# maiziezhoulab/FocalSV

Hardware: AMD Instinct MI355X
Metric: target regions/sec (50 kb, 30x HiFi) (higher is better)
Workload: dtype u32; 1 GPU; 256 synthetic 50 kb regions per GPU, 30x HiFi-like reads U(10k,20k), 0.2% error, seed 1000+i (BASELINE.json configs[1]); regions_per_gpu=256

## Files before the change

focalsv_amd/csrc/asm.hip:

```cpp
#include "asm_kernels.h"
#include "k_kmer.h"
#include "layout.h"
#include <algorithm>
#include <chrono>
#include <cstdio>
#include <cstdlib>
#include <cstring>
#include <vector>
#include <thread>
#include <atomic>

namespace {

enum { KN_SKETCH, KN_UNIQ, KN_CHAIN, KN_BPM, KN_RESCUE, KN_PATH_FAST, KN_PATH_DP, KN_CONSENSUS, KN_REPACK, KN_EXACT, KN_STITCH, KN_PARTITION, KN_BND, KN_BND_CONS,
       KN_UNIQ_LONG, KN_CHAIN_SPILL,
       KN_COUNT,
       ST_SKETCH = KN_COUNT, ST_CHAIN, ST_VERIFY, ST_PATH, ST_CONSENSUS, ST_FINAL };
const char *const kn_names[KN_COUNT] = {"k_sketch", "k_uniq", "k_chain", "k5_bpm", "k_rescue_accept", "k_path_fast", "k_path_dp", "k_consensus",
                                        "k_repack", "k_exact", "k_stitch", "k_partition", "k_bnd_tasks", "k_bnd_consensus", "k_uniq_long", "k_chain_spill"};
static_assert(KN_COUNT <= FSV_MAX_KERNEL_STATS, "fsv_asm_stats holds every kernel's row");
enum { PASS_NONE = -1, PASS_WINDOWS, PASS_JUNCTIONS, PASS_BCIG, PASS_COUNT };

struct KTimes {
    struct Rec { int k; hipEvent_t a, b; uint64_t bytes; };
// ... 281 lines not shown
    A.ovl = W.ovl.p; A.tasks = W.tasks.p; A.task_counter = ct + CT_TASKS; A.task_cap = R.task_cap;
    A.overflow = ct + CT_OVERFLOW; A.warn = W.warn.p; A.set_cols = W.set_cols.p; A.thr_tab = W.thr_tab.p;
    A.n_sets = B.n_sets; A.k_score = P.k; A.min_anchors = min_anchors; A.min_ovlp = min_ovlp; A.bw = final_pass ? P.bw_final : P.bw_ec;
    A.emit_tasks = final_pass ? 0 : 1; A.primary_only = 0;
    A.upair_tab = W.upair_tab.p; A.pair_list = nullptr; A.n_list_dev = nullptr;
    A.amax = wide_anchors ? FSV_AMAX_WIDE : FSV_AMAX;
    A.wide_list = nullptr; A.n_wide = nullptr;
    if (!wide_anchors) {
        TRY(ensure(ctx, W.wide_list, (size_t)B.n_upairs + 4));
        A.wide_list = W.wide_list.p; A.n_wide = ct + CT_WIDE;
    }
    A.spill_list = nullptr; A.n_spill = nullptr;
    if (P.full_lists) {
        TRY(ensure(ctx, W.spill_list, (size_t)B.n_upairs + 4));
        A.spill_list = W.spill_list.p; A.n_spill = ct + CT_SPILL;
    }
    A.stamps = nullptr;
    if (getenv("FSV_CHAIN_STAMPS")) {
        TRY(ensure(ctx, W.tmp, 16));
        TRY(zero(ctx, W.tmp, 16));
        A.stamps = W.tmp.p;
    }
    W.kt.begin(ctx, PASS_WINDOWS, KN_CHAIN, 0);
    const uint32_t n_chunks = ((B.n_upairs + FSV_CHAIN_CH - 1) / FSV_CHAIN_CH + 7u) & ~7u;
    TRY(launch_chain(ctx, CHAIN_CHUNKS, R.short_reads, n_chunks, A, B.n_upairs));
    if (A.wide_list) TRY(chain_wide_pairs(ctx, A, R.short_reads, B.n_upairs));
    W.kt.end(ctx);
    TRY(chain_spilled_pairs(ctx, W, A, B.n_upairs, max_slot, ct));
    if (A.stamps) {
        unsigned long long h[16];
        TRY(download(ctx, h, W.tmp, 16));
        FSV_HIP(ctx, hipStreamSynchronize(ctx->stream));
        static const char *nm[7] = {"stage lists", "lookups", "exit: few anchors", "compaction", "chain DP", "best + walk", "tasks + records"};
        fprintf(stderr, "[fsv] k_chain (%u pairs, tasks %d):", B.n_upairs, A.emit_tasks);
        for (int i = 0; i < 7; i++) fprintf(stderr, " %s %.0f cyc x %llu;", nm[i], h[8 + i] ? (double)h[i] / h[8 + i] : 0.0, h[8 + i]);
        fprintf(stderr, "\n");
        A.stamps = nullptr;
    }
    W.last_chain = A;
    tc.stop();
    return FSV_OK;
}

struct Piece { uint32_t read, rev, len; };
void layout_set(const int32_t *len, uint32_t n, const fsv_hit *hits, uint32_t n_hit, int min_reads,
                std::vector<std::vector<Piece>> &contigs, bool &fallback)
{
    std::vector<uint8_t> contained(n, 0), used(n, 0);
    std::vector<int32_t> succ(2 * n, -1), sovl(2 * n, 0), pred(2 * n, -1);
    fallback = false;
    struct Geom { int ql, tl, qs, qe, tl5, tl3, ext5, ext3, tspan; bool internal; };
    auto geom = [&](const fsv_hit &h) {
        Geom g;
        g.ql = len[h.q]; g.tl = len[h.t]; g.qs = h.x_s; g.qe = h.x_e + 1; g.tl5 = h.y_s; g.tl3 = g.tl - (h.y_e + 1);
        g.ext5 = std::min(g.qs, g.tl5); g.ext3 = std::min(g.ql - g.qe, g.tl3); g.tspan = h.y_e + 1 - h.y_s;
        g.internal = g.ext5 > 1000 || g.ext3 > 1000 || (g.qe - g.qs) < (g.qe - g.qs + g.ext5 + g.ext3) * 0.8f || g.tspan < (g.tspan + g.ext5 + g.ext3) * 0.8f;
        return g;
    };
    for (uint32_t i = 0; i < n_hit; i++) {
        const fsv_hit &h = hits[i];
        const Geom g = geom(h);
        if (g.internal) continue;
        if (g.qs <= g.tl5 && g.ql - g.qe <= g.tl3) {
            if (g.qs >= g.tl5 && g.ql - g.qe >= g.tl3) { if (h.q > h.t) contained[h.q] = 1; }
            else contained[h.q] = 1;
        }
    }
    for (uint32_t v = 0; v < 2 * n; v++) sovl[v] = 0x7fffffff;
    for (uint32_t i = 0; i < n_hit; i++) {
        const fsv_hit &h = hits[i];
        const Geom g = geom(h);
        if (g.internal || contained[h.q] || contained[h.t]) continue;
        if ((g.qs <= g.tl5 && g.ql - g.qe <= g.tl3) || (g.qs >= g.tl5 && g.ql - g.qe >= g.tl3)) continue;
        if (g.qe - g.qs + g.ext5 + g.ext3 < 50 || g.tspan + g.ext5 + g.ext3 < 50) continue;
        int from, to, l;
        if (g.qs > g.tl5) { from = 2 * (int)h.q; to = 2 * (int)h.t + (int)h.rev; l = g.qs - g.tl5; }
        else { from = 2 * (int)h.q + 1; to = 2 * (int)h.t + (h.rev ? 0 : 1); l = (g.ql - g.qe) - g.tl3; }
        if (l < sovl[from] || (l == sovl[from] && succ[from] >= 0 && to < succ[from])) { succ[from] = to; sovl[from] = l; }
    }
    for (uint32_t v = 0; v < 2 * n; v++) { int w = succ[v]; if (w >= 0 && succ[w ^ 1] != (int)(v ^ 1)) succ[v] = -1; }
    for (uint32_t v = 0; v < 2 * n; v++) if (succ[v] >= 0) pred[succ[v]] = (int)v;
    for (uint32_t v = 0; v < 2 * n; v++) {
        const uint32_t r = v >> 1;
        if (contained[r] || used[r]) continue;
        int start = (int)v, steps = 0;
        while (pred[start] >= 0 && !used[pred[start] >> 1] && steps < (int)(2 * n)) { start = pred[start]; steps++; if (start == (int)v) break; }
        int cnt = 0;
        for (int w = start; w >= 0 && !used[w >> 1] && cnt <= (int)(2 * n); w = succ[w]) { cnt++; if (succ[w] == start) break; }
        if (cnt < min_reads) continue;
        std::vector<Piece> c;
        for (int w = start; w >= 0 && !used[w >> 1]; w = succ[w]) {
            used[w >> 1] = 1;
            const bool more = succ[w] >= 0 && !used[succ[w] >> 1];
            c.push_back(Piece{(uint32_t)(w >> 1), (uint32_t)(w & 1), (uint32_t)(more ? sovl[w] : len[w >> 1])});
        }
        contigs.push_back(std::move(c));
    }
    fallback = contigs.empty();
}

}

extern "C" void fsv_asm_default_params(fsv_asm_params *p)
{
    if (!p) return;
    p->k = 51; p->w = 51; p->hpc = 1; p->n_rounds = 3; p->min_ovlp = 1; p->min_anchors = 1; p->lookback = 64;
    p->bw_ec = 20; p->bw_final = 0; p->min_contig_reads = 4;
    p->win_rate_pm = 40; p->k_cap = FSV_K_MAX; p->accept_err_pm = 30; p->bw_rechain = 1; p->w_later = 0; p->partition = 1; p->second_round = 1; p->ins_dag = 1;
    p->min_anchors_final = 1; p->min_ovlp_final = 1; p->graph_layout = 1; p->junction_cigars = 1;
    p->full_lists = 0;
    p->kmer_filter = 0;
    p->kmer_table = 0;
    p->partial_charge = 0;
}

extern "C" void fsv_asm_ont_params(fsv_asm_params *p)
{
    if (!p) return;
    fsv_asm_default_params(p);
    p->min_ovlp = 500; p->min_anchors = 3;
    p->k = 15; p->w = 15; p->hpc = 0;
    p->bw_ec = 150; p->bw_final = 50;
    p->win_rate_pm = 250; p->k_cap = FSV_K_WIDE; p->accept_err_pm = 300;
    p->bw_rechain = 50;
    p->w_later = 63;
    p->partition = 0;
    p->second_round = 0;
    p->ins_dag = 0;
    p->min_contig_reads = 2;
    p->min_anchors_final = 0; p->min_ovlp_final = 0; p->graph_layout = 0;
}

extern "C" void fsv_asm_clr_params(fsv_asm_params *p)
{
    fsv_asm_ont_params(p);
}

extern "C" int fsv_assemble_batch_bound(const fsv_readsets *sets, uint64_t *seq_cap, uint32_t *contig_cap)
{
    if (!sets || !sets->read_len) return FSV_EINVAL;
    uint64_t tot = 0;
    for (uint32_t r = 0; r < sets->n_reads; r++) tot += (uint64_t)sets->read_len[r];
    if (seq_cap) *seq_cap = tot + tot / 8 + 1024 * (uint64_t)sets->n_sets + 4096;
    if (contig_cap) *contig_cap = sets->n_reads + sets->n_sets + 1;
    return FSV_OK;
}

struct PathJob {
    const uint32_t *store; fsv_wtask *tasks; fsv_wres *res; fsv_wpath *paths;
    uint32_t task_cap; const uint32_t *n_tasks_dev; uint32_t *ct;
    int pass, round;
    bool wide_bands; int k_cap;
    bool all_accepted;
};

template <bool STAMP, class Grid>
static int path_walks(fsv_ctx *ctx, AsmWs &W, const PathJob &J, Grid persistent)
{
    const uint32_t *store = J.store; const fsv_wtask *tasks = J.tasks; const fsv_wres *res = J.res; fsv_wpath *paths = J.paths;
    uint32_t *ct = J.ct;
    unsigned long long h[16] = {0};
    uint32_t nl = 0;
    auto clear_stamps = [&]() -> int { TRY(ensure(ctx, W.tmp, 16)); return zero(ctx, W.tmp, 16); };
    auto read_stamps = [&](const uint32_t *cnt) -> int {
        TRY(download(ctx, h, W.tmp, 16));
        if (cnt) FSV_HIP(ctx, hipMemcpyAsync(&nl, cnt, 4, hipMemcpyDeviceToHost, ctx->stream));
        FSV_HIP(ctx, hipStreamSynchronize(ctx->stream));
        return FSV_OK;
    };
    auto per_wave = [&](int i) { return h[8 + i] ? (double)h[i] / h[8 + i] : 0.0; };
    if (!W.occ_sb) FSV_HIP(ctx, hipOccupancyMaxActiveBlocksPerMultiprocessor(&W.occ_sb, k_path_sb<false>, 64, 0));
    const uint32_t grid = persistent(W.occ_sb);
    TRY(ensure(ctx, W.cols_sb, (size_t)grid * FSV_SB_QUADS * 64));
    if (STAMP) TRY(clear_stamps());
    FSV_LAUNCH(ctx, ctx->stream, k_path_sb<STAMP>, dim3(grid), dim3(64), 0, store, tasks, res, W.dp_list2.p, ct + CT_DP_SB, paths, W.cols_sb.p,
               STAMP ? W.tmp.p : nullptr);
    if (STAMP) {
        TRY(read_stamps(nullptr));
        fprintf(stderr, "[fsv] k_path_sb round %d: %llu waves, cycles per wave: forward %.0f, walk %.0f, finish %.0f (grid %u)\n", J.round, h[8], per_wave(0), per_wave(1),
                per_wave(2), grid);
    }
    auto fr = [&](auto kern, int e, const Dev<uint32_t> &list, uint32_t *cnt) -> int {
        int &pf = W.occ_fr[e - 1];
        if (!pf || STAMP) FSV_HIP(ctx, hipOccupancyMaxActiveBlocksPerMultiprocessor(&pf, kern, 64, 0));
        if (STAMP) TRY(clear_stamps());
        FSV_LAUNCH(ctx, ctx->stream, kern, dim3(persistent(pf)), dim3(64), 0, store, tasks, res, list.p, cnt, paths, STAMP ? W.tmp.p : nullptr);
        if (STAMP) {
            TRY(read_stamps(cnt));
            fprintf(stderr, "[fsv] k_path_fr<%d> round %d: %u windows, %llu waves (%d per CU), cycles per wave: table %.0f, walk %.0f, finish %.0f\n", e, J.round, nl, h[8], pf,
                    per_wave(0), per_wave(1), per_wave(2));
        }
        return FSV_OK;
    };
    TRY(fr(k_path_fr<1, STAMP>, 1, W.dp_list16, ct + CT_DP_SB16));
    TRY(fr(k_path_fr<2, STAMP>, 2, W.dp_list, ct + CT_DP));
    TRY(fr(k_path_fr<3, STAMP>, 3, W.dp_list_e3, ct + CT_DP_FR3));
    return FSV_OK;
}

static int path_stage(fsv_ctx *ctx, AsmWs &W, const PathJob &J)
{
    const uint32_t *store = J.store; const fsv_wtask *tasks = J.tasks; const fsv_wres *res = J.res; fsv_wpath *paths = J.paths;
    uint32_t *ct = J.ct;
    const uint32_t task_cap = J.task_cap, n_cu = (uint32_t)ctx->n_cu;
    auto persistent = [&](int per_cu) { return std::min<uint32_t>(fsv_grid_for(task_cap, 64), (uint32_t)std::max(1, per_cu) * n_cu); };
    W.kt.begin(ctx, J.pass, KN_PATH_FAST, 0);
    const bool fix = J.pass == PASS_WINDOWS && !J.wide_bands;
    if (fix) TRY(ensure(ctx, W.fix_list, task_cap));
    const PathLists lists{{W.dp_list16.p, W.dp_list.p, W.dp_list_e3.p, W.dp_list2.p, W.dp_list3.p, W.dp_wide.p, W.dp_xwide.p, fix ? W.fix_list.p : nullptr},
                          {ct + CT_DP_SB16, ct + CT_DP, ct + CT_DP_FR3, ct + CT_DP_SB, ct + CT_DP_GEN, ct + CT_DP_WIDE, ct + CT_DP_XW, fix ? ct + CT_FIX : nullptr}};
    FSV_LAUNCH(ctx, ctx->stream, k_path_fast, dim3((fsv_grid_for(task_cap, 256) + 7u) & ~7u), dim3(256), 0, store, W.ovl.p, tasks, res, task_cap, paths, lists,
               J.all_accepted, J.n_tasks_dev);
    W.kt.end(ctx);
    W.kt.begin(ctx, J.pass, KN_PATH_DP, 0);
    TRY(getenv("FSV_K6_STAMPS") ? path_walks<true>(ctx, W, J, persistent) : path_walks<false>(ctx, W, J, persistent));
    const uint32_t gridg = persistent(2);
    TRY(ensure(ctx, W.cols, (size_t)gridg * 64 * (FSV_WINDOW + 2) * 3));
    FSV_LAUNCH(ctx, ctx->stream, k_path_dp<uint32_t>, dim3(gridg), dim3(64), 0, store, tasks, W.dp_list3.p, ct + CT_DP_GEN, paths,
               (uint32_t *)W.cols.p );
    FSV_LAUNCH(ctx, ctx->stream, k_path_dp<uint64_t>, dim3(gridg), dim3(64), 0, store, tasks, W.dp_wide.p, ct + CT_DP_WIDE, paths, W.cols.p);
    if (J.wide_bands) {
        if (!W.occ_wide) FSV_HIP(ctx, hipOccupancyMaxActiveBlocksPerMultiprocessor(&W.occ_wide, k_path_wide, 64, 0));
        const uint32_t gridw = persistent(std::min(W.occ_wide, 12));
        TRY(ensure(ctx, W.cols_wide, (size_t)gridw * FSV_WINDOW * 2 * FSV_WL * 64));
        FSV_LAUNCH(ctx, ctx->stream, k_path_wide, dim3(gridw), dim3(64), 0, store, tasks, res, W.dp_xwide.p, ct + CT_DP_XW, paths, W.cols_wide.p, J.k_cap);
    }
    if (fix)
        FSV_LAUNCH(ctx, ctx->stream, k_fix_boundary, dim3(persistent(8)), dim3(64), 0, store, W.fix_list.p, ct + CT_FIX, J.tasks, J.res, paths, J.k_cap, ct + CT_FIXED);
    W.kt.end(ctx);
    return FSV_OK;
}

static int second_pass(fsv_ctx *ctx, AsmWs &W, const Round &R)
{
    const fsv_asm_params &P = R.P; const Batch &B = R.B; const Geometry &G = R.G;
    const uint32_t n_gwin = R.n_gwin, task_cap = R.task_cap;
    uint32_t *ct2 = W.ct_of(R.row(PASS_JUNCTIONS));
    TRY(ensure(ctx, W.lb, std::max(1u, n_gwin)));
    W.kt.begin(ctx, PASS_JUNCTIONS, KN_BND, 0);
    FSV_LAUNCH(ctx, ctx->stream, k_newlen, dim3(fsv_grid_for(B.n_reads, 256)), dim3(256), 0, W.gwin_off.p, W.cwin_len.p, B.n_reads, W.new_len.p, W.lb.p);
    const uint32_t a_words = G.word_off[B.n_reads];
    std::vector<uint32_t> brel(B.n_reads + 1, 0);
    for (uint32_t r = 0; r < B.n_reads; r++) {
        const uint64_t nx = (uint64_t)brel[r] + (uint64_t)(G.gwin_off[r + 1] - G.gwin_off[r]) * (FSV_CW_STRIDE / 16) + 2;
        if (nx + a_words >= (1ull << 32)) return fsv_fail(ctx, FSV_EUNSUP, "second consensus pass: store larger than 2^32 words; split the batch");
        brel[r + 1] = (uint32_t)nx;
    }
    const uint32_t b_words = brel[B.n_reads];
    TRY(ensure(ctx, W.sr_store, (size_t)a_words + b_words + 16));
    FSV_HIP(ctx, hipMemcpyAsync(W.sr_store.p, R.store, (size_t)a_words * 4, hipMemcpyDeviceToDevice, ctx->stream));
    TRY(upload(ctx, W.brel_off, brel));
    uint32_t *store2 = W.sr_store.p;
    FSV_LAUNCH(ctx, ctx->stream, k_repack, dim3(B.n_reads), dim3(256), 0, W.gwin_off.p, W.lb.p, W.cwin.p, W.brel_off.p, W.new_len.p, B.n_reads, 0, store2 + a_words,
               W.read_dirty.p);
    FSV_HIP(ctx, hipMemsetAsync(store2 + a_words + b_words, 0, 32, ctx->stream));
    TRY(ensure_each(ctx, task_cap, W.tasks2, W.res2, W.paths2, W.idx2, W.tasks3, W.res3, W.src3));
    TRY(ensure_each(ctx, (size_t)n_gwin + 2, W.bnd_flag, W.bnd_list, W.bnd_patch));
    TRY(ensure(ctx, W.bnd_bytes, (size_t)(n_gwin + 2) * FSV_CW_STRIDE));
    TRY(zero(ctx, W.bnd_flag, (size_t)n_gwin + 2));
    BndArgs A;
    A.tasks = W.tasks.p; A.paths = W.paths.p; A.n_tasks = R.ct + CT_TASKS;
    A.ovl_c = W.ovl_c.p; A.pair_base = W.pair_base.p; A.set_start = W.set_start.p; A.n_sets = B.n_sets; A.pair_read = W.pair_read.p;
    A.gwin_off = W.gwin_off.p; A.lb = W.lb.p; A.cwin_len = W.cwin_len.p;
    A.cov3 = W.cov3.p; A.read_dirty = W.read_dirty.p;
    A.brel_off = W.brel_off.p; A.b_base = a_words; A.thr_tab = W.thr_tab.p;
    A.tasks2 = W.tasks2.p; A.idx2 = W.idx2.p; A.n_tasks2 = ct2 + CT_TASKS;
    A.bnd_flag = W.bnd_flag.p; A.bnd_list = W.bnd_list.p; A.n_bnd = ct2 + CT_B_LIST; A.store2 = store2;
    FSV_LAUNCH(ctx, ctx->stream, k_bnd_tasks, dim3((fsv_grid_for(task_cap, 256) + 7u) & ~7u), dim3(256), 0, A);
    W.kt.end(ctx);
    W.kt.begin(ctx, PASS_JUNCTIONS, KN_BPM, 0);
    TRY(fsv_bpm_windows_dev_n(ctx, store2, W.tasks2.p, task_cap, ct2 + CT_TASKS, W.res2.p, P.k_cap));
    FSV_LAUNCH(ctx, ctx->stream, k_bnd_retry, dim3(fsv_grid_for(task_cap, 256)), dim3(256), 0, W.tasks2.p, W.res2.p, ct2 + CT_TASKS, W.tasks3.p, W.src3.p,
               ct2 + CT_B_RETRY, P.k_cap);
    TRY(fsv_bpm_windows_dev_n(ctx, store2, W.tasks3.p, task_cap, ct2 + CT_B_RETRY, W.res3.p, P.k_cap));
    FSV_LAUNCH(ctx, ctx->stream, k_bnd_scatter, dim3(fsv_grid_for(task_cap, 256)), dim3(256), 0, W.res2.p, W.res3.p, W.src3.p, ct2 + CT_B_RETRY);
    W.kt.end(ctx);
    TRY(path_stage(ctx, W, PathJob{store2, W.tasks2.p, W.res2.p, W.paths2.p, task_cap, ct2 + CT_TASKS, ct2, PASS_JUNCTIONS, R.round, R.wide_bands, P.k_cap, false}));
    const uint32_t grid_l = std::min<uint32_t>(std::max(1u, n_gwin), (uint32_t)ctx->n_cu * 16);
    W.kt.begin(ctx, PASS_JUNCTIONS, KN_BND_CONS, 0);
    if (R.wide_bands) FSV_LAUNCH(ctx, ctx->stream, k_bnd_consensus<FSV_EV_CAP_WIDE>, dim3(grid_l), dim3(64), 0, R.C, A, W.paths2.p, store2, W.bnd_patch.p, W.bnd_bytes.p);
    else FSV_LAUNCH(ctx, ctx->stream, k_bnd_consensus<FSV_EV_CAP>, dim3(grid_l), dim3(64), 0, R.C, A, W.paths2.p, store2, W.bnd_patch.p, W.bnd_bytes.p);
    FSV_LAUNCH(ctx, ctx->stream, k_bnd_apply, dim3(std::max(1u, n_gwin)), dim3(64), 0, W.gwin_read.p, W.gwin_off.p, W.bnd_patch.p, W.bnd_bytes.p, W.bnd_flag.p, n_gwin,
               W.cwin.p, W.cwin_len.p, W.changed.p, W.warn.p);
    W.kt.end(ctx);
    return FSV_OK;
}

static int fsv_bpm_paths_impl(fsv_ctx *ctx, const uint32_t *store, size_t store_words, const fsv_wtask *tasks, uint32_t n_tasks,
                             fsv_wres *res, fsv_wpath *paths)
{
    if (!ctx || !store || (!tasks && n_tasks) || (!res && n_tasks) || (!paths && n_tasks)) return FSV_EINVAL;
    if (n_tasks == 0) return FSV_OK;
    int kmax = 0;
    for (uint32_t i = 0; i < n_tasks; i++) {
        if (tasks[i].k > FSV_K_WIDE || tasks[i].x_len == 0 || tasks[i].x_len > FSV_WINDOW) return fsv_fail(ctx, FSV_EINVAL, "task k/x_len out of range");
        kmax = std::max<int>(kmax, tasks[i].k);
    }
    const int k_cap = kmax > FSV_K_MAX ? kmax : FSV_K_MAX;
    FSV_HIP(ctx, hipSetDevice(ctx->device));
    AsmWs &W = *ws_get(ctx);
    W.kt.reset();
    std::vector<fsv_wtask> t(tasks, tasks + n_tasks);
    for (auto &x : t) x.ovl = 0;
    fsv_ovl o; memset(&o, 0, sizeof(o)); o.valid = 1; o.is_match = 1;
    Dev<uint32_t> d_store;
    TRY(ensure(ctx, d_store, store_words + 16));
    TRY(zero(ctx, d_store, store_words + 16));
    FSV_HIP(ctx, hipMemcpyAsync(d_store.p, store, store_words * 4, hipMemcpyHostToDevice, ctx->stream));
    TRY(upload(ctx, W.tasks, t));
    TRY(upload(ctx, W.ovl, std::vector<fsv_ovl>{o}));
    TRY(ensure_each(ctx, n_tasks, W.res, W.paths, W.dp_list, W.dp_list2, W.dp_list3, W.dp_list16, W.dp_list_e3, W.dp_wide, W.dp_xwide));
    TRY(ensure(ctx, W.counters, CT_SLOT));
    TRY(zero(ctx, W.counters, CT_SLOT));
    TRY(zero(ctx, W.paths, n_tasks));
    TRY(fsv_bpm_windows_dev_n(ctx, d_store.p, W.tasks.p, n_tasks, nullptr, W.res.p, k_cap));
    TRY(path_stage(ctx, W, PathJob{d_store.p, W.tasks.p, W.res.p, W.paths.p, n_tasks, nullptr, W.counters.p, PASS_NONE, 0, kmax > FSV_K_MAX, k_cap, true}));
    TRY(download(ctx, res, W.res, n_tasks));
    TRY(download(ctx, paths, W.paths, n_tasks));
    FSV_HIP(ctx, hipStreamSynchronize(ctx->stream));
    return FSV_OK;
}

static int launch_bpm_ext(fsv_ctx *ctx, const uint32_t *store, const fsv_wtask *tasks, const uint32_t *list, const uint32_t *n_dev, uint32_t bound, int k_cap,
                          fsv_wext *out, unsigned long long *n_run)
{
    if (!bound) return FSV_OK;
    const uint32_t grid = std::min<uint32_t>(fsv_grid_for(bound, 64), 8u * (uint32_t)std::max(1, ctx->n_cu));
    FSV_LAUNCH(ctx, ctx->stream, k_bpm_ext, dim3(grid), dim3(64), 0, store, tasks, list, n_dev, bound, k_cap, out, n_run);
    return FSV_OK;
}

static int fsv_bpm_extensions_impl(fsv_ctx *ctx, const uint32_t *store, size_t store_words, const fsv_wtask *tasks, const uint8_t *dir, uint32_t n_tasks,
                                   int32_t k_cap, fsv_wext *out)
{
    if (!ctx || !store || (n_tasks && (!tasks || !dir || !out))) return FSV_EINVAL;
    if (k_cap < 1 || k_cap > FSV_K_WIDE) return fsv_fail(ctx, FSV_EINVAL, "k_cap must be in [1, 95]");
    if (n_tasks == 0) return FSV_OK;
    std::vector<fsv_wtask> t(tasks, tasks + n_tasks);
    for (uint32_t i = 0; i < n_tasks; i++) {
        fsv_wtask &x = t[i];
        if (x.k > FSV_K_MAX || x.x_len == 0 || x.x_len > FSV_WINDOW || dir[i] > 1) return fsv_fail(ctx, FSV_EINVAL, "extension task: k <= 31 (FSV_K_MAX), 1 <= x_len <= 375, dir 0 or 1");
        if (x.x_start < 0 || x.y_len < 0 || (uint64_t)x.x_word + ((uint64_t)x.x_start + x.x_len + 15) / 16 > store_words ||
            (uint64_t)x.y_word + ((uint64_t)x.y_len + 15) / 16 > store_words)
            return fsv_fail(ctx, FSV_EINVAL, "extension task reaches outside the store");
        x.ovl = i; x.win = dir[i];
    }
    FSV_HIP(ctx, hipSetDevice(ctx->device));
    AsmWs &W = *ws_get(ctx);
    Dev<uint32_t> d_store;
    TRY(ensure(ctx, d_store, store_words + 16));
    TRY(zero(ctx, d_store, store_words + 16));
    FSV_HIP(ctx, hipMemcpyAsync(d_store.p, store, store_words * 4, hipMemcpyHostToDevice, ctx->stream));
    TRY(upload(ctx, W.ch.ext_tasks, t));
    TRY(ensure(ctx, W.ch.ext_res, n_tasks));
    TRY(launch_bpm_ext(ctx, d_store.p, W.ch.ext_tasks.p, nullptr, nullptr, n_tasks, k_cap, W.ch.ext_res.p, nullptr));
    TRY(download(ctx, out, W.ch.ext_res, n_tasks));
    FSV_HIP(ctx, hipStreamSynchronize(ctx->stream));
    return FSV_OK;
}

static int fsv_asm_last_charge_impl(const fsv_ctx *ctx, fsv_charge_stats *out)
{
    if (!ctx || !out || !ctx->asm_ws) return FSV_EINVAL;
    const AsmWs &W = *(const AsmWs *)ctx->asm_ws;
    if (!W.ch.valid) return FSV_EINVAL;
    *out = W.ch.last;
    return FSV_OK;
}

extern "C" int fsv_asm_last_stats(const fsv_ctx *ctx, fsv_asm_stats *out)
{
    if (!ctx || !out || !ctx->asm_ws) return FSV_EINVAL;
    *out = ((const AsmWs *)ctx->asm_ws)->stats;
    return FSV_OK;
}


static int prepare_batch(fsv_ctx *ctx, AsmWs &W, const fsv_readsets *sets, Round &R)
{
    const fsv_asm_params &P = R.P; Batch &B = R.B;
    B.n_reads = sets->n_reads;
    R.set_flags = sets->set_flags;
    B.set_start.clear(); R.caller_set.clear();
    for (uint32_t s = 0; s < sets->n_sets; s++) {
        const bool low = !R.low_cov.empty() && R.low_cov[s];
        for (uint32_t r = sets->set_start[s]; r < sets->set_start[s + 1]; r++) if (low || r == sets->set_start[s]) { B.set_start.push_back(r); R.caller_set.push_back(s); }
        if (sets->set_start[s + 1] == sets->set_start[s]) { B.set_start.push_back(sets->set_start[s]); R.caller_set.push_back(s); }
    }
    B.n_sets = (uint32_t)R.caller_set.size();
    B.set_start.push_back(B.n_reads);
    B.read_set.resize(B.n_reads); B.pair_base.resize(B.n_sets + 1); B.upair_base.resize(B.n_sets + 1);
    uint64_t np = 0;
    for (uint32_t s = 0; s < B.n_sets; s++) {
        uint64_t ns = B.set_start[s + 1] - B.set_start[s];
        B.pair_base[s] = (uint32_t)np;
        B.upair_base[s] = (uint32_t)(np / 2);
        np += ns > 1 ? ns * (ns - 1) : 0;
        for (uint32_t r = B.set_start[s]; r < B.set_start[s + 1]; r++) B.read_set[r] = s;
    }
    if (np >= (1ull << 31)) return fsv_fail(ctx, FSV_EUNSUP, "too many read pairs in one batch; split it");
    B.pair_base[B.n_sets] = (uint32_t)np; B.n_pairs = (uint32_t)np;
    B.upair_base[B.n_sets] = (uint32_t)(np / 2); B.n_upairs = (uint32_t)(np / 2);
    std::vector<int32_t> &len = R.len;
    len.assign(sets->read_len, sets->read_len + B.n_reads);

    std::vector<uint8_t> thr(FSV_WINDOW + 1);
    for (int i = 0; i <= FSV_WINDOW; i++) thr[i] = thr_for_len_host(i, P.win_rate_pm);
    TRY(upload(ctx, W.thr_tab, thr));
    TRY(upload(ctx, W.set_start, B.set_start));
    TRY(upload(ctx, W.read_set, B.read_set));
    TRY(upload(ctx, W.pair_base, B.pair_base));
    TRY(upload(ctx, W.upair_base, B.upair_base));
    if (B.n_upairs) {
        TRY(ensure(ctx, W.upair_tab, B.n_upairs));
        TRY(ensure(ctx, W.pair_read, B.n_pairs));
        FSV_LAUNCH(ctx, ctx->stream, k_pair_tab, dim3((B.n_upairs + 255) / 256), dim3(256), 0, W.set_start.p, W.pair_base.p, W.upair_base.p, B.n_sets, B.n_upairs,
                   W.upair_tab.p, W.pair_read.p);
    }
    TRY(ensure(ctx, W.warn, B.n_reads));
    TRY(zero(ctx, W.warn, B.n_reads));

    R.mz_fixed.assign(B.n_reads + 1, 0);
    {
        uint64_t m = 0;
        for (uint32_t r = 0; r < B.n_reads; r++) { R.mz_fixed[r] = (uint32_t)m; m += mz_slots((int64_t)len[r] + len[r] / 8 + 64, P.w_later > 0 ? std::min(P.w, P.w_later) : P.w, P.full_lists != 0); }
        if (m >= (1ull << 32)) return fsv_fail(ctx, FSV_EUNSUP, "batch too large for 32-bit offsets; split it");
        R.mz_fixed[B.n_reads] = (uint32_t)m;
    }
    TRY(make_geometry(ctx, B, len, R.G, P.w, &R.mz_fixed));
    for (uint32_t r = 0; r <= B.n_reads; r++) R.G.word_off[r] = (uint32_t)sets->word_off[r];
    R.store = sets->store_dev;
    R.wide_bands = P.k_cap > FSV_K_MAX;
    for (uint32_t r = 0; r < B.n_reads; r++) { R.reads_in_bytes += (uint64_t)(len[r] + 3) / 4; if (len[r] >= 65536) R.short_reads = false; }
    const size_t n_ct = (size_t)(3 * P.n_rounds + 2) * CT_SLOT;
    TRY(ensure(ctx, W.counters, n_ct));
    TRY(zero(ctx, W.counters, n_ct));
    R.h_ct.assign(n_ct, 0u);
    TRY(ensure(ctx, W.set_cols, B.n_reads));
    TRY(zero(ctx, W.set_cols, B.n_reads));
    return FSV_OK;
}

static int begin_round(fsv_ctx *ctx, AsmWs &W, Round &R)
{
    R.ct = W.ct_of(R.row(PASS_WINDOWS));
    TRY(upload(ctx, W.word_off, R.G.word_off));
    TRY(upload(ctx, W.len, R.len));
    TRY(upload(ctx, W.mz_off, R.G.mz_off));
    TRY(upload(ctx, W.gwin_off, R.G.gwin_off));
    TRY(upload(ctx, W.gwin_read, R.G.gwin_read));
    if (R.G.task_bound >= (1ull << 31)) return fsv_fail(ctx, FSV_EUNSUP, "window task bound exceeds 2^31; split the batch");
    const uint32_t task_cap = R.task_cap = (uint32_t)std::max<uint64_t>(R.G.task_bound, 1);
    R.n_gwin = R.G.gwin_off[R.B.n_reads];
    TRY(ensure_each(ctx, task_cap, W.tasks, W.res, W.paths, W.dp_list, W.dp_list_e3, W.dp_list2, W.dp_list3, W.dp_list16, W.dp_wide));
    TRY(ensure(ctx, W.dp_xwide, R.wide_bands ? task_cap : 16));
    return FSV_OK;
}

static int charge_stage(fsv_ctx *ctx, AsmWs &W, const Round &R)
{
    const fsv_asm_params &P = R.P; const Batch &B = R.B;
    const uint32_t ext_cap = 2u * R.task_cap;
    ChargeState &S = W.ch;
    TRY(ensure_each(ctx, ext_cap, S.ext_tasks, S.ext_res, S.ext_list));
    TRY(ensure(ctx, S.list, (size_t)B.n_pairs + 4));
    TRY(ensure(ctx, S.n, 2));
    TRY(zero(ctx, S.n, 2));
    ChargeArgs A;
    A.ovl = W.ovl.p; A.n_pairs = B.n_pairs; A.tasks = W.tasks.p; A.res = W.res.p; A.paths = W.paths.p; A.ovl_c = W.ovl_c.p;
    A.ext_tasks = S.ext_tasks.p; A.ext_res = S.ext_res.p; A.ext_list = S.ext_list.p; A.n_ext = S.n.p;
    A.ovl_list = S.list.p; A.n_ovl = S.n.p + 1; A.stats = S.ct.p;
    A.k_cap = P.k_cap; A.accept_err_pm = P.accept_err_pm;
    TRY(S.clock.mark(ctx));
    FSV_LAUNCH(ctx, ctx->stream, k_charge_tasks, dim3(fsv_grid_for(B.n_pairs, 64)), dim3(64), 0, A);
    TRY(launch_bpm_ext(ctx, R.store, S.ext_tasks.p, S.ext_list.p, S.n.p, ext_cap, P.k_cap, S.ext_res.p, S.ct.p + CH_EXT));
    FSV_LAUNCH(ctx, ctx->stream, k_charge_accept, dim3(fsv_grid_for(B.n_pairs, 64)), dim3(64), 0, A);
    TRY(S.clock.mark(ctx));
    return FSV_OK;
}

static int verify_stage(fsv_ctx *ctx, AsmWs &W, const Round &R)
{
    const fsv_asm_params &P = R.P; const Batch &B = R.B;
    uint32_t *ct = R.ct;
    unsigned long long *cols = (unsigned long long *)(ct + CT_COLS_LO);
    Span tv(ctx, W.kt, ST_VERIFY);
    W.kt.begin(ctx, PASS_WINDOWS, KN_BPM, 0);
    TRY(fsv_bpm_windows_dev_n(ctx, R.store, W.tasks.p, R.task_cap, ct + CT_TASKS, W.res.p, P.k_cap));
    W.kt.end(ctx);
    W.kt.begin(ctx, PASS_WINDOWS, KN_RESCUE, (uint64_t)B.n_pairs * sizeof(fsv_ovl) * 2);
    if (R.wide_bands)
        FSV_LAUNCH(ctx, ctx->stream, k_rescue_accept<true>, dim3(fsv_grid_for(B.n_pairs, 64)), dim3(64), 0, R.store, W.ovl.p, B.n_pairs, W.tasks.p, W.res.p, cols,
                   W.ovl_c.p, P.k_cap, P.accept_err_pm, (uint32_t *)nullptr, (uint32_t *)nullptr);
    else {
        TRY(ensure(ctx, W.left_list, (size_t)B.n_pairs + 4));
        const uint32_t gridl = std::min<uint32_t>(std::max(1u, B.n_pairs), 8u * (uint32_t)ctx->n_cu);
        if (!P.partial_charge) {
            FSV_LAUNCH(ctx, ctx->stream, k_rescue_accept<false>, dim3(fsv_grid_for(B.n_pairs, 64)), dim3(64), 0, R.store, W.ovl.p, B.n_pairs, W.tasks.p, W.res.p, cols,
                       W.ovl_c.p, P.k_cap, P.accept_err_pm, W.left_list.p, ct + CT_LEFT);
            FSV_LAUNCH(ctx, ctx->stream, k_left_rescue<false>, dim3(gridl), dim3(64), 0, R.store, W.ovl.p, W.left_list.p, ct + CT_LEFT, W.tasks.p, W.res.p, W.paths.p,
                       W.ovl_c.p, P.k_cap, P.accept_err_pm);
        } else {
            FSV_LAUNCH(ctx, ctx->stream, (k_rescue_accept<false, true>), dim3(fsv_grid_for(B.n_pairs, 64)), dim3(64), 0, R.store, W.ovl.p, B.n_pairs, W.tasks.p, W.res.p,
                       cols, W.ovl_c.p, P.k_cap, P.accept_err_pm, W.left_list.p, ct + CT_LEFT);
            FSV_LAUNCH(ctx, ctx->stream, k_left_rescue<true>, dim3(gridl), dim3(64), 0, R.store, W.ovl.p, W.left_list.p, ct + CT_LEFT, W.tasks.p, W.res.p, W.paths.p,
                       W.ovl_c.p, P.k_cap, P.accept_err_pm);
        }
    }
    W.kt.end(ctx);
    tv.stop();
    Span tp(ctx, W.kt, ST_PATH);
    TRY(path_stage(ctx, W, PathJob{R.store, W.tasks.p, W.res.p, W.paths.p, R.task_cap, R.ct + CT_TASKS, R.ct, PASS_WINDOWS, R.round, R.wide_bands, R.P.k_cap, false}));
    tp.stop();
    if (P.partial_charge) TRY(charge_stage(ctx, W, R));
    return FSV_OK;
}

static int consensus_setup(fsv_ctx *ctx, AsmWs &W, Round &R)
{
    const fsv_asm_params &P = R.P; const Batch &B = R.B;
    const uint32_t n_gwin = R.n_gwin;
    TRY(ensure(ctx, W.cwin, (size_t)n_gwin * FSV_CW_STRIDE));
    TRY(ensure(ctx, W.cwin_len, n_gwin));
    TRY(ensure(ctx, W.new_len, B.n_reads));
    if (!B.n_pairs) TRY(zero(ctx, W.ovl_c, 1));
    TRY(ensure(ctx, W.gwin_tab, std::max(1u, n_gwin)));
    FSV_LAUNCH(ctx, ctx->stream, k_gwin_tab, dim3(fsv_grid_for(n_gwin, 256)), dim3(256), 0, W.gwin_read.p, W.gwin_off.p, W.read_set.p, W.set_start.p, W.pair_base.p, n_gwin,
               W.gwin_tab.p);
    ConsArgs &C = R.C;
    C.store = R.store; C.word_off = W.word_off.p; C.read_len = W.len.p;
    C.read_set = W.read_set.p; C.set_start = W.set_start.p; C.pair_base = W.pair_base.p;
    C.gwin_off = W.gwin_off.p; C.gwin_read = W.gwin_read.p; C.ovl_c = W.ovl_c.p;
    C.gwin_tab = W.gwin_tab.p; C.tasks = W.tasks.p;
    C.paths = W.paths.p; C.cwin = W.cwin.p; C.cwin_len = W.cwin_len.p; C.warn = W.warn.p;
    C.n_reads = B.n_reads;
    TRY(ensure(ctx, W.changed, B.n_reads));
    TRY(zero(ctx, W.changed, B.n_reads));
    C.changed = W.changed.p;
    C.read_dirty = nullptr;
    C.junction_vote = P.second_round ? 0 : 1;
    C.ins_dag = P.ins_dag ? 1 : 0;
    C.cov3 = nullptr;
    if (P.second_round && B.n_pairs) { TRY(ensure(ctx, W.cov3, std::max(1u, n_gwin))); C.cov3 = W.cov3.p; }
    if (B.n_pairs) {
        TRY(ensure(ctx, W.read_dirty, B.n_reads));
        FSV_LAUNCH(ctx, ctx->stream, k_read_dirty, dim3(B.n_reads), dim3(64), 0, W.ovl_c.p, W.paths.p, W.read_set.p, W.set_start.p, W.pair_base.p, B.n_reads, W.read_dirty.p);
        C.read_dirty = W.read_dirty.p;
    }
    return FSV_OK;
}

static int partition_setup(fsv_ctx *ctx, AsmWs &W, const Round &R, SiteArgs &SA, SiteLists &SL)
{
    const Batch &B = R.B;
    const uint32_t n_gwin = R.n_gwin;
    const size_t vec_cap = (size_t)B.n_pairs * 64 + (1u << 20);
    TRY(ensure(ctx, W.site_cnt, std::max(1u, n_gwin)));
    const size_t rec_cap = (size_t)n_gwin * 4 + 65536;
    TRY(ensure(ctx, W.site_rec, rec_cap));
    TRY(ensure(ctx, W.site_off, std::max(1u, n_gwin)));
    TRY(ensure(ctx, W.site_vec, vec_cap));
    TRY(ensure(ctx, W.site_cursor, 4));
    TRY(ensure(ctx, W.redo, B.n_reads));
    TRY(ensure(ctx, W.site_lists, (size_t)std::max(1u, n_gwin) * 2));
    TRY(zero(ctx, W.site_cursor, 4));
    TRY(zero(ctx, W.redo, B.n_reads));
    SA.site_cnt = W.site_cnt.p; SA.site_rec = W.site_rec.p; SA.vec = W.site_vec.p;
    SA.site_off = W.site_off.p; SA.rec_cursor = W.site_cursor.p + 3; SA.rec_cap = (uint32_t)std::min<size_t>(rec_cap, 0xfffffff0u);
    SA.vec_cursor = W.site_cursor.p; SA.vec_cap = (uint32_t)std::min<size_t>(vec_cap, 0xfffffff0u);
    SA.read_sites = W.redo.p;
    SL.site_cnt = SA.site_cnt; SL.win_list = W.site_lists.p; SL.redo_list = SL.win_list + std::max(1u, n_gwin);
    SL.win_n = W.site_cursor.p + 1;
    return FSV_OK;
}

static int junction_cigars(fsv_ctx *ctx, AsmWs &W, const Round &R, SiteArgs &SA, SiteLists &SL)
{
    const fsv_asm_params &P = R.P;
    const uint32_t n_gwin = R.n_gwin, task_cap = R.task_cap;
    uint32_t *ct3 = W.ct_of(R.row(PASS_BCIG));
    TRY(ensure_each(ctx, task_cap, W.tasks2, W.res2, W.paths2, W.bc_idx, W.bc_rec));
    TRY(ensure(ctx, W.bc_win, (size_t)(n_gwin + 2) * 3));
    FSV_LAUNCH(ctx, ctx->stream, k_bcwin_init, dim3(fsv_grid_for(n_gwin + 2, 256)), dim3(256), 0, W.bc_win.p, n_gwin + 2);
    BcigArgs BA;
    BA.tasks = W.tasks.p; BA.paths = W.paths.p; BA.n_tasks = R.ct + CT_TASKS;
    BA.pair_read = W.pair_read.p; BA.read_dirty = W.read_dirty.p; BA.gwin_off = W.gwin_off.p;
    BA.thr_tab = W.thr_tab.p; BA.k_cap = P.k_cap;
    BA.tasks2 = W.tasks2.p; BA.bc_idx = W.bc_idx.p; BA.n_tasks2 = ct3 + CT_TASKS;
    BA.n_same = ct3 + CT_B_RETRY; BA.n_used = ct3 + CT_B_LIST;
    BA.res2 = W.res2.p; BA.paths2 = W.paths2.p; BA.bc_rec = W.bc_rec.p; BA.bc_win = W.bc_win.p;
    W.kt.begin(ctx, KN_PARTITION, 0);
    FSV_LAUNCH(ctx, ctx->stream, k_bcig_tasks, dim3((fsv_grid_for(task_cap, 256) + 7u) & ~7u), dim3(256), 0, BA);
    W.kt.end(ctx);
    W.kt.begin(ctx, PASS_BCIG, KN_BPM, 0);
    TRY(fsv_bpm_windows_dev_n(ctx, R.store, W.tasks2.p, task_cap, ct3 + CT_TASKS, W.res2.p, P.k_cap));
    W.kt.end(ctx);
    TRY(path_stage(ctx, W, PathJob{R.store, W.tasks2.p, W.res2.p, W.paths2.p, task_cap, ct3 + CT_TASKS, ct3, PASS_BCIG, R.round, R.wide_bands, P.k_cap, false}));
    W.kt.begin(ctx, KN_PARTITION, 0);
    FSV_LAUNCH(ctx, ctx->stream, k_bcig_accept, dim3(fsv_grid_for(task_cap, 256)), dim3(256), 0, BA);
    W.kt.end(ctx);
    SA.bc_idx = W.bc_idx.p; SA.bc_rec = W.bc_rec.p; SA.bc_paths = W.paths2.p;
    SL.bc_win = W.bc_win.p;
    return FSV_OK;
}

static int consensus_stage(fsv_ctx *ctx, AsmWs &W, Round &R)
{
    const fsv_asm_params &P = R.P; const Batch &B = R.B;
    const uint32_t n_gwin = R.n_gwin;
    TRY(consensus_setup(ctx, W, R));
    const ConsArgs &C = R.C;
    const bool partition = B.n_pairs && P.partition;
    SiteArgs SA{};
    SiteLists SL{};
    if (partition) TRY(partition_setup(ctx, W, R, SA, SL));
    if (partition && P.junction_cigars) TRY(junction_cigars(ctx, W, R, SA, SL));
    const dim3 grid_w((n_gwin + 7u) & ~7u);
    W.kt.begin(ctx, PASS_WINDOWS, KN_CONSENSUS, (uint64_t)n_gwin * (96 + 448));
    if (R.wide_bands) {
        if (partition) FSV_LAUNCH(ctx, ctx->stream, (k_consensus<FSV_EV_CAP_WIDE, 1>), grid_w, dim3(64), 0, C, n_gwin, SL);
        else FSV_LAUNCH(ctx, ctx->stream, (k_consensus<FSV_EV_CAP_WIDE, 0>), grid_w, dim3(64), 0, C, n_gwin, SL);
    } else {
        if (partition) FSV_LAUNCH(ctx, ctx->stream, (k_consensus<FSV_EV_CAP, 1>), grid_w, dim3(64), 0, C, n_gwin, SL);
        else FSV_LAUNCH(ctx, ctx->stream, (k_consensus<FSV_EV_CAP, 0>), grid_w, dim3(64), 0, C, n_gwin, SL);
    }
    W.kt.end(ctx);
    if (partition) {
        const uint32_t grid_l = std::min<uint32_t>(std::max(1u, n_gwin), (uint32_t)ctx->n_cu * 16);
        W.kt.begin(ctx, KN_PARTITION, (uint64_t)B.n_reads * 4);
        FSV_LAUNCH(ctx, ctx->stream, k_snp_sites, dim3(grid_l), dim3(64), 0, C, SA, SL);
        FSV_LAUNCH(ctx, ctx->stream, k_hap_partition, dim3(B.n_reads), dim3(64), 0, C, SA, W.ovl.p, W.ovl_c.p, SL);
        if (R.wide_bands) FSV_LAUNCH(ctx, ctx->stream, k_consensus_redo<FSV_EV_CAP_WIDE>, dim3(grid_l), dim3(64), 0, C, SL);
        else FSV_LAUNCH(ctx, ctx->stream, k_consensus_redo<FSV_EV_CAP>, dim3(grid_l), dim3(64), 0, C, SL);
        W.kt.end(ctx);
    }
    return FSV_OK;
}

static int finish_round(fsv_ctx *ctx, AsmWs &W, Round &R)
{
    const fsv_asm_params &P = R.P; const Batch &B = R.B;
    const uint32_t n_gwin = R.n_gwin;
    TRY(ensure(ctx, W.lb, std::max(1u, n_gwin)));
    FSV_LAUNCH(ctx, ctx->stream, k_newlen, dim3(fsv_grid_for(B.n_reads, 256)), dim3(256), 0, W.gwin_off.p, W.cwin_len.p, B.n_reads, W.new_len.p, W.lb.p);
    std::vector<int32_t> nlen(B.n_reads);
    TRY(download(ctx, nlen.data(), W.new_len, B.n_reads));
    for (int pass = 0; pass < PASS_COUNT; pass++)
        FSV_HIP(ctx, hipMemcpyAsync(R.h_ct.data() + (size_t)R.row(pass) * CT_SLOT, W.ct_of(R.row(pass)), CT_SLOT * 4, hipMemcpyDeviceToHost, ctx->stream));
    FSV_HIP(ctx, hipStreamSynchronize(ctx->stream));
    if (R.h_ct[(size_t)R.round * CT_SLOT + CT_OVERFLOW]) return fsv_fail(ctx, FSV_ECAP, "internal window task buffer overflow");
    Geometry G2;
    TRY(make_geometry(ctx, B, nlen, G2, P.w, &R.mz_fixed));
    Dev<uint32_t> &dst = W.store[R.round & 1];
    const uint32_t total_words = G2.word_off[B.n_reads];
    TRY(ensure(ctx, dst, (size_t)total_words + 8));
    TRY(upload(ctx, W.unpack_off, G2.word_off));
    W.kt.begin(ctx, KN_REPACK, (uint64_t)n_gwin * 384 + (uint64_t)total_words * 4);
    FSV_LAUNCH(ctx, ctx->stream, k_repack, dim3(B.n_reads), dim3(256), 0, W.gwin_off.p, W.lb.p, W.cwin.p, W.unpack_off.p, W.new_len.p, B.n_reads,
               R.round + 1 < P.n_rounds ? 1 : 0, dst.p);
    W.kt.end(ctx);
    FSV_HIP(ctx, hipMemsetAsync(dst.p + total_words, 0, 32, ctx->stream));
    R.store = dst.p;
    R.len = nlen;
    for (int32_t l : R.len) if (l >= 65536) R.short_reads = false;
    R.G = G2;
    return FSV_OK;
}

struct SetLayout { std::vector<std::vector<Piece>> contigs; bool fallback = false; };
struct Final {
    std::vector<uint32_t> hit_first, hwarn, h_setcols;
    const fsv_hit *hraw = nullptr;
    bool any_inexact = false;
    std::vector<SetLayout> lay;
    uint64_t used = 0;
    Trace trace;
};

static int begin_final(fsv_ctx *ctx, AsmWs &W, Round &R)
{
    R.ct = W.ct_of(R.P.n_rounds); R.task_cap = 0;
    TRY(upload(ctx, W.word_off, R.G.word_off));
    TRY(upload(ctx, W.len, R.len));
    TRY(upload(ctx, W.mz_off, R.G.mz_off));
    TRY(ensure(ctx, W.tasks, 2));
    return FSV_OK;
}

static int rechain_listed(fsv_ctx *ctx, AsmWs &W, const Round &R, const uint32_t *n_list_dev)
{
    const fsv_asm_params &P = R.P; const Batch &B = R.B;
    ChainArgs A2 = W.last_chain;
    A2.bw = P.bw_rechain; A2.emit_tasks = 0; A2.pair_list = W.inexact_list.p; A2.n_list_dev = n_list_dev;
    A2.primary_only = 1;
    TRY(ensure(ctx, W.upair_tab_sw, std::max(1u, B.n_upairs)));
    FSV_LAUNCH(ctx, ctx->stream, k_pair_tab_swap, dim3(fsv_grid_for(B.n_upairs, 256)), dim3(256), 0, W.upair_tab.p, B.n_upairs, W.upair_tab_sw.p);
    for (int side = 0; side < 2; side++) {
        const size_t tk = W.kt.begin(ctx, KN_CHAIN, 0);
        if (side == 1) A2.upair_tab = W.upair_tab_sw.p;
        if (A2.wide_list) FSV_HIP(ctx, hipMemsetAsync(A2.n_wide, 0, 4, ctx->stream));
        if (A2.spill_list) FSV_HIP(ctx, hipMemsetAsync(A2.n_spill, 0, 4, ctx->stream));
        TRY(launch_chain(ctx, CHAIN_PAIRS, R.short_reads, B.n_upairs, A2, B.n_upairs));
        if (A2.wide_list) TRY(chain_wide_pairs(ctx, A2, R.short_reads, B.n_upairs));
        W.kt.end(ctx, tk);
        TRY(chain_spilled_pairs(ctx, W, A2, B.n_upairs, longest_slot(R.G, B.n_reads), R.ct));
    }
    return FSV_OK;
}

static int final_overlaps(fsv_ctx *ctx, AsmWs &W, Round &R, Final &F)
{
    const fsv_asm_params &P = R.P; const Batch &B = R.B;
    TRY(begin_final(ctx, W, R));
    const bool have_prev = P.n_rounds > 0 && B.n_pairs > 0;
    if (have_prev) {
        TRY(ensure(ctx, W.ovl_prev, B.n_pairs));
        FSV_HIP(ctx, hipMemcpyAsync(W.ovl_prev.p, W.ovl.p, (size_t)B.n_pairs * sizeof(fsv_ovl), hipMemcpyDeviceToDevice, ctx->stream));
    }
    TRY(overlap_stage(ctx, W, R, true));
    F.trace("overlaps");
    if (!B.n_pairs) return FSV_OK;
    TRY(ensure(ctx, W.hits, B.n_pairs));
    TRY(ensure(ctx, W.set_hits, (size_t)2 * B.n_sets + 2));
    TRY(zero(ctx, W.set_hits, B.n_sets));
    W.kt.begin(ctx, KN_EXACT, (uint64_t)B.n_pairs * sizeof(fsv_ovl));
    TRY(ensure(ctx, W.exact_flag, (size_t)B.n_upairs + 16));
    FSV_LAUNCH(ctx, ctx->stream, k_exact, dim3(B.n_upairs), dim3(64), 0, R.store, W.word_off.p, W.len.p, W.read_set.p, W.pair_base.p, W.upair_tab.p, W.ovl.p,
               W.hits.p, W.set_hits.p, W.exact_flag.p);
    W.kt.end(ctx);
    if (!have_prev) return FSV_OK;
    TRY(ensure(ctx, W.inexact_list, (size_t)B.n_upairs + 4));
    uint32_t *n_list_dev = R.ct + CT_INEXACT;
    FSV_LAUNCH(ctx, ctx->stream, k_inexact_list, dim3(fsv_grid_for(B.n_upairs, 256)), dim3(256), 0, W.upair_tab.p, W.exact_flag.p, W.ovl_prev.p, B.n_upairs,
               W.inexact_list.p, n_list_dev);
    TRY(rechain_listed(ctx, W, R, n_list_dev));
    FSV_LAUNCH(ctx, ctx->stream, k_accept_inexact, dim3(fsv_grid_for(2ull * B.n_upairs, 256)), dim3(256), 0, W.upair_tab.p, W.inexact_list.p, 0u, W.ovl.p, W.ovl_prev.p,
               W.read_set.p, W.pair_base.p, W.hits.p, W.set_hits.p, n_list_dev);
    return FSV_OK;
}

static int gather_hits(fsv_ctx *ctx, AsmWs &W, Round &R, Final &F)
{
    const Batch &B = R.B;
    F.hit_first.assign(B.n_sets + 1, 0);
    F.hwarn.resize(B.n_reads); F.h_setcols.assign(B.n_reads, 0u);
    if (B.n_pairs) TRY(download(ctx, F.hit_first.data() + 1, W.set_hits, B.n_sets));
    TRY(download(ctx, F.hwarn.data(), W.warn, B.n_reads));
    TRY(download(ctx, F.h_setcols.data(), W.set_cols, B.n_reads));
    FSV_HIP(ctx, hipMemcpyAsync(R.h_ct.data() + (size_t)R.P.n_rounds * CT_SLOT, R.ct, CT_SLOT * 4, hipMemcpyDeviceToHost, ctx->stream));
    FSV_HIP(ctx, hipStreamSynchronize(ctx->stream));
    if (B.n_pairs) {
        std::vector<uint32_t> &hit_first = F.hit_first;
// ... 23 lines not shown
{
    const fsv_asm_params &P = R.P; const Batch &B = R.B; const Geometry &G = R.G;
    const std::vector<int32_t> &len = R.len;
    const std::vector<uint32_t> &hit_first = F.hit_first;
    const fsv_hit *hraw = F.hraw;
    std::vector<uint32_t> &h_store = W.h_store;
    bool any_inexact = false;
    if (P.graph_layout && hraw) {
        for (uint32_t s2 = 0; s2 < B.n_sets; s2++) {
            bool inexact = false;
            for (uint32_t i = hit_first[s2]; i < hit_first[s2 + 1] && !inexact; i++) inexact = !(hraw[i].slot >> 31);
            if (!inexact) continue;
            if (!any_inexact && h_store.size() < (size_t)G.word_off[B.n_reads] + 1) h_store.resize((size_t)G.word_off[B.n_reads] + 1);
            any_inexact = true;
            const uint32_t w0 = G.word_off[B.set_start[s2]], w1 = G.word_off[B.set_start[s2 + 1]];
            if (w1 > w0) FSV_HIP(ctx, hipMemcpyAsync(h_store.data() + w0, R.store + w0, (size_t)(w1 - w0) * 4, hipMemcpyDeviceToHost, ctx->stream));
        }
        if (any_inexact) FSV_HIP(ctx, hipStreamSynchronize(ctx->stream));
    }
    F.any_inexact = any_inexact;
    const uint8_t *set_flags = R.set_flags;
    std::vector<SetLayout> &lay = F.lay;
    lay.resize(B.n_sets);
    const uint32_t nthr = std::max(1u, std::min({8u, std::thread::hardware_concurrency(), B.n_sets / 16 + 1}));
    std::atomic<uint32_t> next{0};
    std::atomic<int> rc_work{FSV_OK};
    auto work = [&]() {
        try {
        for (uint32_t s = next.fetch_add(1); s < B.n_sets && rc_work.load() == FSV_OK; s = next.fetch_add(1)) {
            const uint32_t r0 = B.set_start[s], ns = B.set_start[s + 1] - r0;
            if (ns == 0) continue;
            if (R.is_low(s)) { lay[s].fallback = true; continue; }
            const uint32_t nh_s = hit_first[s + 1] - hit_first[s];
            const bool unphased = set_flags && (set_flags[R.caller_set[s]] & FSV_SET_UNPHASED);
            if (P.graph_layout && !unphased) {
                fsv_layout::ReadBases rb; rb.words = any_inexact ? h_store.data() : nullptr; rb.word_off = G.word_off.data() + r0; rb.len = len.data() + r0;
                fsv_layout::Graph g(len.data() + r0, (int)ns, rb);
                std::vector<fsv_layout::Hit> hs(nh_s);
                for (uint32_t i = 0; i < nh_s; i++) {
                    const fsv_hit &h = hraw[hit_first[s] + i];
                    const int tl = len[r0 + h.t];
                    fsv_layout::Hit &x = hs[i];
                    x.qn = (int32_t)h.q; x.tn = (int32_t)h.t; x.qs = h.x_s; x.qe = h.x_e + 1; x.rev = (uint8_t)h.rev; x.el = (uint8_t)(h.slot >> 31); x.del = 0;
                    if (h.rev) { x.ts = tl - h.y_e - 1; x.te = tl - h.y_s; } else { x.ts = h.y_s; x.te = h.y_e + 1; }
                }
                g.set_hits(std::move(hs));
                g.build();
                std::vector<std::vector<fsv_layout::PieceOut>> cs;
                g.unitigs(P.min_contig_reads, cs);
                for (auto &c : cs) { std::vector<Piece> pc; for (auto &e : c) pc.push_back(Piece{e.read, e.rev, e.len}); lay[s].contigs.push_back(std::move(pc)); }
                lay[s].fallback = cs.empty();
                continue;
            }
            layout_set(len.data() + r0, ns, hraw + hit_first[s], nh_s, P.min_contig_reads, lay[s].contigs, lay[s].fallback);
        }
        } catch (const std::bad_alloc &) { int ok = FSV_OK; rc_work.compare_exchange_strong(ok, FSV_ENOMEM); }
        catch (...) { int ok = FSV_OK; rc_work.compare_exchange_strong(ok, FSV_EINTERNAL); }
    };
    struct Joiner { std::vector<std::thread> thr; ~Joiner() { for (auto &t : thr) if (t.joinable()) t.join(); } };
    {
        Joiner j;
        j.thr.reserve(nthr);
        for (uint32_t t = 1; t < nthr; t++) j.thr.emplace_back(work);
        work();
    }
    if (rc_work.load() != FSV_OK) return fsv_fail(ctx, rc_work.load(), rc_work.load() == FSV_ENOMEM ? "out of host memory (layout)" : "exception in the layout of a read set");
    return FSV_OK;
}

static int emit_contigs(fsv_ctx *ctx, AsmWs &W, const Round &R, Final &F, fsv_contigs *out)
{
    const Batch &B = R.B;
    std::vector<fsv_piece> pieces;
    uint64_t used = 0;
    uint32_t nc = 0;
    int rc_out = FSV_OK;
    for (uint32_t s = 0; s < B.n_sets && rc_out == FSV_OK; s++) {
        const uint32_t r0 = B.set_start[s], ns = B.set_start[s + 1] - r0;
        int32_t st = 0;
        for (uint32_t r = r0; r < r0 + ns; r++) st |= (int32_t)(F.hwarn[r] & (FSV_W_MZ_TRUNC | FSV_W_ANCHOR_TRUNC | FSV_W_INS_EVENTS | FSV_W_WINDOW_KEPT | FSV_W_INTERNAL | FSV_W_SITES));
        const uint32_t cs = R.caller_set[s];
        if (ns == 0) { out->set_status[cs] |= st; continue; }
        if (F.lay[s].fallback) st |= FSV_W_NO_LAYOUT;
        for (auto &c : F.lay[s].contigs) {
            uint64_t clen = 0;
            for (auto &pc : c) clen += pc.len;
            if (nc >= out->contig_cap || used + clen > out->seq_cap) { rc_out = fsv_fail(ctx, FSV_ECAP, "contig output buffers too small (use fsv_assemble_batch_bound)"); break; }
            for (auto &pc : c) { pieces.push_back(fsv_piece{r0 + pc.read, pc.rev, pc.len, 0u, used}); used += pc.len; }
            out->set[nc] = cs; out->n_reads[nc] = (uint32_t)c.size();
            out->off[++nc] = used;
        }
        out->set_status[cs] |= st;
    }
    F.trace("layout");
    if (rc_out != FSV_OK) return rc_out;
    out->n_contigs = nc;
    ctx->last_contigs_dev = nullptr;
    ctx->last_contig_off.assign(out->off, out->off + nc + 1);
    if (!pieces.empty()) {
        TRY(upload(ctx, W.pieces, pieces));
        TRY(ensure(ctx, W.contig_out, used + 16));
        W.kt.begin(ctx, KN_STITCH, used + used / 4);
        FSV_LAUNCH(ctx, ctx->stream, k_stitch, dim3((uint32_t)pieces.size()), dim3(256), 0, R.store, W.word_off.p, W.len.p, W.pieces.p, W.contig_out.p);
        W.kt.end(ctx);
        ctx->last_contigs_dev = W.contig_out.p;
        TRY(download(ctx, out->seq, W.contig_out, used));
        FSV_HIP(ctx, hipStreamSynchronize(ctx->stream));
    }
    F.trace("stitch+d2h");
    F.used = used;
    return FSV_OK;
}

static void fill_stats(AsmWs &W, const Round &R, const Final &F)
{
    const fsv_asm_params &P = R.P; const Batch &B = R.B;
    const std::vector<uint32_t> &h_ct = R.h_ct;
    KTimes &kt = W.kt;
    auto set = [&](int pass, int k, size_t round, uint64_t bytes) { if (uint64_t *b = kt.bytes_of(pass, k, round)) *b = bytes; };
    auto add = [&](int pass, int k, size_t round, uint64_t bytes) { if (uint64_t *b = kt.bytes_of(pass, k, round)) *b += bytes; };
    auto n_dp_of = [](const uint32_t *c) { return (uint64_t)c[CT_DP_SB] + c[CT_DP_SB16] + c[CT_DP] + c[CT_DP_FR3] + c[CT_DP_GEN] + c[CT_DP_WIDE] + c[CT_DP_XW]; };
    uint64_t mz_total[17] = {0}, n_windows2 = 0;
    for (int sl = 0; sl <= P.n_rounds; sl++) {
        const uint32_t *c = h_ct.data() + (size_t)sl * CT_SLOT;
        mz_total[sl] = (uint64_t)c[CT_MZ_LO] | (uint64_t)c[CT_MZ_HI] << 32;
        W.n_long_reads += c[CT_UQ_LONG]; W.n_spilled_pairs += c[CT_SPILLED];
        if (sl == P.n_rounds) { W.stats.n_inexact_candidates = c[CT_INEXACT]; break; }
        W.stats.n_windows += c[CT_TASKS];
        W.stats.dp_columns += (uint64_t)c[CT_COLS_LO] | (uint64_t)c[CT_COLS_HI] << 32;
        W.stats.n_path_dp += n_dp_of(c);
        W.stats.n_path_fr += (uint64_t)c[CT_DP_SB16] + c[CT_DP] + c[CT_DP_FR3];
        const uint64_t nt = c[CT_TASKS], n_dp = n_dp_of(c);
        set(PASS_WINDOWS, KN_BPM, sl, nt * 212ull);
        add(PASS_WINDOWS, KN_RESCUE, sl, nt * 16ull);
        set(PASS_WINDOWS, KN_PATH_FAST, sl, nt * (16ull + 196ull) + (nt - n_dp) * 128ull);
        set(PASS_WINDOWS, KN_PATH_DP, sl, n_dp * (196ull + 128ull));
        add(PASS_WINDOWS, KN_CONSENSUS, sl, nt * 128ull);
        if (kt.bytes_of(PASS_BCIG, KN_BPM, sl)) {
            const uint32_t *c3 = h_ct.data() + (size_t)(PASS_BCIG * (P.n_rounds + 1) + sl) * CT_SLOT;
            const uint64_t n3 = c3[CT_TASKS], n_dp3 = n_dp_of(c3);
            n_windows2 += n3;
            W.stats.n_junction_cigars += n3;
            W.stats.n_junction_used += c3[CT_B_LIST];
            if (getenv("FSV_BCIG_DEBUG")) fprintf(stderr, "[fsv] round %d: %u overlaps set aside for the left-extension pass; fix_boundary: %u candidates, %u windows moved\n", sl, c[CT_LEFT], c[CT_FIX], c[CT_FIXED]);
            if (getenv("FSV_BCIG_DEBUG")) fprintf(stderr, "[fsv] round %d: %llu junction cigars, %u accepted but showing what the window cigars show, %u used\n", sl, (unsigned long long)n3, c3[CT_B_RETRY], c3[CT_B_LIST]);
            set(PASS_BCIG, KN_BPM, sl, n3 * 212ull);
            set(PASS_BCIG, KN_PATH_FAST, sl, n3 * (16ull + 196ull) + (n3 - n_dp3) * 128ull);
            set(PASS_BCIG, KN_PATH_DP, sl, n_dp3 * (196ull + 128ull));
        }
        if (kt.bytes_of(PASS_JUNCTIONS, KN_BND, sl)) {
            const uint32_t *c2 = h_ct.data() + (size_t)(PASS_JUNCTIONS * (P.n_rounds + 1) + sl) * CT_SLOT;
            const uint64_t n2 = c2[CT_TASKS], n3 = c2[CT_B_RETRY], n_dp2 = n_dp_of(c2);
            n_windows2 += n2 + n3;
            set(PASS_JUNCTIONS, KN_BND, sl, nt * (sizeof(fsv_wtask) + 128ull) + n2 * sizeof(fsv_wtask));
            set(PASS_JUNCTIONS, KN_BPM, sl, (n2 + n3) * 212ull);
            set(PASS_JUNCTIONS, KN_PATH_FAST, sl, n2 * (16ull + 196ull) + (n2 - n_dp2) * 128ull);
            set(PASS_JUNCTIONS, KN_PATH_DP, sl, n_dp2 * (196ull + 128ull));
            set(PASS_JUNCTIONS, KN_BND_CONS, sl, n2 * 128ull + (uint64_t)c2[CT_B_LIST] * (sizeof(BndPatch) + 2ull * FSV_BND_HALF));
        }
    }
    for (size_t i = 0; i <= (size_t)P.n_rounds; i++) {
        const uint32_t *c = h_ct.data() + i * CT_SLOT;
        const uint64_t raw = (uint64_t)c[CT_MZRAW_LO] | (uint64_t)c[CT_MZRAW_HI] << 32, bases = (uint64_t)c[CT_BASES_LO] | (uint64_t)c[CT_BASES_HI] << 32;
        set(PASS_WINDOWS, KN_SKETCH, i, bases / 4 + raw * sizeof(fsv_mz));
        set(PASS_WINDOWS, KN_UNIQ, i, raw * sizeof(fsv_mz) + mz_total[i] * 2 * sizeof(fsv_mz));
        set(PASS_WINDOWS, KN_CHAIN, i, mz_total[i] * 32ull + (uint64_t)B.n_pairs * sizeof(fsv_ovl) + (i < (size_t)P.n_rounds ? (uint64_t)c[CT_TASKS] * sizeof(fsv_wtask) : 0ull));
    }
    for (uint32_t s2 = 0; s2 < B.n_sets; s2++) if (B.set_start[s2] < B.n_reads && B.set_start[s2 + 1] > B.set_start[s2]) W.stats.dp_columns += F.h_setcols[B.set_start[s2]];
    W.stats.algo_bytes = (W.stats.n_windows + n_windows2) * 212ull + R.reads_in_bytes * (uint64_t)(P.n_rounds + 1) + F.used;
    W.stats.ms_total = std::chrono::duration<double, std::milli>(std::chrono::steady_clock::now() - R.t_enter).count();
    W.stats.n_kernels = KN_COUNT;
    for (int k = 0; k < KN_COUNT; k++) { memset(&W.stats.kernels[k], 0, sizeof(fsv_kernel_stat)); strncpy(W.stats.kernels[k].name, kn_names[k], 23); }
    for (auto &r : kt.recs) {
        float ms = 0;
        const bool ok = hipEventElapsedTime(&ms, r.a, r.b) == hipSuccess;
        if (r.k >= KN_COUNT) {
            double *dst = r.k == ST_SKETCH ? &W.stats.ms_sketch : r.k == ST_CHAIN ? &W.stats.ms_chain : r.k == ST_VERIFY ? &W.stats.ms_verify
                        : r.k == ST_PATH ? &W.stats.ms_path : r.k == ST_CONSENSUS ? &W.stats.ms_consensus : &W.stats.ms_final;
            if (ok) *dst += ms;
            continue;
        }
        if (ok) W.stats.kernels[r.k].ms += ms;
        W.stats.kernels[r.k].launches++;
        W.stats.kernels[r.k].algo_bytes += r.bytes;
    }
}

static void add_stats(fsv_asm_stats &total, const fsv_asm_stats &st)
{
    total.n_pairs += st.n_pairs; total.n_overlaps += st.n_overlaps; total.n_windows += st.n_windows; total.n_windows_matched += st.n_windows_matched;
    total.n_paths += st.n_paths; total.n_path_dp += st.n_path_dp; total.dp_columns += st.dp_columns; total.algo_bytes += st.algo_bytes;
    total.n_exact_overlaps += st.n_exact_overlaps; total.n_inexact_candidates += st.n_inexact_candidates; total.n_path_fr += st.n_path_fr;
    total.ms_sketch += st.ms_sketch; total.ms_chain += st.ms_chain; total.ms_verify += st.ms_verify; total.ms_path += st.ms_path;
    total.ms_consensus += st.ms_consensus; total.ms_final += st.ms_final; total.ms_total += st.ms_total;
    total.n_kernels = st.n_kernels;
    for (uint32_t k = 0; k < st.n_kernels; k++) {
        memcpy(total.kernels[k].name, st.kernels[k].name, sizeof(st.kernels[k].name));
        total.kernels[k].ms += st.kernels[k].ms; total.kernels[k].launches += st.kernels[k].launches; total.kernels[k].algo_bytes += st.kernels[k].algo_bytes;
    }
}

static bool readsets_present(const fsv_readsets *sets, bool with_sets)
{
    return sets && sets->store_dev && sets->word_off && sets->read_len && (!with_sets || sets->set_start);
}

enum { RS_SETS = 1, RS_LEN = 2, RS_WORD_OFF = 4, RS_ALL = RS_SETS | RS_LEN | RS_WORD_OFF };
static int check_readsets(fsv_ctx *ctx, const fsv_readsets *sets, unsigned what)
{
    const uint32_t n_reads = sets->n_reads, n_sets = sets->n_sets;
    if (what & RS_SETS) {
        if (n_sets == 0 ? n_reads != 0 : (sets->set_start[0] != 0 || sets->set_start[n_sets] != n_reads)) return fsv_fail(ctx, FSV_EINVAL, "set_start must span [0, n_reads]");
        for (uint32_t s = 0; s < n_sets; s++) if (sets->set_start[s + 1] < sets->set_start[s]) return fsv_fail(ctx, FSV_EINVAL, "set_start not monotone");
    }
    if (what & RS_LEN)
        for (uint32_t r = 0; r < n_reads; r++) if (sets->read_len[r] < 1 || sets->read_len[r] >= (1 << 24)) return fsv_fail(ctx, FSV_EUNSUP, "read length must be in [1, 2^24)");
    if ((what & RS_WORD_OFF) && n_reads)
        for (uint32_t r = 0; r <= n_reads; r++) if (sets->word_off[r] >= (1ull << 32)) return fsv_fail(ctx, FSV_EUNSUP, "store larger than 2^32 words; split the batch");
    return FSV_OK;
}

static std::vector<uint32_t> read_set_of(const fsv_readsets *sets)
{
    std::vector<uint32_t> read_set(sets->n_reads);
    for (uint32_t s = 0; s < sets->n_sets; s++) for (uint32_t r = sets->set_start[s]; r < sets->set_start[s + 1]; r++) read_set[r] = s;
    return read_set;
}

static int stage_sketch_reads(fsv_ctx *ctx, AsmWs &W, const fsv_readsets *sets, int w, const std::vector<uint32_t> *read_set, Geometry &G, bool full_lists = false)
{
    const uint32_t n_reads = sets->n_reads;
    Batch B;
    B.n_reads = n_reads; B.n_sets = 1; B.set_start = {0u, n_reads};
    const std::vector<int32_t> len(sets->read_len, sets->read_len + n_reads);
    TRY(make_geometry(ctx, B, len, G, w, nullptr, full_lists));
    for (uint32_t r = 0; r <= n_reads; r++) G.word_off[r] = (uint32_t)sets->word_off[r];
    TRY(upload(ctx, W.word_off, G.word_off));
    TRY(upload(ctx, W.len, len));
    TRY(upload(ctx, W.mz_off, G.mz_off));
    if (read_set) TRY(upload(ctx, W.read_set, *read_set));
    TRY(ensure(ctx, W.warn, n_reads));
    TRY(zero(ctx, W.warn, n_reads));
    TRY(ensure(ctx, W.mz, G.mz_off[n_reads]));
    TRY(ensure(ctx, W.mz_cnt, n_reads));
    return FSV_OK;
}

template <class T> int append_on_device(fsv_ctx *ctx, Dev<T> &b, size_t have, const T *src, size_t n, size_t slack = 0, size_t min_elems = 0)
{
    if (!n) return FSV_OK;
    if (b.cap < (have + n + slack) * sizeof(T)) {
        Dev<T> bigger;
        TRY(ensure(ctx, bigger, std::max((have + n) * 2, min_elems)));
        if (have) FSV_HIP(ctx, hipMemcpyAsync(bigger.p, b.p, have * sizeof(T), hipMemcpyDeviceToDevice, ctx->stream));
        FSV_HIP(ctx, hipStreamSynchronize(ctx->stream));
        b.swap(bigger);
    }
    FSV_HIP(ctx, hipMemcpyAsync(b.p + have, src, n * sizeof(T), hipMemcpyDeviceToDevice, ctx->stream));
    return FSV_OK;
}

struct KmerJob {
    const fsv_readsets *sets; int w, k, hpc;
    const SketchFilter *sketch_flt;
    double *ms;
};
struct KmerResult {
    std::vector<fsv_kmer_set> sets;
    std::vector<uint32_t> hist;
    std::vector<uint64_t> flt_off;
};
struct KmerRun {
    const KmerJob &J; KmerResult &R; EventClock clock;
    std::vector<uint64_t> entries, tab_off; std::vector<KmerTile> tiles; std::vector<int32_t> cutoff;
};

static int kmer_sketch(fsv_ctx *ctx, AsmWs &W, KmerRun &K)
{
    const KmerJob &J = K.J; const fsv_readsets *sets = J.sets;
    const uint32_t n_reads = sets->n_reads, n_sets = sets->n_sets;
    K.entries.assign(n_sets, 0); K.tab_off.assign((size_t)n_sets + 1, 0);
    if (!n_reads) return FSV_OK;
    const std::vector<uint32_t> read_set = read_set_of(sets);
    Geometry G;
    TRY(stage_sketch_reads(ctx, W, sets, J.w, &read_set, G));
    TRY(K.clock.mark(ctx));
    TRY(launch_sketch(ctx, W, SketchJob{sets->store_dev, n_reads, G.word_off[n_reads], G.max_words, J.w, J.k, J.hpc, nullptr, J.w, false, nullptr,
                                     J.sketch_flt ? *J.sketch_flt : SketchFilter{}}));
    TRY(K.clock.mark(ctx));
    std::vector<uint32_t> cnt(n_reads);
    TRY(download(ctx, cnt.data(), W.mz_cnt, n_reads));
    FSV_HIP(ctx, hipStreamSynchronize(ctx->stream));
    for (uint32_t r = 0; r < n_reads; r++) K.entries[read_set[r]] += std::min<uint32_t>(cnt[r], G.mz_off[r + 1] - G.mz_off[r]);
    for (uint32_t s = 0; s < n_sets; s++) {
        const uint64_t slots = kmer_table_slots(K.entries[s]), tile = std::min<uint64_t>(slots, FSV_KMER_TILE);
        K.tab_off[s + 1] = K.tab_off[s] + slots;
        for (uint64_t f = 0; f < slots; f += tile) K.tiles.push_back(KmerTile{s, (uint32_t)tile, f});
    }
    if (K.tiles.size() >= (1ull << 31)) return fsv_fail(ctx, FSV_EUNSUP, "k-mer tables too large for one pass; split the batch");
    return FSV_OK;
}

static int kmer_count(fsv_ctx *ctx, AsmWs &W, KmerRun &K)
{
    KmerTableState &S = W.km;
    const uint32_t n_reads = K.J.sets->n_reads, n_sets = K.J.sets->n_sets;
    const uint64_t total_slots = K.tab_off[n_sets];
// ... 635 lines not shown
```

focalsv_amd/csrc/asm_kernels.h:

```cpp
#pragma once
#include "bpm_device.h"
#include "k_sketch.h"
#include <type_traits>

#define FSV_AMAX       1024
#define FSV_AMAX_WIDE_LONG 2560
#define FSV_AMAX_WIDE  4096
#define FSV_PATH_CAP    416
#define FSV_CW_STRIDE   448
#define FSV_INS_MAXLEN   12
#define FSV_SB_MAXERR    7
#define FSV_SB_QUADS ((FSV_WINDOW + 3) / 4)
#define FSV_FR_MAXERR    3
#define FSV_EV_CAP_WIDE 2048
#define FSV_EV_CAP     256

static_assert(sizeof(fsv_wpath) == 128, "fsv_wpath layout");

namespace {


struct ChainArgs {
    const uint32_t *store;
    const uint32_t *word_off;
// ... 705 lines not shown
        __threadfence_block();
        __syncthreads();
    }
}

__host__ __device__ inline size_t chain_lds_bytes(bool short_reads, int amax) { return short_reads ? (size_t)amax * 12 + (size_t)amax / 8 : (size_t)amax * 24; }

__device__ __forceinline__ int double_thr(int pre, int x_len, int k_cap)
{
    if (pre == 0 && x_len >= 4) pre = 1;
    int t = pre * 2;
    if (x_len >= 300 && t < k_cap) t = k_cap;
    if (t > k_cap) t = k_cap;
    return t;
}

template <bool WIDE, bool DEFER = false>
__global__ __launch_bounds__(64) void k_rescue_accept(const uint32_t *__restrict__ store, fsv_ovl *__restrict__ ovl, uint32_t n_pairs,
                                                      fsv_wtask *__restrict__ tasks, fsv_wres *__restrict__ res,
                                                      unsigned long long *__restrict__ stat_cols, uint4 *__restrict__ ovl_c, int k_cap, int accept_err_pm,
                                                      uint32_t *__restrict__ left_list, uint32_t *__restrict__ n_left)
{
    const uint32_t p = blockIdx.x * 64 + threadIdx.x;
    if (p >= n_pairs) return;
    fsv_ovl o = ovl[p];
    if (!o.valid) { ovl_c[p] = make_uint4(0u, 0u, 0u, 0u); return; }
    fsv_wtask *T = tasks + o.first_win;
    fsv_wres *R = res + o.first_win;
    int align = 0;
    unsigned long long cols = 0;
    int n_bad = 0;
    long long tlen0 = 0, terr0 = 0;
#pragma unroll 4
    for (int j = 0; j < o.n_win; j++) {
        const int e = R[j].err, xl = T[j].x_len;
        if (e >= 0) { align += xl; terr0 += e; } else n_bad++;
        tlen0 += xl;
    }
    for (int j = n_bad ? o.n_win - 1 : -1; j >= 0; j--) {
        if (R[j].err < 0) continue;
        int next = R[j].y_beg + R[j].end_site - R[j].extra_begin + 1;
        for (int k2 = j + 1; k2 < o.n_win && R[k2].err < 0; k2++) {
            fsv_wtask u = T[k2];
            if (next >= u.y_len) break;
            u.k = (uint8_t)double_thr(u.k, u.x_len, k_cap);
            u.y_start = next;
            fsv_wres r;
            if (!bpm_window_geometry(u, r, k_cap)) break;
            if ((u.x_len + 2 * u.k - r.extra_begin - r.extra_end) + u.k < u.x_len) break;
            if (WIDE) { WideNoSink none; bpm_run_wide(store, u, r, none, k_cap); }
            else bpm_run(store, u, r, BpmNoSink());
            cols += u.x_len;
            if (r.err < 0) break;
            T[k2] = u; R[k2] = r;
            align += u.x_len;
            next = r.y_beg + r.end_site - r.extra_begin + 1;
        }
    }
    if (n_bad && left_list) {
        bool left = false;
        for (int j = 1; j < o.n_win && !left; j++) left = R[j].err >= 0 && R[j - 1].err < 0;
        if (left) {
            left_list[atomicAdd(n_left, 1u)] = p;
            o.is_match = 0; ovl[p] = o;
            ovl_c[p] = make_uint4((uint32_t)o.x_s, (uint32_t)o.first_win, (uint32_t)o.n_win, 0u);
            if (cols) atomicAdd(stat_cols, cols);
            return;
        }
    }
    long long tlen = tlen0, terr = terr0;
    if (n_bad) {
        terr = 0;
#pragma unroll 4
        for (int j = 0; j < o.n_win; j++) { const int e = R[j].err; terr += e >= 0 ? e : T[j].x_len; }
    }
    o.align_len = align; o.err_sum = (int32_t)terr;
    const bool covered = (long long)(o.x_e - o.x_s + 1) * 9 <= (long long)align * 10;
    o.is_match = (covered && (DEFER || terr * 1000 <= tlen * accept_err_pm)) ? 1 : 0;
    ovl[p] = o;
    ovl_c[p] = make_uint4((uint32_t)o.x_s, (uint32_t)o.first_win, (uint32_t)o.n_win | (o.is_match && !DEFER ? 0x80000000u : 0u), 0u);
    if (cols) atomicAdd(stat_cols, cols);
}

struct PathLists {
    uint32_t *list[8], *cnt[8];
};
template <class Words>
__device__ __forceinline__ void path_record(fsv_wpath *__restrict__ P, const fsv_wtask &t, int start, int end, int plen, int err, bool raw0, uint32_t tail10,
                                            bool with_ops, Words word)
{
    uint32_t head10 = 0;
    if (with_ops) {
        uint2 *dst = reinterpret_cast<uint2 *>(P->ops);
        for (int i = 0; i < FSV_PATH_CAP / 32; i++) {
            const uint32_t v0 = word(2 * i), v1 = word(2 * i + 1);
            if (i == 0) head10 = v0 & 0xfffffu;
            dst[i] = make_uint2(v0, v1);
        }
    }
    P->ry_start = t.y_start - t.k + start;
    P->ry_end = t.y_start - t.k + end;
    P->path_len = (int16_t)plen; P->err = (int16_t)err; P->state = 1; P->y_rev = t.y_rev;
    P->pad = (uint16_t)((head10 ? 1u : 0u) | (tail10 ? 2u : 0u) | (raw0 ? 4u : 0u)); P->y_word = t.y_word; P->y_len = t.y_len;
}

__device__ __forceinline__ bool path_gapfree(const uint32_t *__restrict__ store, const fsv_wtask &t, const fsv_wres &r, fsv_wpath *__restrict__ P, bool write_clean_ops)
{
    const int n = t.x_len;
    const int start = r.end_site - n + 1;
    uint32_t ops32[26];
#pragma unroll
    for (int i = 0; i < 26; i++) ops32[i] = 0;
    bool ok = r.err == 0;
    if (!ok && start >= 0) {
        int mm = 0;
        const int win0 = t.y_start - t.k;
#pragma unroll
        for (int c = 0; c < 6; c++) {
            if (c * 64 < n) {
                uint32_t xb4[4], yb4[4], yv4[4];
                fetch64_x(store, t.x_word, t.x_start + c * 64, xb4);
                fetch64(store, t.y_word, t.y_len, t.y_rev, win0 + start + c * 64, yb4, yv4);
#pragma unroll
                for (int q = 0; q < 4; q++) {
                    const int b = c * 4 + q;
                    if (b * 16 < n) {
                        uint32_t d = mismatch_fields16(xb4[q], yb4[q], yv4[q]);
                        const int lim = min(16, n - b * 16);
                        if (lim < 16) d &= (1u << (2 * lim)) - 1u;
                        ops32[b] = d;
                        mm += __popc(d);
                    }
                }
            }
        }
        ok = (mm == r.err);
    }
    if (!ok) return false;
    int s2 = start, e2 = r.end_site;
    if (r.err > 0) {
        for (int i = n - 1; i >= 0 && ((ops32[i >> 4] >> ((i & 15) << 1)) & 3u) == 1u; i--) { ops32[i >> 4] |= 3u << ((i & 15) << 1); e2--; }
        for (int i = 0; i < n && ((ops32[i >> 4] >> ((i & 15) << 1)) & 3u) == 1u; i++) { ops32[i >> 4] |= 3u << ((i & 15) << 1); s2++; }
    }
    uint32_t tail10 = 0;
    if (r.err > 0) {
        const int a = max(n - 10, 0), wi = a >> 4, sh = (a & 15) << 1;
        const uint32_t lo = ops32[wi] >> sh, hi = (sh && wi + 1 < 26) ? ops32[wi + 1] << (32 - sh) : 0u;
        tail10 = (lo | hi) & 0xfffffu;
    }
    path_record(P, t, s2, e2, n, r.err, r.err > 0 && start == 0, tail10, r.err > 0 || write_clean_ops, [&](int wd) { return ops32[wd]; });
    return true;
}

__global__ __launch_bounds__(256) void k_path_fast(const uint32_t *__restrict__ store, const fsv_ovl *__restrict__ ovl,
                                                   const fsv_wtask *__restrict__ tasks, const fsv_wres *__restrict__ res, uint32_t n_tasks,
                                                   fsv_wpath *__restrict__ paths, PathLists L, bool write_clean_ops, const uint32_t *__restrict__ n_dev)
{
    if (n_dev) n_tasks = min(*n_dev, n_tasks);
    uint32_t blk;
    if (!xcd_block((n_tasks + 255u) >> 8, blk)) return;
    const uint32_t tid = blk * blockDim.x + threadIdx.x;
    if (tid >= n_tasks) return;
    const fsv_wtask t = tasks[tid];
    const fsv_wres r = res[tid];
    fsv_wpath *P = paths + tid;
    if (r.err < 0 || !ovl[t.ovl].is_match) { P->state = 0; return; }
    const bool ok = path_gapfree(store, t, r, P, write_clean_ops);
    if (L.cnt[7] && r.err > 0 && t.k <= FSV_K_MAX && (r.end_site == (int)t.x_len + 2 * (int)t.k - 1 || r.end_site - ((int)t.x_len - 1) <= r.err))
        L.list[7][atomicAdd(L.cnt[7], 1u)] = tid;
    {
        const int cls = ok ? -1 : (t.k <= FSV_K_MAX && r.err <= FSV_FR_MAXERR) ? r.err - 1 : t.k <= 15 ? (r.err <= FSV_SB_MAXERR ? 3 : 4) : t.k <= FSV_K_MAX ? 5 : 6;
        if (__any(cls >= 0)) {
            const int lane = (int)(threadIdx.x & 63u);
            unsigned long long mine = 0ull;
#pragma unroll
            for (int c = 0; c < 7; c++) {
                const unsigned long long m = __ballot(cls == c);
                if (cls == c) mine = m;
            }
            const int leader = mine ? __ffsll((long long)mine) - 1 : lane;
            uint32_t base = 0, *cnt = L.cnt[0], *list = L.list[0];
#pragma unroll
            for (int c = 1; c < 7; c++) { cnt = cls == c ? L.cnt[c] : cnt; list = cls == c ? L.list[c] : list; }
            if (cls >= 0 && lane == leader) base = atomicAdd(cnt, (uint32_t)__popcll(mine));
            const uint32_t at = __shfl(base, leader, 64) + (uint32_t)__popcll(mine & ((1ull << lane) - 1ull));
            if (cls >= 0) { P->state = 2; list[at] = tid; }
        }
    }
}

struct PathWalk {
    static constexpr int WORDS = 28, CAP = WORDS * 16;
    uint32_t (*ops)[64]; int lane;
    int plen, start, ci, cur, row, dir;
    uint32_t acc;
    __device__ __forceinline__ PathWalk(uint32_t (*s_ops)[64], int lane64) : ops(s_ops), lane(lane64) {}
    __device__ __forceinline__ void clear(int n, int end, int err, int row_)
    {
        for (int i = 0; i < WORDS; i++) ops[i][lane] = 0;
        plen = 0; start = end; ci = n - 1; cur = err; row = row_; dir = 0; acc = 0;
    }
    __device__ __forceinline__ void put(uint32_t code)
    {
        acc |= code << ((plen & 15) << 1);
        if ((plen & 15) == 15) { ops[plen >> 4][lane] = acc; acc = 0; }
        plen++;
        cur -= (int)(code != 0u);
        start -= (int)(code != 3u);
        row += (int)(code == 3u) - (int)(code == 2u);
        ci -= (int)(code != 2u);
        dir = (int)code;
    }
    __device__ __forceinline__ void matches(int steps)
    {
        const int np = plen + steps;
        if ((np >> 4) != (plen >> 4)) { ops[plen >> 4][lane] = acc; acc = 0; }
        plen = np; start -= steps; ci -= steps; dir = 0;
    }
    __device__ __forceinline__ void flush() { if (plen & 15) ops[plen >> 4][lane] = acc; }
    __device__ __forceinline__ uint32_t word(int wi) const { return ops[wi][lane]; }
    __device__ __forceinline__ uint32_t get(int i) const { return (ops[i >> 4][lane] >> ((i & 15) << 1)) & 3u; }
    __device__ __forceinline__ void set(int i, uint32_t v)
    {
        const int wi = i >> 4, sh = (i & 15) << 1;
        ops[wi][lane] = (ops[wi][lane] & ~(3u << sh)) | (v << sh);
    }
};

__device__ __forceinline__ void path_finish(const uint32_t *__restrict__ store, const fsv_wtask &t, fsv_wpath *__restrict__ P, PathWalk &w, int end, int err)
{
    int plen = w.plen, start = w.start, dir = w.dir;
    const int col = w.ci + 1;
    if (col > 0) { start -= col; plen += col; dir = 0; }
    if (plen > FSV_PATH_CAP) { P->state = 0; return; }
    if (dir != 3) start++;
    const bool raw0 = err > 0 && start == 0;
    if (err > 0) {
        int stop = -1;
        for (int i = 0; i < plen && w.get(i) == 1; i++) { w.set(i, 3); end--; stop = i; }
        for (int i = plen - 1; i >= 0 && w.get(i) == 1; i--) { w.set(i, 3); start++; }
        int xi = 0, yi = 0;
        BaseCache xc, yc;
        for (int i = plen - 1; i > stop;) {
            const int f = i & 15;
            const uint32_t wv = w.word(i >> 4);
            const uint32_t m = wv & 0xAAAAAAAAu & (f == 15 ? 0xffffffffu : ((1u << (2 * f + 2)) - 1u));
            const int skip = min(m == 0u ? f + 1 : f - ((31 - __clz(m)) >> 1), i - stop);
            if (skip > 0) { xi += skip; yi += skip; i -= skip; continue; }
            const uint32_t op = (wv >> (2 * f)) & 3u;
            int pi = i + 1, x2 = xi, y2 = yi;
            if (op == 3) y2--; else x2--;
            for (; pi < plen && x2 >= 0 && y2 >= 0; pi++, x2--, y2--) {
                const uint32_t pv = w.get(pi);
                const bool same = xc.get(store, t.x_word, t.x_start + x2) == yc.ycol(store, t, start + y2);
                if (pv >= 2 || (pv == 0 && !same)) break;
                if (pv == 1 && same) { w.set(pi - 1, 0); err--; }
                else w.set(pi - 1, pv);
                w.set(pi, op);
            }
            if (op == 2) yi++; else xi++;
            i--;
        }
    }
    auto packed = [&](int wd) -> uint32_t {
        const int a = plen - 16 - 16 * wd;
        uint32_t v = 0;
        if (a >= 0) {
            const int wi = a >> 4, sh = (a & 15) << 1;
            const uint32_t w0 = w.word(wi), w1 = (sh && wi + 1 < PathWalk::WORDS) ? w.word(wi + 1) : 0u;
            v = sh ? (w0 >> sh) | (w1 << (32 - sh)) : w0;
        } else if (a > -16) v = w.word(0) << ((-a) << 1);
        return rev_fields2(v);
    };
    path_record(P, t, start, end, plen, err, raw0, w.word(0) & 0xfffffu, true, packed);
}

template <class WordT, int LANES> struct PathSink {
    WordT *cols; uint32_t lane;
    __device__ __forceinline__ WordT &at(int c, int w) const { return cols[((size_t)c * 3 + w) * LANES + lane]; }
    __device__ __forceinline__ void operator()(int i, uint64_t d0, uint64_t vp, uint64_t vn) const
    {
        at(i + 1, 0) = (WordT)d0; at(i + 1, 1) = (WordT)vp; at(i + 1, 2) = (WordT)vn;
    }
};

template <class WordT, int LANES>
__device__ __forceinline__ void path_general(const uint32_t *__restrict__ store, const fsv_wtask &t, fsv_wpath *__restrict__ P, uint32_t (*s_ops)[64],
                                             int lane64, WordT *cols_slice)
{
    const int n = t.x_len, k = t.k, band = 2 * k + 1;
    fsv_wres r;
    const PathSink<WordT, LANES> sink{cols_slice, LANES == 1 ? 0u : (uint32_t)lane64};
    bpm_run(store, t, r, sink);
    if (r.err < 0) { P->state = 0; return; }
    PathWalk w(s_ops, lane64);
    w.clear(n, r.end_site, r.err, band - (n + 2 * k - r.end_site));
    WordT vp = sink.at(n, 1), vn = sink.at(n, 2);
    while (w.ci >= 0 && w.cur != 0) {
        const int row = w.row, cur = w.cur;
        const WordT d0 = sink.at(w.ci + 1, 0);
        const WordT vpi = w.ci > 0 ? sink.at(w.ci, 1) : (WordT)0, vni = w.ci > 0 ? sink.at(w.ci, 2) : (WordT)0;
        const WordT hn = vpi & d0, hp = vni | ~(vpi | d0);
        const int diag = cur - (int)((~(d0 >> row)) & 1u);
        const bool can_up = row != 0, can_left = row == 0 || row != band - 1;
        int left = cur, up = cur;
        if (can_left) left = cur - (int)((hp >> row) & 1u) + (int)((hn >> row) & 1u);
        if (can_up) up = cur - (int)((vp >> (row - 1)) & 1u) + (int)((vn >> (row - 1)) & 1u);
        int best = diag;
        uint32_t code = diag != cur ? 1u : 0u;
        if (can_up && up < best) { best = up; code = 2u; }
        if (can_left && left < best) code = 3u;
        if (code != 2u) { vp = vpi; vn = vni; }
        w.put(code);
    }
    w.flush();
    path_finish(store, t, P, w, r.end_site, r.err);
}

template <class WordT>
__global__ __launch_bounds__(64) void k_path_dp(const uint32_t *__restrict__ store, const fsv_wtask *__restrict__ tasks,
                                                const uint32_t *__restrict__ dp_list, const uint32_t *__restrict__ n_dev,
                                                fsv_wpath *__restrict__ paths, WordT *__restrict__ cols)
{
    __shared__ uint32_t s_ops[PathWalk::WORDS][64];
    const int lane64 = threadIdx.x;
    const uint32_t n_list = *n_dev;
    for (uint32_t li = blockIdx.x * 64 + threadIdx.x; li < n_list; li += gridDim.x * 64) {
        const uint32_t tid = dp_list[li];
        const fsv_wtask t = tasks[tid];
        path_general<WordT, 64>(store, t, paths + tid, s_ops, lane64, cols + (size_t)blockIdx.x * (FSV_WINDOW + 2) * 3 * 64);
    }
}

__device__ __forceinline__ void fix_boundary_dev(const uint32_t *__restrict__ store, fsv_wtask &t, fsv_wres &r, fsv_wpath *__restrict__ P, uint32_t (*s_ops)[64],
                                                 uint64_t *cols, int k_cap)
{
    const uint4 h = *reinterpret_cast<const uint4 *>(P);
    if ((h.w & 0xffu) != 1u || r.err <= 0 || t.k > FSV_K_MAX || (r.extra_begin & 0x4000)) return;
    const int n = t.x_len, k = t.k, wlen = n + 2 * k;
    const bool raw0 = ((h.w >> 16) & 4u) != 0u;
    fsv_wtask t2 = t;
// ... 655 lines not shown
```

focalsv_amd/csrc/fsv_internal.h:

```cpp
#pragma once
#include <hip/hip_runtime.h>
#include <stdint.h>
#include <chrono>
#include <cstdio>
#include <cstdlib>
#include <new>
#include <stdexcept>
#include <string>
#include <vector>
#include "focalsv_hip.h"

struct fsv_ctx {
    int device = -1;
    hipStream_t stream = nullptr;
    bool own_stream = false;
    int n_cu = 0;
    int clock_khz = 0;
    uint64_t hbm_bytes = 0;
    std::string name;
    std::string last_error;
    void *asm_ws = nullptr;
    void (*asm_ws_free)(fsv_ctx *) = nullptr;
    const char *last_contigs_dev = nullptr;
    std::vector<uint64_t> last_contig_off;
// ... 13 lines not shown
static inline int fsv_fail(fsv_ctx *ctx, int code, const char *msg)
{
    if (ctx) ctx->last_error = msg;
    return code;
}

__device__ __forceinline__ uint32_t fsv_base_fwd(const uint32_t *__restrict__ store, uint32_t word_off, int pos)
{
    return (store[word_off + ((uint32_t)pos >> 4)] >> (((uint32_t)pos & 15u) << 1)) & 3u;
}

__device__ __forceinline__ uint32_t fsv_base_at(const uint32_t *__restrict__ store, uint32_t word_off, int len, int rev, int p)
{
    int q = rev ? (len - 1 - p) : p;
    uint32_t b = fsv_base_fwd(store, word_off, q);
    return rev ? (3u - b) : b;
}

__device__ __forceinline__ int wave_max_i32(int v)
{
    const int lowest = -2147483647 - 1;
    v = max(v, __builtin_amdgcn_update_dpp(lowest, v, 0xB1, 0xF, 0xF, false));
    v = max(v, __builtin_amdgcn_update_dpp(lowest, v, 0x4E, 0xF, 0xF, false));
    v = max(v, __builtin_amdgcn_update_dpp(lowest, v, 0x141, 0xF, 0xF, false));
    v = max(v, __builtin_amdgcn_update_dpp(lowest, v, 0x140, 0xF, 0xF, false));
    const int a = __builtin_amdgcn_readlane(v, 0), b = __builtin_amdgcn_readlane(v, 16);
    const int c = __builtin_amdgcn_readlane(v, 32), d = __builtin_amdgcn_readlane(v, 48);
    return max(max(a, b), max(c, d));
}
__device__ __forceinline__ long long wave_max_i64(long long v)
{
    for (int off = 32; off > 0; off >>= 1) { long long o = __shfl_xor(v, off, 64); v = o > v ? o : v; }
    return v;
}

__device__ __forceinline__ uint32_t block_waves_before_256(uint32_t wave_total, uint32_t *s_w, uint32_t *total)
{
    const uint32_t wv = threadIdx.x >> 6;
    if ((threadIdx.x & 63u) == 63u) s_w[wv] = wave_total;
    __syncthreads();
    uint32_t before = 0, all = 0;
#pragma unroll
    for (uint32_t v = 0; v < 4; v++) { const uint32_t c = s_w[v]; if (v < wv) before += c; all += c; }
    *total = all;
    return before;
}
__device__ __forceinline__ uint32_t block_offset_256(uint32_t cnt, uint32_t *s_w, uint32_t *total)
{
    const uint32_t lane = threadIdx.x & 63u;
    uint32_t incl = cnt;
    for (uint32_t off = 1; off < 64; off <<= 1) { const uint32_t o = __shfl_up(incl, off, 64); if (lane >= off) incl += o; }
    return block_waves_before_256(incl, s_w, total) + incl - cnt;
}
__device__ __forceinline__ uint32_t block_rank_256(bool keep, uint32_t *s_w, uint32_t *total)
{
    const uint64_t bal = __ballot(keep);
    return block_waves_before_256((uint32_t)__popcll(bal), s_w, total) + (uint32_t)__popcll(bal & ((1ull << (threadIdx.x & 63u)) - 1ull));
}

#define FSV_KMER_EMPTY (~0ull)
struct KmerSet {
    uint64_t base, size;
    __device__ __forceinline__ uint64_t start(uint64_t h) const { return (h ^ (h >> 29)) & (size - 1); }
    __device__ __forceinline__ bool has(const unsigned long long *__restrict__ keys, uint64_t h) const
    {
        uint64_t slot = start(h);
        for (uint64_t probe = 0; probe < size; probe++) {
            const unsigned long long cur = keys[base + slot];
            if (cur == h) return true;
            if (cur == FSV_KMER_EMPTY) return false;
            slot = (slot + 1) & (size - 1);
        }
        return false;
    }
    __device__ __forceinline__ uint64_t claim(unsigned long long *keys, uint64_t h) const
    {
        uint64_t slot = start(h);
        for (uint64_t probe = 0; probe < size; probe++) {
            unsigned long long cur = keys[base + slot];
            if (cur == FSV_KMER_EMPTY) { cur = atomicCAS(&keys[base + slot], FSV_KMER_EMPTY, h); if (cur == FSV_KMER_EMPTY) cur = h; }
            if (cur == h) return slot;
            slot = (slot + 1) & (size - 1);
        }
        return size;
    }
};

int fsv_live_contexts(int device);

#define FSV_GUARD(ctx, call)                                                            \
    try { return (call); }                                                              \
    catch (const std::bad_alloc &) { return fsv_fail(ctx, FSV_ENOMEM, "out of host memory"); } \
    catch (const std::exception &e) { if (ctx) (ctx)->last_error = std::string("exception: ") + e.what(); return FSV_EINTERNAL; } \
    catch (...) { return fsv_fail(ctx, FSV_EINTERNAL, "unknown exception"); }

static inline unsigned fsv_grid_for(uint64_t n, unsigned block) { return (unsigned)((n + block - 1) / block); }

#define TRY(x) do { int rc_ = (x); if (rc_ != FSV_OK) return rc_; } while (0)

template <class T> struct Dev {
    T *p = nullptr;
    size_t cap = 0;
    Dev() = default;
    Dev(const Dev &) = delete;
    Dev &operator=(const Dev &) = delete;
    ~Dev() { if (p) (void)hipFree(p); }
    void swap(Dev &o) { T *tp = p; p = o.p; o.p = tp; const size_t tc = cap; cap = o.cap; o.cap = tc; }
};

template <class T> int ensure(fsv_ctx *ctx, Dev<T> &b, size_t n)
{
    const size_t bytes = n * sizeof(T);
    if (bytes <= b.cap && b.p) return FSV_OK;
    if (b.p) { FSV_HIP(ctx, hipStreamSynchronize(ctx->stream)); FSV_HIP(ctx, hipFree(b.p)); b.p = nullptr; b.cap = 0; }
    const size_t want = bytes + bytes / 8 + 256;
    FSV_HIP(ctx, hipMalloc((void **)&b.p, want));
    b.cap = want;
    return FSV_OK;
}

template <class T> int upload(fsv_ctx *ctx, Dev<T> &b, const std::vector<T> &v)
{
    TRY(ensure(ctx, b, v.empty() ? 1 : v.size()));
    if (!v.empty()) FSV_HIP(ctx, hipMemcpyAsync(b.p, v.data(), v.size() * sizeof(T), hipMemcpyHostToDevice, ctx->stream));
    return FSV_OK;
}

template <class T> int zero(fsv_ctx *ctx, Dev<T> &b, size_t n) { FSV_HIP(ctx, hipMemsetAsync(b.p, 0, n * sizeof(T), ctx->stream)); return FSV_OK; }
template <class T> int download(fsv_ctx *ctx, T *host, const Dev<T> &b, size_t n) { FSV_HIP(ctx, hipMemcpyAsync(host, b.p, n * sizeof(T), hipMemcpyDeviceToHost, ctx->stream)); return FSV_OK; }
template <class... Ts> int ensure_each(fsv_ctx *ctx, size_t n, Dev<Ts> &...b) { int rc = FSV_OK; (void)(((rc = ensure(ctx, b, n)) == FSV_OK) && ...); return rc; }

#define FSV_LAUNCH(ctx, stream, kern, grid, block, lds, ...) \
    do { hipLaunchKernelGGL(kern, grid, block, lds, stream, __VA_ARGS__); FSV_HIP(ctx, hipGetLastError()); } while (0)

struct Timer {
    std::chrono::steady_clock::time_point t0; fsv_ctx *ctx;
    explicit Timer(fsv_ctx *c) : ctx(c) { (void)hipStreamSynchronize(c->stream); t0 = std::chrono::steady_clock::now(); }
    double stop() { (void)hipStreamSynchronize(ctx->stream); return std::chrono::duration<double, std::milli>(std::chrono::steady_clock::now() - t0).count(); }
};
struct Trace {
    fsv_ctx *ctx = nullptr; const char *who = ""; std::chrono::steady_clock::time_point t0 = std::chrono::steady_clock::now();
    void operator()(const char *what)
    {
        if (!getenv("FSV_TRACE")) return;
        (void)hipStreamSynchronize(ctx->stream);
        const auto t = std::chrono::steady_clock::now();
        fprintf(stderr, "[fsv] %s %-14s %.2f ms\n", who, what, std::chrono::duration<double, std::milli>(t - t0).count());
        t0 = t;
    }
};

int fsv_bpm_windows_dev_n(fsv_ctx *ctx, const uint32_t *store_dev, const fsv_wtask *tasks_dev, uint32_t n_tasks, const uint32_t *n_dev,
                          fsv_wres *res_dev, int k_cap);
```

focalsv_amd/csrc/k5_bpm.hip:

```cpp
#include "bpm_device.h"
#include <algorithm>

namespace {

__global__ __launch_bounds__(256) void k5_bpm_kernel(const uint32_t *__restrict__ store, const fsv_wtask *__restrict__ tasks,
                                                     uint32_t n_tasks, fsv_wres *__restrict__ res, const uint32_t *__restrict__ n_dev)
{
    if (n_dev) n_tasks = min(*n_dev, n_tasks);
    uint32_t blk;
    if (!xcd_block((n_tasks + 255u) >> 8, blk)) return;
    const uint32_t tid = blk * blockDim.x + threadIdx.x;
    if (tid >= n_tasks) return;
    const fsv_wtask t = tasks[tid];
    fsv_wres r;
    bool exact = bpm_window_geometry(t, r);
    if (exact) {
        const int n = t.x_len;
        uint32_t acc = 0;
#pragma unroll
        for (int c = 0; c < (FSV_WINDOW + 63) / 64; c++) {
            if (c * 64 < n) {
                uint32_t xb[4], yb[4], yv[4];
                fetch64_x(store, t.x_word, t.x_start + c * 64, xb);
                fetch64(store, t.y_word, t.y_len, t.y_rev, t.y_start + c * 64, yb, yv);
#pragma unroll
                for (int j = 0; j < 4; j++) {
                    const int i = c * 64 + j * 16;
                    if (i < n) {
                        const int lim = min(16, n - i);
                        const uint32_t fm = lim < 16 ? (1u << (2 * lim)) - 1u : 0xffffffffu, vm = (1u << lim) - 1u;
                        acc |= ((xb[j] ^ yb[j]) & fm) | ((yv[j] & vm) ^ vm);
                    }
                }
            }
        }
        exact = acc == 0u;
        if (exact) { r.end_site = n - 1 + t.k; r.err = 0; }
    }
    if (!exact) {
        if (t.k <= 15) { BpmNoSink32 none; bpm_run32(store, t, r, none); }
        else bpm_run(store, t, r, BpmNoSink());
    }
    res[tid] = r;
}

__global__ __launch_bounds__(256) void k5_bpm_wide_kernel(const uint32_t *__restrict__ store, const fsv_wtask *__restrict__ tasks,
                                                          uint32_t n_tasks, fsv_wres *__restrict__ res, const uint32_t *__restrict__ n_dev, int k_cap)
{
    uint32_t tid = blockIdx.x * blockDim.x + threadIdx.x;
    if (n_dev) n_tasks = min(*n_dev, n_tasks);
    if (tid >= n_tasks) return;
    const fsv_wtask t = tasks[tid];
    fsv_wres r;
    WideNoSink none;
    bpm_run_wide(store, t, r, none, k_cap);
    res[tid] = r;
}

}

extern "C" int fsv_bpm_windows_dev(fsv_ctx *ctx, const uint32_t *store_dev, const fsv_wtask *tasks_dev, uint32_t n_tasks,
                                   fsv_wres *res_dev)
{
    return fsv_bpm_windows_dev_n(ctx, store_dev, tasks_dev, n_tasks, nullptr, res_dev, FSV_K_MAX);
}

int fsv_bpm_windows_dev_n(fsv_ctx *ctx, const uint32_t *store_dev, const fsv_wtask *tasks_dev, uint32_t n_tasks, const uint32_t *n_dev,
                          fsv_wres *res_dev, int k_cap)
{
    if (!ctx || !store_dev || (!tasks_dev && n_tasks) || (!res_dev && n_tasks)) return FSV_EINVAL;
    if (n_tasks == 0) return FSV_OK;
    if (k_cap > FSV_K_WIDE) return fsv_fail(ctx, FSV_EUNSUP, "window thresholds above 95 (bands above 191 rows) are not built");
    FSV_HIP(ctx, hipSetDevice(ctx->device));
    if (k_cap > FSV_K_MAX)
        FSV_LAUNCH(ctx, ctx->stream, k5_bpm_wide_kernel, dim3(fsv_grid_for(n_tasks, 256)), dim3(256), 0, store_dev, tasks_dev, n_tasks, res_dev, n_dev, k_cap);
    else
    FSV_LAUNCH(ctx, ctx->stream, k5_bpm_kernel, dim3((fsv_grid_for(n_tasks, 256) + 7u) & ~7u), dim3(256), 0, store_dev, tasks_dev, n_tasks, res_dev, n_dev);
    return FSV_OK;
}

extern "C" int fsv_bpm_windows(fsv_ctx *ctx, const uint32_t *store, size_t store_words, const fsv_wtask *tasks,
                               uint32_t n_tasks, fsv_wres *res)
{
    if (!ctx || !store || (!tasks && n_tasks) || (!res && n_tasks)) return FSV_EINVAL;
    int kmax = 0;
    for (uint32_t i = 0; i < n_tasks; i++) {
        if (tasks[i].k > FSV_K_WIDE || tasks[i].x_len == 0 || tasks[i].x_len > FSV_WINDOW) return fsv_fail(ctx, FSV_EINVAL, "task k/x_len out of range");
        kmax = std::max<int>(kmax, tasks[i].k);
    }
    const int k_cap = kmax > FSV_K_MAX ? kmax : FSV_K_MAX;
    void *d_store = nullptr, *d_tasks = nullptr, *d_res = nullptr;
    int rc = FSV_OK;
    FSV_HIP(ctx, hipSetDevice(ctx->device));
    if (hipMalloc(&d_store, store_words * 4 + 16) != hipSuccess || hipMalloc(&d_tasks, (size_t)n_tasks * sizeof(fsv_wtask) + 16) != hipSuccess ||
        hipMalloc(&d_res, (size_t)n_tasks * sizeof(fsv_wres) + 16) != hipSuccess) {
        rc = fsv_fail(ctx, FSV_ENOMEM, "hipMalloc failed");
    }
    if (rc == FSV_OK) rc = fsv_h2d(ctx, d_store, store, store_words * 4);
    if (rc == FSV_OK) rc = fsv_h2d(ctx, d_tasks, tasks, (size_t)n_tasks * sizeof(fsv_wtask));
    if (rc == FSV_OK) rc = fsv_bpm_windows_dev_n(ctx, (const uint32_t *)d_store, (const fsv_wtask *)d_tasks, n_tasks, nullptr, (fsv_wres *)d_res, k_cap);
    if (rc == FSV_OK) rc = fsv_d2h(ctx, res, d_res, (size_t)n_tasks * sizeof(fsv_wres));
    (void)hipFree(d_store); (void)hipFree(d_tasks); (void)hipFree(d_res);
    return rc;
}
```

focalsv_amd/csrc/k_consensus.h:

```cpp
#pragma once

namespace {

struct ConsArgs {
    const uint32_t *store;
    const uint32_t *word_off;
    const int32_t *read_len;
    const uint32_t *read_set;
    const uint32_t *set_start;
    const uint32_t *pair_base;
    const uint32_t *gwin_off;
    const uint32_t *gwin_read;
    const uint4 *ovl_c;
    const uint4 *gwin_tab;
    const fsv_wtask *tasks;
    const fsv_wpath *paths;
    uint8_t *cwin;
    uint16_t *cwin_len;
    uint32_t *warn;
    uint32_t *changed;
    uint32_t n_reads;
    const uint32_t *read_dirty;
    uint8_t *cov3;
    int junction_vote;
    int ins_dag;
};

__device__ __forceinline__ bool vote_wins(int cnt, int total, bool homo)
{
    if (cnt * 5 >= total * 3) return true;
    return homo && cnt * 1000 >= total * 515;
}

__global__ __launch_bounds__(64) void k_read_dirty(const uint4 *__restrict__ ovl_c, const fsv_wpath *__restrict__ paths, const uint32_t *__restrict__ read_set,
                                                   const uint32_t *__restrict__ set_start, const uint32_t *__restrict__ pair_base, uint32_t n_reads,
                                                   uint32_t *__restrict__ read_dirty)
{
    const uint32_t r = blockIdx.x;
    if (r >= n_reads) return;
    const uint32_t s = read_set[r], r0 = set_start[s], ns = set_start[s + 1] - r0;
    const uint32_t pbase = pair_base[s] + (r - r0) * (ns - 1), n_ovl = ns - 1;
    bool dirty = false;
    for (uint32_t oi = threadIdx.x; oi < n_ovl; oi += 64) {
        const uint4 oc = ovl_c[pbase + oi];
        if (!(oc.z >> 31)) continue;
        const int n_win = (int)(oc.z & 0x7fffffffu);
        int prev_end = 0; bool prev_ok = false;
        for (int j = 0; j < n_win && !dirty; j++) {
            const uint4 h0 = *reinterpret_cast<const uint4 *>(paths + (oc.y + (uint32_t)j));
            const bool ok = (h0.w & 0xffu) == 1u;
            if (ok) {
                if ((int16_t)(h0.z >> 16) != 0) dirty = true;
                if (prev_ok && (int)h0.x - prev_end - 1 != 0) dirty = true;
                prev_end = (int)h0.y;
            }
            prev_ok = ok;
        }
    }
    const bool any = __ballot(dirty) != 0ull;
    if (threadIdx.x == 0) read_dirty[r] = any ? 1u : 0u;
}

__global__ void k_gwin_tab(const uint32_t *__restrict__ gwin_read, const uint32_t *__restrict__ gwin_off, const uint32_t *__restrict__ read_set,
                           const uint32_t *__restrict__ set_start, const uint32_t *__restrict__ pair_base, uint32_t n_gwin, uint4 *__restrict__ tab)
{
    const uint32_t gw = blockIdx.x * blockDim.x + threadIdx.x;
    if (gw >= n_gwin) return;
    const uint32_t r = gwin_read[gw], s = read_set[r], r0 = set_start[s], ns = set_start[s + 1] - r0;
    tab[gw] = make_uint4(r, pair_base[s] + (r - r0) * (ns - 1), ns - 1, gw - gwin_off[r]);
}

#define FSV_SITE_MARK 0xffffffffu
#define FSV_DG_N 64
#define FSV_DG_E 128
#define FSV_DG_A 8
#define FSV_DG_D 8
#define FSV_DG_K 64
struct DagLds {
    uint32_t keys[FSV_DG_K];
    uint16_t e_w[FSV_DG_E];
    uint8_t e_from[FSV_DG_E], e_to[FSV_DG_E], e_alive[FSV_DG_E], e_vis[FSV_DG_E];
    uint8_t base[FSV_DG_N], alive[FSV_DG_N], out_n[FSV_DG_N], in_n[FSV_DG_N];
    uint8_t out_e[FSV_DG_N][FSV_DG_A], in_e[FSV_DG_N][FSV_DG_A];
    uint8_t queue[4 * FSV_DG_E];
    uint8_t stk_node[16], stk_bi[16], stk_cons[16];
    int n_node, n_edge, ok;
};

__device__ __forceinline__ int dg_node(DagLds &D, uint8_t b)
{
    const int id = D.n_node;
    if (id >= FSV_DG_N) { D.ok = 0; return FSV_DG_N - 1; }
    D.base[id] = b; D.alive[id] = 1; D.out_n[id] = 0; D.in_n[id] = 0; D.n_node = id + 1;
    return id;
}
__device__ __forceinline__ void dg_edge(DagLds &D, int u, int v, int w, int vis)
{
    const int e = D.n_edge;
    if (e >= FSV_DG_E || D.out_n[u] >= FSV_DG_A || D.in_n[v] >= FSV_DG_A) { D.ok = 0; return; }
    D.e_from[e] = (uint8_t)u; D.e_to[e] = (uint8_t)v; D.e_w[e] = (uint16_t)w; D.e_alive[e] = 1; D.e_vis[e] = (uint8_t)vis; D.n_edge = e + 1;
    D.out_e[u][D.out_n[u]++] = (uint8_t)e; D.in_e[v][D.in_n[v]++] = (uint8_t)e;
}
__device__ __forceinline__ int dg_find(const DagLds &D, int u, int v)
{
    for (int i = 0; i < D.in_n[v]; i++) { const int e = D.in_e[v][i]; if (D.e_alive[e] && D.e_from[e] == u) return e; }
    return -1;
}
__device__ __forceinline__ int dg_outdeg(const DagLds &D, int u) { int c = 0; for (int i = 0; i < D.out_n[u]; i++) c += D.e_alive[D.out_e[u][i]]; return c; }
__device__ __forceinline__ int dg_indeg(const DagLds &D, int u) { int c = 0; for (int i = 0; i < D.in_n[u]; i++) c += D.e_alive[D.in_e[u][i]]; return c; }
__device__ __forceinline__ void dg_delete(DagLds &D, int x)
{
    D.alive[x] = 0; D.base[x] = 'D';
    for (int i = 0; i < D.out_n[x]; i++) D.e_alive[D.out_e[x][i]] = 0;
    for (int i = 0; i < D.in_n[x]; i++) D.e_alive[D.in_e[x][i]] = 0;
    D.out_n[x] = 0; D.in_n[x] = 0;
}
template <bool OUT>
__device__ __forceinline__ void dg_merge(DagLds &D, int start)
{
    int sp = 0;
    D.stk_node[0] = (uint8_t)start; D.stk_bi[0] = 0;
    if (!D.alive[start] || (OUT ? dg_outdeg(D, start) : dg_indeg(D, start)) == 0) return;
    while (sp >= 0 && D.ok) {
        const int cur = D.stk_node[sp], bi = D.stk_bi[sp];
        if (bi >= 4) { sp--; continue; }
        D.stk_bi[sp] = (uint8_t)(bi + 1);
        const uint8_t want = (uint8_t)("ACGT"[bi]);
        int flag = 0, weight = 0, cons = -1;
        const int nl = OUT ? D.out_n[cur] : D.in_n[cur];
        for (int i = 0; i < nl; i++) {
            const int e = OUT ? D.out_e[cur][i] : D.in_e[cur][i];
            if (!D.e_alive[e]) continue;
            const int g = OUT ? D.e_to[e] : D.e_from[e];
            if (D.base[g] != want || (OUT ? dg_indeg(D, g) : dg_outdeg(D, g)) != 1) continue;
            if (flag == 0) { flag = 1; cons = g; D.e_vis[e] = 1; weight = D.e_w[e]; }
            else {
                flag++;
                weight += D.e_w[e];
                const int ng = OUT ? D.out_n[g] : D.in_n[g];
                for (int j = 0; j < ng; j++) {
                    const int e2 = OUT ? D.out_e[g][j] : D.in_e[g][j];
                    if (!D.e_alive[e2]) continue;
                    const int o = OUT ? D.e_to[e2] : D.e_from[e2];
                    const int e3 = OUT ? dg_find(D, cons, o) : dg_find(D, o, cons);
                    if (e3 >= 0) { D.e_vis[e3] = 1; D.e_w[e3] = (uint16_t)(D.e_w[e3] + D.e_w[e2]); }
                    else if (OUT) dg_edge(D, cons, o, D.e_w[e2], 1);
                    else dg_edge(D, o, cons, D.e_w[e2], 1);
                }
                dg_delete(D, g);
            }
        }
        if (flag > 1) { const int e = OUT ? dg_find(D, cur, cons) : dg_find(D, cons, cur); if (e >= 0) D.e_w[e] = (uint16_t)weight; }
        if (flag > 0 && D.alive[cons] && (OUT ? dg_outdeg(D, cons) : dg_indeg(D, cons)) != 0) {
            if (sp + 1 >= 16) { D.ok = 0; return; }
            sp++;
            D.stk_node[sp] = (uint8_t)cons; D.stk_bi[sp] = 0;
        }
    }
}
__device__ __forceinline__ int dg_weight(const DagLds &D, int u, bool in)
{
    int w = 0;
    if (in) { for (int i = 0; i < D.in_n[u]; i++) if (D.e_alive[D.in_e[u][i]]) w += D.e_w[D.in_e[u][i]]; }
    else for (int i = 0; i < D.out_n[u]; i++) if (D.e_alive[D.out_e[u][i]]) w += D.e_w[D.out_e[u][i]];
    return w;
}
__device__ __forceinline__ int dag_insertion(DagLds &D, int nk, uint32_t &out_key)
{
    out_key = 0;
    if (nk > FSV_DG_K) return -1;
    for (int z = 1; z < nk; z++) { const uint32_t kv = D.keys[z]; int z2 = z; for (; z2 > 0 && D.keys[z2 - 1] > kv; z2--) D.keys[z2] = D.keys[z2 - 1]; D.keys[z2] = kv; }
    uint32_t distinct[FSV_DG_D]; int cnt[FSV_DG_D], nd = 0;
    for (int i = 0; i < nk; i++) {
        if (nd && distinct[nd - 1] == D.keys[i]) { cnt[nd - 1]++; continue; }
        if (nd == FSV_DG_D) return -1;
        distinct[nd] = D.keys[i]; cnt[nd] = 1; nd++;
    }
    if (nd == 1) { out_key = distinct[0]; return cnt[0]; }
    D.n_node = 0; D.n_edge = 0; D.ok = 1;
    const int S = dg_node(D, 'S'), E = dg_node(D, 'E');
    for (int i = 0; i < nd; i++) {
        const int len = (int)(distinct[i] >> 24);
        int last = S;
        for (int j = 0; j < len; j++) { const int nn = dg_node(D, (uint8_t)("ACGT"[(distinct[i] >> (2 * j)) & 3u])); dg_edge(D, last, nn, cnt[i], 0); last = nn; }
        if (last != S) dg_edge(D, last, E, cnt[i], 0);
    }
    int qh = 0, qt = 0;
    D.queue[qt++] = (uint8_t)S;
    while (qh < qt && D.ok) {
        const int cur = D.queue[qh++];
        dg_merge<false>(D, cur);
        dg_merge<true>(D, cur);
        if (!D.alive[cur]) continue;
        for (int i = 0; i < D.out_n[cur]; i++) if (D.e_alive[D.out_e[cur][i]]) D.e_vis[D.out_e[cur][i]] = 1;
        for (int i = 0; i < D.out_n[cur]; i++) {
            const int e = D.out_e[cur][i];
            if (!D.e_alive[e]) continue;
            const int o = D.e_to[e];
            bool all = true;
            for (int j = 0; j < D.in_n[o]; j++) if (D.e_alive[D.in_e[o][j]] && !D.e_vis[D.in_e[o][j]]) { all = false; break; }
            if (all) { if (qt < 4 * FSV_DG_E) D.queue[qt++] = (uint8_t)o; else D.ok = 0; }
        }
    }
    if (!D.ok) return -1;
    int best_s = -1, best_e = -1, ws = 0, we = 0;
    for (int i = 0; i < D.out_n[S]; i++) { const int e = D.out_e[S][i]; if (D.e_alive[e]) { const int o = D.e_to[e], w = o == E ? dg_weight(D, E, true) : dg_weight(D, o, false); if (w > ws) { ws = w; best_s = o; } } }
    for (int i = 0; i < D.in_n[E]; i++) { const int e = D.in_e[E][i]; if (D.e_alive[e]) { const int o = D.e_from[e], w = dg_weight(D, o, false); if (w > we) { we = w; best_e = o; } } }
    uint32_t seq = 0; int L = 0;
    if (ws >= we) {
// ... 314 lines not shown
                    np++;
                }
            }
            n2 += L; p += L;
            continue;
        }
        const bool after_ins = pend && p > 0;
        if (pend) { atomicAdd(&S.cnt[xp][2], 1u << 16); pend = false; }
        if (op == 3u) { atomicAdd(&S.cnt[xp][2], 1u); n3++; }
        else if (op == 1u) {
            const bool flagged = after_ins || fmm_pos == p;
            const uint32_t e = (uint32_t)xp | ((uint32_t)(p - n3) << 9) | (flagged ? 1u << 23 : 0u);
            if (np == 0) ent[0] = e; else if (np == 1) ent[1] = e; else if (np == 2) ent[2] = e; else ent[3] = e;
            np++;
            if (flagged) fmm_pos = p + 1;
        } else if (after_ins) fstart = xp;
        p++;
    }
    if (fstart >= 0) { atomicAdd(&S.cov[fstart], 65536); atomicAdd(&S.cov[xs + plen - n2], -65536); }
    if (np) cons_flush<EVC>(S, store, y_word, y_len, y_rev, ry_start, ent, np);
    return n2;
}

struct SiteLists {
    uint32_t *site_cnt;
    uint32_t *win_list;
    uint32_t *redo_list;
    uint32_t *win_n;
    const int32_t *bc_win;
};
template <int EVC, int MODE>
__device__ __forceinline__ void consensus_window(const ConsArgs &A, const uint32_t gw, const SiteLists &L)
{
    __shared__ Tally<EVC> S;
    __shared__ uint32_t s_anydev;
    const int lane = threadIdx.x;
    const uint4 gt = A.gwin_tab[gw];
    const uint32_t r = gt.x, pbase = gt.y, n_ovl = gt.z;
    const int g = (int)gt.w;
    const int xlen = A.read_len[r];
    const int gs = g * FSV_WINDOW, glen = min(FSV_WINDOW, xlen - gs);
    S.stage_backbone(lane, A.store + A.word_off[r], gs, xlen);
    uint8_t *dst = A.cwin + (size_t)gw * FSV_CW_STRIDE;
    if (A.read_dirty && !A.read_dirty[r]) {
        __syncthreads();
        for (int c = lane; c < glen; c += 64) dst[c] = (uint8_t)S.xb(gs, gs + c);
        if (lane == 0) { A.cwin_len[gw] = (uint16_t)glen; if (MODE == 1) L.site_cnt[gw] = 0u; }
        return;
    }
    S.reset(lane);
    if (lane == 0) s_anydev = 0;
    __syncthreads();
    for (uint32_t oi = lane; oi < n_ovl; oi += 64) {
        const uint4 oc = A.ovl_c[pbase + oi];
        const int o_x_s = (int)oc.x, o_n_win = (int)(oc.z & 0x7fffffffu);
        const int j = g - o_x_s / FSV_WINDOW;
        if (!(oc.z >> 31) || j < 0 || j >= o_n_win) continue;
        const uint32_t ti = oc.y + (uint32_t)j;
        const fsv_wpath *P = A.paths + ti;
        const uint4 h0 = *reinterpret_cast<const uint4 *>(P);
        const uint2 h1 = *reinterpret_cast<const uint2 *>((const uint8_t *)P + 16);
        uint2 pv[13];
        load_path_ops(P, pv);
        atomicAdd(&S.cover, 1u);
        if ((h0.w & 0xffu) != 1u) continue;
        const bool clean_path = (int16_t)(h0.z >> 16) == 0;
        const uint32_t nz = clean_path ? 0u : S.stage_path(lane, pv);
        const int ry_start = (int)h0.x, plen = (int)(int16_t)(h0.z & 0xffffu);
        const uint32_t y_word = h1.x; const int y_len = (int)h1.y, y_rev = (int)((h0.w >> 8) & 0xffu);
        const int xs = max(gs, o_x_s) - gs;
        bool pend = false;
        if (j > 0 && A.junction_vote) {
            const uint4 hp = *reinterpret_cast<const uint4 *>(A.paths + ti - 1);
            if ((hp.w & 0xffu) == 1u) {
                const int gap = ry_start - (int)hp.y - 1;
                if (gap > 0 && xs == 0) {
                    pend = true;
                    if (gap <= FSV_INS_MAXLEN) {
                        uint32_t key = (uint32_t)gap << 24;
                        for (int b = 0; b < gap; b++) key |= fsv_base_at(A.store, y_word, y_len, y_rev, ry_start - gap + b) << (2 * b);
                        S.add_event(0, key);
                    }
                }
            }
        }
        if (pend || nz) s_anydev = 1u;
        int n2 = 0;
        if (clean_path) { if (pend) S.cnt_add(xs, 5u); }
        else n2 = cons_walk<EVC>(S, S.path[lane], nz, plen, xs, glen, pend, A.store, y_word, y_len, y_rev, ry_start);
        atomicAdd(&S.cov[xs], 1);
        atomicAdd(&S.cov[xs + plen - n2], -1);
    }
    __syncthreads();
    const bool verbatim = S.cover < 3u || s_anydev == 0u;
    if (A.cov3 && lane == 0) A.cov3[gw] = S.cover >= 3u ? 1 : 0;
    if (S.evn > (uint32_t)EVC && lane == 0) atomicOr(&A.warn[r], (uint32_t)FSV_W_INS_EVENTS);
    const int bc_lo = (MODE == 1 && L.bc_win) ? L.bc_win[3 * (size_t)gw + 1] : 1, bc_hi = (MODE == 1 && L.bc_win) ? L.bc_win[3 * (size_t)gw + 2] : 0;
    bool site = false;
    int c0, c1;
    lane_columns(lane, glen, c0, c1);
    const bool differs = S.decide_columns(lane, c0, c1, gs, glen, xlen, verbatim, A.ins_dag, [&](int c, int arrived, bool) {
        if (MODE != 1) return;
        int oa[4], alt;
#pragma unroll
        for (int b = 0; b < 4; b++) oa[b] = (int)S.cnt_get(c, (uint32_t)b);
        if (oa[0] + oa[1] + oa[2] + oa[3] > 1 && c >= bc_lo && c <= bc_hi) site = true;
        if (split_sub_site(oa, (int)S.cnt_get(c, 4u), arrived, alt)) site = true;
    });
    if (differs && A.changed) A.changed[r] = 1u;
    if (MODE == 1) {
        const bool any_site = __ballot(site) != 0ull || (L.bc_win && L.bc_win[3 * (size_t)gw]);
        if (lane == 0) {
            L.site_cnt[gw] = any_site ? FSV_SITE_MARK : 0u;
            if (any_site) L.win_list[atomicAdd(&L.win_n[0], 1u)] = gw;
        }
    }
    uint8_t (*s_out)[14] = S.out();
    uint32_t mine = 0;
    for (int c = c0; c < c1; c++) mine += s_out[c][0];
    const int incl = wave_incl_sum((int)mine, lane);
    uint32_t off = (uint32_t)incl - mine;
    const uint32_t tot = (uint32_t)__shfl(incl, 63, 64);
    if (tot > FSV_CW_STRIDE) {
        for (int c = lane; c < glen; c += 64) dst[c] = (uint8_t)S.xb(gs, gs + c);
        if (lane == 0) { A.cwin_len[gw] = (uint16_t)glen; atomicOr(&A.warn[r], (uint32_t)FSV_W_WINDOW_KEPT); }
        return;
    }
    for (int c = c0; c < c1; c++) for (int b = 0; b < s_out[c][0]; b++) dst[off++] = s_out[c][1 + b];
    if (lane == 0) A.cwin_len[gw] = (uint16_t)tot;
}

template <int EVC, int MODE>
__global__ __launch_bounds__(64) void k_consensus(ConsArgs A, uint32_t n_gwin, SiteLists L)
{
    uint32_t gw;
    if (xcd_block(n_gwin, gw)) consensus_window<EVC, MODE>(A, gw, L);
}

template <int EVC>
__global__ __launch_bounds__(64) void k_consensus_redo(ConsArgs A, SiteLists L)
{
    const uint32_t n = L.win_n[1];
    for (uint32_t i = blockIdx.x; i < n; i += gridDim.x) {
        consensus_window<EVC, 0>(A, L.redo_list[i], L);
        __syncthreads();
    }
}

#define FSV_BC_SIDE 100
#define FSV_BC_USELESS 50
#define FSV_BC_SCAN 10
struct BcigArgs {
    const fsv_wtask *tasks; const fsv_wpath *paths; const uint32_t *n_tasks;
    const uint32_t *pair_read, *read_dirty, *gwin_off; const uint8_t *thr_tab; int k_cap;
    fsv_wtask *tasks2; int32_t *bc_idx; uint32_t *n_tasks2;
    const fsv_wres *res2; const fsv_wpath *paths2; uint4 *bc_rec; int32_t *bc_win;
    uint32_t *n_same, *n_used;
};
struct OpReader {
    const uint32_t *w; uint32_t cur = 0; int idx = -1;
    __device__ __forceinline__ OpReader(const fsv_wpath *P) : w(reinterpret_cast<const uint32_t *>(P->ops)) {}
    __device__ __forceinline__ uint32_t get(int i) { const int wi = i >> 4; if (wi != idx) { cur = w[wi]; idx = wi; } return (cur >> ((i & 15) << 1)) & 3u; }
};
__device__ __forceinline__ int scan_ops(const fsv_wpath *P, int plen, int err0, int scan_x, int dir)
{
    if (err0 == 0) return 0;
    OpReader R(P);
    int x_i = 0, err = 0;
    for (int p = 0; p < plen; p++) {
        const uint32_t op = R.get(dir ? plen - 1 - p : p);
        if (op == 2u) { err++; continue; }
        if (op != 0u) err++;
        if (++x_i >= scan_x) return err;
    }
    return err;
}
__device__ __forceinline__ int scan_ops_interval(const fsv_wpath *P, int plen, int err0, int xb, int xe)
{
    if (err0 == 0) return 0;
    OpReader R(P);
    int x_i = 0, err = 0;
    for (int p = 0; p < plen; p++) {
        const uint32_t op = R.get(p);
        if (op == 2u) { err++; continue; }
        if (x_i == xb) err = 0;
        x_i++;
        if (op != 0u) err++;
        if (x_i == xe + 1) return err;
    }
    return err;
}

__global__ void k_bcwin_init(int32_t *__restrict__ bc_win, uint32_t n_gwin)
{
    const uint32_t gw = blockIdx.x * blockDim.x + threadIdx.x;
    if (gw < n_gwin) { bc_win[3 * (size_t)gw] = 0; bc_win[3 * (size_t)gw + 1] = 0x7fffffff; bc_win[3 * (size_t)gw + 2] = -1; }
}

__global__ __launch_bounds__(256) void k_bcig_tasks(BcigArgs A)
{
    const uint32_t n_tasks = min(*A.n_tasks, gridDim.x * blockDim.x);
    uint32_t blk;
    if (!xcd_block((n_tasks + 255u) >> 8, blk)) return;
    const uint32_t ti = blk * blockDim.x + threadIdx.x;
    if (ti >= n_tasks) return;
    A.bc_idx[ti] = -1;
    if (ti + 1 >= n_tasks) return;
    const fsv_wtask t0 = A.tasks[ti];
    if (!A.read_dirty[A.pair_read[t0.ovl]]) return;
    const uint4 h0 = *reinterpret_cast<const uint4 *>(A.paths + ti), h1 = *reinterpret_cast<const uint4 *>(A.paths + ti + 1);
    if ((h0.w & 0xffu) != 1u || (h1.w & 0xffu) != 1u) return;
    const int y_distance = (int)h1.x - (int)h0.y - 1;
    if (y_distance == 0 && !((h0.w >> 16) & 2u) && !((h1.w >> 16) & 1u)) return;
    const fsv_wtask t1 = A.tasks[ti + 1];
    if (t1.ovl != t0.ovl) return;
    int y_start = (int)h0.y, x_start = t0.x_start + (int)t0.x_len - 1;
    const int leftLen = min(min(x_start - t0.x_start, y_start), FSV_BC_SIDE);
    const int rightLen = min(min(t1.x_start + (int)t1.x_len - x_start, t0.y_len - y_start), FSV_BC_SIDE);
    const int xLen = leftLen + rightLen;
    if (xLen <= 0) return;
    x_start -= leftLen; y_start -= leftLen;
    const int thr = double_thr(A.thr_tab[xLen], xLen, A.k_cap);
    if (thr > FSV_K_MAX) return;
    const uint32_t slot = atomicAdd(A.n_tasks2, 1u);
    fsv_wtask w;
    w.x_word = t0.x_word; w.y_word = t0.y_word; w.x_start = x_start; w.y_start = y_start; w.y_len = t0.y_len;
    w.x_len = (uint16_t)xLen; w.k = (uint8_t)thr; w.y_rev = t0.y_rev; w.ovl = t0.ovl; w.win = ti;
    A.tasks2[slot] = w;
    A.bc_idx[ti] = (int32_t)slot;
}

__global__ __launch_bounds__(256) void k_bcig_accept(BcigArgs A)
{
    const uint32_t slot = blockIdx.x * blockDim.x + threadIdx.x;
    if (slot >= *A.n_tasks2) return;
    A.bc_rec[slot] = make_uint4(0, 0, 0, 0);
    const fsv_wtask w = A.tasks2[slot];
    const fsv_wres r = A.res2[slot];
    const uint32_t ti = w.win;
    const fsv_wpath *PB = A.paths2 + slot, *P0 = A.paths + ti, *P1 = A.paths + ti + 1;
    const uint4 hb = *reinterpret_cast<const uint4 *>(PB);
    if (r.err < 0 || (hb.w & 0xffu) != 1u) return;
    const int xLen = w.x_len, thr = w.k;
    if (xLen + 2 * thr - r.extra_begin - r.extra_end < xLen) return;
    const fsv_wtask t0 = A.tasks[ti], t1 = A.tasks[ti + 1];
    const uint4 h0 = *reinterpret_cast<const uint4 *>(P0), h1 = *reinterpret_cast<const uint4 *>(P1);
    const int x_end0 = t0.x_start + (int)t0.x_len - 1, leftLen = x_end0 - w.x_start, rightLen = xLen - leftLen;
    int y_distance = (int)h1.x - (int)h0.y - 1;
    if (y_distance < 0) y_distance = -y_distance;
    int L = FSV_BC_USELESS, R = FSV_BC_USELESS;
    const uint32_t first_ti = ti - t0.win;
    if (t0.win == 0 && w.x_start == t0.x_start) L = 0;
    {
        const bool last_junction = ti + 2 >= *A.n_tasks || A.tasks[ti + 2].ovl != t0.ovl;
        if (last_junction && w.x_start + xLen - 1 == t1.x_start + (int)t1.x_len - 1) R = 0;
    }
    (void)first_ti;
    if (leftLen <= L || rightLen <= R) return;
    const int plb = (int)(int16_t)(hb.z & 0xffffu), eb = (int)(int16_t)(hb.z >> 16);
    const int pl0 = (int)(int16_t)(h0.z & 0xffffu), e0 = (int)(int16_t)(h0.z >> 16), pl1 = (int)(int16_t)(h1.z & 0xffffu), e1 = (int)(int16_t)(h1.z >> 16);
    const int m_err = scan_ops_interval(PB, plb, eb, L, xLen - R - 1);
    const int b_err = scan_ops(P0, pl0, e0, leftLen - L, 1), f_err = scan_ops(P1, pl1, e1, rightLen - R, 0);
    if (f_err + b_err + y_distance + 1 < m_err) return;
    bool differs = false, mm0 = false, mm1 = false;
    int lo0 = 0x7fffffff, hi0d = -1, lo1 = 0x7fffffff, hi1d = -1;
    {
        OpReader RB(PB), R0(P0), R1(P1);
        int pb = 0, xb = 0, yb = (int)hb.x;
        const int x0c = (w.x_start + L) - t0.x_start;
        int p0 = 0, x0 = 0, y0 = (int)h0.x;
        if (e0 != 0) { while (p0 < pl0 && x0 < x0c) { const uint32_t op = R0.get(p0++); if (op == 2u) y0++; else { x0++; if (op != 3u) y0++; } } }
        else { x0 = x0c; y0 += x0c; p0 = x0c; }
        if (eb != 0) { while (pb < plb && xb < L) { const uint32_t op = RB.get(pb++); if (op == 2u) yb++; else { xb++; if (op != 3u) yb++; } } }
        else { xb = L; yb += L; pb = L; }
        auto next = [](OpReader &Rd, int &p, int pl, int e, int &y, uint32_t &op_out, int &y_out) {
            if (e == 0) { op_out = 0u; y_out = y; y++; p++; return; }
            while (p < pl) { const uint32_t op = Rd.get(p++); if (op == 2u) { y++; continue; } op_out = op; y_out = y; if (op != 3u) y++; return; }
            op_out = 0u; y_out = y;
        };
        const int hi0 = leftLen;
        for (; xb <= hi0; xb++) {
            uint32_t ob, ow; int ybp, ywp;
            next(RB, pb, plb, eb, yb, ob, ybp);
            next(R0, p0, pl0, e0, y0, ow, ywp);
            if (ob != ow || (ob != 3u && ybp != ywp)) { if (lo0 > xb) lo0 = xb; hi0d = xb; }
            if (ob == 1u || ow == 1u) mm0 = true;
        }
        int p1 = 0, y1 = (int)h1.x;
        const int hi1 = leftLen + (rightLen - 1 - R);
        for (; xb <= hi1; xb++) {
            uint32_t ob, ow; int ybp, ywp;
            next(RB, pb, plb, eb, yb, ob, ybp);
            next(R1, p1, pl1, e1, y1, ow, ywp);
            if (ob != ow || (ob != 3u && ybp != ywp)) { if (lo1 > xb) lo1 = xb; hi1d = xb; }
            if (ob == 1u || ow == 1u) mm1 = true;
        }
        differs = lo0 <= hi0d || lo1 <= hi1d;
    }
    if (!differs) { atomicAdd(A.n_same, 1u); return; }
    atomicAdd(A.n_used, 1u);
    A.bc_rec[slot] = make_uint4(1u, (uint32_t)w.x_start, (uint32_t)xLen | ((uint32_t)L << 16) | ((uint32_t)R << 24), 0u);
    const uint32_t rd = A.pair_read[t0.ovl], g0 = A.gwin_off[rd] + (uint32_t)(t0.x_start / FSV_WINDOW);
    const int gs0 = (t0.x_start / FSV_WINDOW) * FSV_WINDOW;
    if (lo0 <= hi0d) {
        if (mm0) A.bc_win[3 * (size_t)g0] = 1;
        atomicMin(&A.bc_win[3 * (size_t)g0 + 1], w.x_start + lo0 - gs0); atomicMax(&A.bc_win[3 * (size_t)g0 + 2], w.x_start + hi0d - gs0);
    }
    if (lo1 <= hi1d) {
        if (mm1) A.bc_win[3 * (size_t)(g0 + 1)] = 1;
        atomicMin(&A.bc_win[3 * (size_t)(g0 + 1) + 1], w.x_start + lo1 - gs0 - FSV_WINDOW); atomicMax(&A.bc_win[3 * (size_t)(g0 + 1) + 2], w.x_start + hi1d - gs0 - FSV_WINDOW);
    }
}

#define FSV_SITE_WIN_CAP 255
#define FSV_SITE_RAW_CAP 1024
#define FSV_SITE_READ_CAP 512
#define FSV_K7_GROUP_CAP 10000
struct SiteArgs {
    uint32_t *site_cnt;
    uint2 *site_rec;
    uint32_t *site_off;
    uint32_t *rec_cursor; uint32_t rec_cap;
    int8_t *vec;
    uint32_t *vec_cursor;
    uint32_t vec_cap;
    uint32_t *read_sites;
    const int32_t *bc_idx;
    const uint4 *bc_rec;
    const fsv_wpath *bc_paths;
};

__device__ __forceinline__ void snp_sites_window(const ConsArgs &A, const uint32_t gw, const SiteArgs &S)
{
    __shared__ TallyCols T;
    __shared__ uint8_t s_alt[FSV_WINDOW + 1];
    __shared__ uint8_t s_sidx[FSV_WINDOW + 1];
    __shared__ uint32_t s_nsite, s_vbase, s_rbase;
    __shared__ uint32_t s_scan[64];
    const int lane = threadIdx.x;
    const uint4 gt = A.gwin_tab[gw];
    const uint32_t r = gt.x, pbase = gt.y, n_ovl = gt.z;
    const int g = (int)gt.w;
    const int xlen = A.read_len[r];
    const int gs = g * FSV_WINDOW, glen = min(FSV_WINDOW, xlen - gs);
    if (lane == 0) S.site_cnt[gw] = 0;
    T.stage_backbone(lane, A.store + A.word_off[r], gs, xlen);
    T.reset(lane);
    for (int i = lane; i < FSV_WINDOW + 1; i += 64) s_alt[i] = 0;
    if (lane == 0) s_nsite = 0;
    __syncthreads();
    const uint32_t vstride = (n_ovl + 3u) & ~3u;
    for (int pass = 0; pass < 2; pass++) {
        for (uint32_t oi = lane; oi < n_ovl; oi += 64) {
            const uint4 oc = A.ovl_c[pbase + oi];
            const int o_x_s = (int)oc.x, o_n_win = (int)(oc.z & 0x7fffffffu);
            const int j = g - o_x_s / FSV_WINDOW;
            if (!(oc.z >> 31) || j < 0 || j >= o_n_win) continue;
            const uint32_t ti = oc.y + (uint32_t)j;
            const fsv_wpath *P = A.paths + ti;
            const uint4 h0 = *reinterpret_cast<const uint4 *>(P);
            if ((h0.w & 0xffu) != 1u) continue;
            const int xs = max(gs, o_x_s) - gs;
            if (pass == 0) atomicAdd(&T.cover, 1u);
            auto walk = [&](const fsv_wpath *Q, int x0, int lo, int hi) -> int {
                const uint4 q0 = *reinterpret_cast<const uint4 *>(Q);
                const int plen = (int)(int16_t)(q0.z & 0xffffu), ry0 = (int)q0.x, col0 = x0 - gs;
                if ((int16_t)(q0.z >> 16) == 0) {
                    if (pass == 1) for (int xi = max(lo, -col0); xi <= min(hi, plen - 1) && col0 + xi < glen; xi++) if (s_alt[col0 + xi]) S.vec[s_vbase + (uint32_t)s_sidx[col0 + xi] * vstride + oi] = 0;
                    return plen;
                }
                const uint2 q1 = *reinterpret_cast<const uint2 *>((const uint8_t *)Q + 16);
                const uint32_t y_word = q1.x; const int y_len = (int)q1.y, y_rev = (int)((q0.w >> 8) & 0xffu);
                uint2 pv[13];
                load_path_ops(Q, pv);
                T.stage_path(lane, pv);
                int n2 = 0, n3 = 0;
                for (int p = 0; p < plen; p++) {
                    const uint32_t rest = T.path[lane][p >> 4] >> ((p & 15) << 1);
                    if (pass == 0 && rest == 0u) { p = (((p >> 4) + 1) << 4) - 1; continue; }
                    const uint32_t op = rest & 3u;
                    if (op == 2u) { n2++; continue; }
                    const int xi = p - n2, c = col0 + xi;
                    if (xi >= lo && xi <= hi && c >= 0 && c < glen) {
                        if (pass == 0) {
                            if (op == 3u) T.cnt_add(c, 4u);
                            else if (op == 1u) T.cnt_add(c, fsv_base_at(A.store, y_word, y_len, y_rev, ry0 + p - n3));
                        } else {
                            const uint32_t alt = s_alt[c];
                            if (alt) {
                                int8_t v = 0;
                                if (op == 3u) v = 2;
                                else if (op == 1u) v = fsv_base_at(A.store, y_word, y_len, y_rev, ry0 + p - n3) + 1u == alt ? 1 : 2;
                                S.vec[s_vbase + (uint32_t)s_sidx[c] * vstride + oi] = v;
                            }
                        }
                    }
                    if (op == 3u) n3++;
                }
                return plen - n2;
            };
            int cur_beg = 0, cur_end = 0x7fffffff;
            if (S.bc_idx) {
                const int32_t sb = j >= 1 ? S.bc_idx[ti - 1] : -1, se = j + 1 < o_n_win ? S.bc_idx[ti] : -1;
                const uint4 rb = sb >= 0 ? S.bc_rec[sb] : make_uint4(0, 0, 0, 0), re = se >= 0 ? S.bc_rec[se] : make_uint4(0, 0, 0, 0);
                if ((rb.x | re.x) & 1u) {
                    const fsv_wtask t = A.tasks[ti];
                    const int x_total_start = t.x_start, x_length = t.x_len, x_total_end = x_total_start + x_length - 1;
                    if (rb.x & 1u) {
                        const int bx = (int)rb.y, blen = (int)(rb.z & 0xffffu), bL = (int)((rb.z >> 16) & 0xffu), bR = (int)(rb.z >> 24);
                        const int xleft = x_total_start - bx, xright = bx + blen - 1 - x_total_start + 1;
                        if (xleft > bL && xright > bR) { cur_beg = xright - bR; walk(S.bc_paths + sb, bx, xleft, xleft + (xright - bR) - 1); }
                    }
                    if (re.x & 1u) {
                        const int bx = (int)re.y, blen = (int)(re.z & 0xffffu), bL = (int)((re.z >> 16) & 0xffu), bR = (int)(re.z >> 24);
                        const int xleft = x_total_end - bx, xright = bx + blen - 1 - x_total_end + 1;
                        if (xleft > bL && xright > bR) { cur_end = (x_length - 1) - ((xleft + 1) - bL); walk(S.bc_paths + se, bx, bL, xleft); }
                    }
                }
            }
            const int xcols = walk(P, gs + xs, cur_beg, cur_end);
            if (pass == 0) {
                atomicAdd(&T.cov[xs], 1);
                atomicAdd(&T.cov[xs + xcols], -1);
            }
        }
        __syncthreads();
        if (pass == 1 || T.cover == 0u) break;
        int c0, c1, run = 0;
        lane_columns(lane, glen, c0, c1);
        for (int c = c0; c < c1; c++) run += T.cov[c];
        s_scan[lane] = (uint32_t)run;
        __syncthreads();
        int arrived = 0, mine = 0;
        for (int i = 0; i < lane; i++) arrived += (int)s_scan[i];
        for (int c = c0; c < c1; c++) {
            arrived += T.cov[c];
            int oa[4], alt;
#pragma unroll
            for (int b = 0; b < 4; b++) oa[b] = (int)T.cnt_get(c, (uint32_t)b);
            if (!split_sub_site(oa, (int)T.cnt_get(c, 4u), arrived, alt)) continue;
            s_alt[c] = (uint8_t)(alt + 1);
            mine++;
        }
        s_scan[lane] = (uint32_t)mine;
        __syncthreads();
        int first = 0, all = 0;
        for (int i = 0; i < 64; i++) { if (i < lane) first += (int)s_scan[i]; all += (int)s_scan[i]; }
        if (all == 0) break;
        if (all > FSV_SITE_WIN_CAP) { if (lane == 0) atomicOr(&A.warn[r], (uint32_t)FSV_W_SITES); break; }
        if (lane == 0) {
            const uint32_t off = atomicAdd(S.vec_cursor, (uint32_t)all * vstride), roff = atomicAdd(S.rec_cursor, (uint32_t)all);
            s_vbase = off; s_rbase = roff;
            s_nsite = (off + (uint32_t)all * vstride <= S.vec_cap && roff + (uint32_t)all <= S.rec_cap) ? (uint32_t)all : 0u;
            if (!s_nsite) atomicOr(&A.warn[r], (uint32_t)FSV_W_SITES);
        }
        __syncthreads();
        if (!s_nsite) break;
        for (uint32_t i = lane; i < (uint32_t)all * vstride; i += 64) S.vec[s_vbase + i] = -1;
        for (int c = c0, k = first; c < c1; c++) {
            if (!s_alt[c]) continue;
            s_sidx[c] = (uint8_t)k;
            const int p = gs + c;
            const bool homo = homo_strict([&](int pp) { return T.xb(gs, pp); }, p, xlen);
            S.site_rec[(size_t)s_rbase + k] = make_uint2((uint32_t)p | (homo ? 0x80000000u : 0u), s_vbase + (uint32_t)k * vstride);
// ... 33 lines not shown
    const uint4 gt = A.gwin_tab[g0];
    const uint32_t pbase = gt.y, n_ovl = gt.z;
    if (lane == 0) s_n = 0;
    __syncthreads();
    for (uint32_t gb = g0; gb < g1; gb += 64) {
        const uint32_t gw = gb + lane;
        const uint32_t c = gw < g1 ? S.site_cnt[gw] : 0u;
        uint32_t incl = c;
        for (int d = 1; d < 64; d <<= 1) { const uint32_t v = __shfl_up(incl, d); if (lane >= d) incl += v; }
        const uint32_t base = s_n + incl - c;
        for (uint32_t k = 0; k < c; k++)
            if (base + k < FSV_SITE_RAW_CAP) { const uint2 rec = S.site_rec[(size_t)S.site_off[gw] + k]; s_pos[base + k] = (int32_t)rec.x; s_voff[base + k] = rec.y; }
        __syncthreads();
        if (lane == 63) s_n = base + c;
        __syncthreads();
    }
    int nS = (int)s_n;
    if (nS == 0) return;
    if (nS > FSV_SITE_RAW_CAP) { if (lane == 0) atomicOr(&A.warn[r], (uint32_t)FSV_W_SITES); return; }
    if (nS > 1) {
        for (int j = lane; j < nS; j += 64) {
            const int p = s_pos[j] & 0x7fffffff;
            const bool left = j > 0 && p == (s_pos[j - 1] & 0x7fffffff) + 1, right = j + 1 < nS && p + 1 == (s_pos[j + 1] & 0x7fffffff);
            s_keep[j] = !(left || right);
        }
        __syncthreads();
        if (lane == 0) {
            int m = 0;
            for (int j = 0; j < nS; j++) if (s_keep[j]) { s_pos[m] = s_pos[j]; s_voff[m] = s_voff[j]; m++; }
            s_n = (uint32_t)m;
        }
        __syncthreads();
        nS = (int)s_n;
        if (nS == 0) return;
    }
    if (nS > FSV_SITE_READ_CAP) { if (lane == 0) atomicOr(&A.warn[r], (uint32_t)FSV_W_SITES); return; }
    for (uint32_t i = lane; i < n_ovl; i += 64) {
        if (!(ovl_c[pbase + i].z >> 31)) continue;
        int st = -1;
        for (int j = 0; j < nS; j++) {
            const int8_t v = S.vec[s_voff[j] + i];
            const bool inf = v == 0 || v == 1;
            if (st == -1) { if (inf) st = 0; }
            else if (st == 0) { if (!inf) st = 2; }
            else if (inf) { st = 3; break; }
        }
        if (st == 3) {
            for (int j = 0; j < nS; j++) S.vec[s_voff[j] + i] = 2;
            ovl[pbase + i].is_match = 4;
            ovl_c[pbase + i].z &= 0x7fffffffu;
            s_redo = 1u;
        }
    }
    __threadfence_block();
    __syncthreads();
    for (int i = 0; i < nS; i++) {
        if (lane < FSV_SITE_READ_CAP / 32) s_bt[i][lane] = 0;
        int best = 1;
        for (int j = 0; j < i; j++) {
            bool bad = false;
            for (uint32_t o = lane; o < n_ovl; o += 64) {
                const int8_t a = S.vec[s_voff[i] + o], b = S.vec[s_voff[j] + o];
                if (a != b && (a == 0 || a == 1) && (b == 0 || b == 1)) bad = true;
            }
            if (__ballot(bad)) continue;
            const int cand = (int)s_max[j] + 1;
            if (cand > best) {
                best = cand;
                if (lane < FSV_SITE_READ_CAP / 32) s_bt[i][lane] = 0;
            }
            if (cand == best && lane == 0) s_bt[i][j >> 5] |= 1u << (j & 31);
            __syncthreads();
        }
        if (lane == 0) { s_max[i] = (uint16_t)best; s_visit[i] = 0; }
        __syncthreads();
    }
    for (int i = lane; i < nS; i += 64) {
        int rank = 0;
        for (int j = 0; j < nS; j++) rank += (s_max[j] > s_max[i]) || (s_max[j] == s_max[i] && j < i);
        s_order[rank] = (uint16_t)i;
    }
    __syncthreads();
    uint32_t n_groups = 0;
    for (int oi = 0; oi < nS; oi++) {
        const int root = s_order[oi];
        if (s_visit[root]) continue;
        int depth = 0;
        if (lane == 0) { s_buf[0] = (uint16_t)root; s_cur[0] = 0; s_visit[root] = 1; }
        __syncthreads();
        while (depth >= 0) {
            const int id = s_buf[depth];
            bool leaf = true;
            for (int w = 0; w < FSV_SITE_READ_CAP / 32; w++) if (s_bt[id][w]) leaf = false;
            if (leaf) {
                if (n_groups <= FSV_K7_GROUP_CAP) {
                    const int plen = depth + 1;
                    int occ0 = 0, occ1 = 0;
                    for (uint32_t ob = 0; ob < n_ovl; ob += 64) {
                        const uint32_t o = ob + lane;
                        int8_t rv = -1;
                        if (o < n_ovl) for (int k = 0; k < plen && rv == -1; k++) { const int8_t v = S.vec[s_voff[s_buf[k]] + o]; if (v == 0 || v == 1) rv = v; }
                        occ0 += __popcll(__ballot(rv == 0));
                        occ1 += __popcll(__ballot(rv == 1));
                    }
                    bool useful = false;
                    if (occ0 && occ1) {
                        const double low = (double)(occ0 + occ1) * 0.3;
                        if ((double)occ1 >= low && (double)occ0 >= low) useful = true;
                        else if (occ1 >= 5 && occ0 >= 5) useful = true;
                        else if (occ1 >= 3 && occ0 >= 3 && plen >= 2) {
                            int far = 0;
                            for (int k = 0; k < plen; k++) {
                                const int cur = s_pos[s_buf[k]] & 0x7fffffff;
                                bool nearby = false;
                                if (k > 0 && (s_pos[s_buf[k - 1]] & 0x7fffffff) - cur < 10) nearby = true;
                                if (k + 1 < plen && cur - (s_pos[s_buf[k + 1]] & 0x7fffffff) < 10) nearby = true;
                                if (!nearby) far++;
                            }
                            useful = far > 0;
                        }
                    }
                    if (useful)
                        for (uint32_t o = lane; o < n_ovl; o += 64) {
                            int8_t rv = -1;
                            for (int k = 0; k < plen && rv == -1; k++) { const int8_t v = S.vec[s_voff[s_buf[k]] + o]; if (v == 0 || v == 1) rv = v; }
                            if (rv == 1 && (ovl_c[pbase + o].z >> 31)) { ovl[pbase + o].is_match = 2; ovl_c[pbase + o].z &= 0x7fffffffu; s_redo = 1u; }
                        }
                    n_groups++;
                }
                depth--;
                continue;
            }
            int nxt = -1;
            for (int j = s_cur[depth]; j < id; j++) if (s_bt[id][j >> 5] >> (j & 31) & 1u) { nxt = j; break; }
            __syncthreads();
            if (nxt < 0 || n_groups > FSV_K7_GROUP_CAP) { depth--; continue; }
            if (lane == 0) { s_cur[depth] = (uint16_t)(nxt + 1); s_buf[depth + 1] = (uint16_t)nxt; s_cur[depth + 1] = 0; s_visit[nxt] = 1; }
            __syncthreads();
            depth++;
        }
        __syncthreads();
    }
    if (s_redo) {
        uint32_t base = lane == 0 ? atomicAdd(&L.win_n[1], g1 - g0) : 0u;
        base = __shfl(base, 0);
        for (uint32_t i = lane; i < g1 - g0; i += 64) L.redo_list[base + i] = g0 + i;
    }
}

#define FSV_BND_HALF 187
#define FSV_BND_SIDE 25
struct BndArgs {
    const fsv_wtask *tasks; const fsv_wpath *paths; const uint32_t *n_tasks;
    const uint4 *ovl_c; const uint32_t *pair_base, *set_start; uint32_t n_sets; const uint32_t *pair_read;
    const uint32_t *gwin_off, *lb; const uint16_t *cwin_len; const uint8_t *cov3; const uint32_t *read_dirty;
    const uint32_t *brel_off; uint32_t b_base;
    const uint8_t *thr_tab;
    fsv_wtask *tasks2; int32_t *idx2; uint32_t *n_tasks2;
    uint32_t *bnd_flag, *bnd_list, *n_bnd;
    const uint32_t *store2;
};

__global__ __launch_bounds__(256) void k_bnd_tasks(BndArgs A)
{
    const uint32_t n_tasks = min(*A.n_tasks, gridDim.x * blockDim.x);
    uint32_t blk;
    if (!xcd_block((n_tasks + 255u) >> 8, blk)) return;
    const uint32_t ti = blk * blockDim.x + threadIdx.x;
    if (ti >= n_tasks) return;
    A.idx2[ti] = -1;
    const fsv_wtask t = A.tasks[ti];
    if (t.x_start % FSV_WINDOW != 0 || t.x_start == 0) return;
    const uint32_t p = t.ovl;
    const uint32_t r = A.pair_read[p];
    const uint4 oc = A.ovl_c[p];
    const uint4 h0 = *reinterpret_cast<const uint4 *>(A.paths + ti);
    const uint32_t dirty = A.read_dirty[r], gwo = A.gwin_off[r];
    if (!(dirty && (oc.z >> 31) && (h0.w & 0xffu) == 1u)) return;
    const uint32_t gw = gwo + (uint32_t)(t.x_start / FSV_WINDOW);
    const uint32_t cov = A.cov3[gw], cwl = A.cwin_len[gw];
    const int LB = (int)A.lb[gw];
    if (!cov || LB == 0) return;
    const int len_now = LB + (int)cwl;
    const int cws = max(0, LB - FSV_BND_HALF), cwe = min(len_now - 1, LB + FSV_BND_HALF - 1), blen = cwe - cws + 1;
    const int y_start = (int)h0.x - FSV_BND_HALF;
    if (y_start < 0 || blen < 1) return;
    const uint32_t xw2 = A.b_base + A.brel_off[r];
    if (y_start + blen <= t.y_len) {
        uint32_t acc = 0;
#pragma unroll
        for (int c = 0; c < 6; c++) {
            if (c * 64 < blen) {
                uint32_t xb[4], yb[4], yv[4];
                fetch64_x(A.store2, xw2, cws + c * 64, xb);
                fetch64(A.store2, t.y_word, t.y_len, t.y_rev, y_start + c * 64, yb, yv);
#pragma unroll
                for (int j = 0; j < 4; j++) {
                    const int b = c * 64 + j * 16;
                    if (b < blen) {
                        const int lim = min(16, blen - b);
                        acc |= (xb[j] ^ yb[j]) & (lim < 16 ? (1u << (2 * lim)) - 1u : 0xffffffffu);
                    }
                }
            }
        }
        const bool same = acc == 0u;
        if (same) { A.idx2[ti] = -2; atomicAdd(&A.bnd_flag[gw], 2u); return; }
    }
    const uint32_t slot = atomicAdd(A.n_tasks2, 1u);
    fsv_wtask w;
    w.x_word = xw2; w.y_word = t.y_word; w.x_start = cws; w.y_start = y_start; w.y_len = t.y_len;
    w.x_len = (uint16_t)blen; w.k = A.thr_tab[blen]; w.y_rev = t.y_rev; w.ovl = p; w.win = ti;
    A.tasks2[slot] = w;
    A.idx2[ti] = (int32_t)slot;
    if (!(atomicOr(&A.bnd_flag[gw], 1u) & 1u)) A.bnd_list[atomicAdd(A.n_bnd, 1u)] = gw;
}

__global__ __launch_bounds__(256) void k_bnd_retry(fsv_wtask *__restrict__ tasks2, const fsv_wres *__restrict__ res2, const uint32_t *__restrict__ n_tasks2,
                                                   fsv_wtask *__restrict__ tasks3, uint32_t *__restrict__ src3, uint32_t *__restrict__ n3, int k_cap)
{
    const uint32_t i = blockIdx.x * blockDim.x + threadIdx.x;
    if (i >= *n_tasks2 || res2[i].err >= 0) return;
    fsv_wtask t = tasks2[i];
    t.k = (uint8_t)double_thr(t.k, t.x_len, k_cap);
    tasks2[i].k = t.k;
    const uint32_t j = atomicAdd(n3, 1u);
    tasks3[j] = t; src3[j] = i;
}

__global__ __launch_bounds__(256) void k_bnd_scatter(fsv_wres *__restrict__ res2, const fsv_wres *__restrict__ res3, const uint32_t *__restrict__ src3,
                                                     const uint32_t *__restrict__ n3)
{
    const uint32_t j = blockIdx.x * blockDim.x + threadIdx.x;
    if (j < *n3) res2[src3[j]] = res3[j];
}

struct BndPatch { uint16_t ts, told, tnew, hs, hold, hnew, valid, pad; };

template <int EVC>
__global__ __launch_bounds__(64) void k_bnd_consensus(ConsArgs A, BndArgs B, const fsv_wpath *__restrict__ paths2, const uint32_t *__restrict__ store2,
                                                      BndPatch *__restrict__ patch, uint8_t *__restrict__ patch_bytes)
{
    static_assert(2 * FSV_BND_HALF + 1 <= FSV_WINDOW, "a junction's backbone fits the tally of a window");
    struct Lds : Tally<EVC> {
        uint32_t terr;
        uint16_t off[FSV_WINDOW + 2];
        uint8_t own[FSV_WINDOW + 1];
    };
    __shared__ Lds S;
    const int lane = threadIdx.x;
    const uint32_t n_list = *B.n_bnd;
    for (uint32_t li = blockIdx.x; li < n_list; li += gridDim.x) {
        __syncthreads();
        const uint32_t gw = B.bnd_list[li];
        const uint4 gt = A.gwin_tab[gw];
        const uint32_t r = gt.x, pbase = gt.y, n_ovl = gt.z;
        const int g = (int)gt.w;
        const int gs = g * FSV_WINDOW;
        const int LB = (int)B.lb[gw], len_now = LB + (int)B.cwin_len[gw];
        const int cws = max(0, LB - FSV_BND_HALF), cwe = min(len_now - 1, LB + FSV_BND_HALF - 1), blen = cwe - cws + 1;
        if (lane == 0) { patch[gw].valid = 0; S.terr = 0; }
        S.stage_backbone(lane, store2 + B.b_base + B.brel_off[r], cws, len_now);
        S.reset(lane);
        __syncthreads();
        for (uint32_t oi = lane; oi < n_ovl; oi += 64) {
            const uint4 oc = A.ovl_c[pbase + oi];
            const int o_x_s = (int)oc.x, o_n_win = (int)(oc.z & 0x7fffffffu);
            const int j = g - o_x_s / FSV_WINDOW;
            if (!(oc.z >> 31) || j < 0 || j >= o_n_win || o_x_s > gs) continue;
            const int32_t slot = B.idx2[oc.y + (uint32_t)j];
            if (slot == -2) { atomicAdd(&S.cover, 1u); atomicAdd(&S.cov[0], 1); atomicAdd(&S.cov[blen], -1); continue; }
            if (slot < 0) continue;
            const fsv_wpath *P = paths2 + slot;
            const uint4 h0 = *reinterpret_cast<const uint4 *>(P);
            if ((h0.w & 0xffu) != 1u) continue;
            const uint2 h1 = *reinterpret_cast<const uint2 *>((const uint8_t *)P + 16);
            const int perr = (int)(int16_t)(h0.z >> 16);
            atomicAdd(&S.cover, 1u);
            const int ry_start = (int)h0.x, plen = (int)(int16_t)(h0.z & 0xffffu);
            int n2 = 0;
            if (perr != 0) {
                atomicAdd(&S.terr, (uint32_t)perr);
                uint2 pv[13];
                load_path_ops(P, pv);
                const uint32_t nz = S.stage_path(lane, pv);
                n2 = cons_walk<EVC>(S, S.path[lane], nz, plen, 0, blen, false, A.store, h1.x, (int)h1.y, (int)((h0.w >> 8) & 0xffu), ry_start);
            }
            atomicAdd(&S.cov[0], 1);
            atomicAdd(&S.cov[plen - n2], -1);
        }
        __syncthreads();
        if (S.cover < 3u || S.terr == 0u) continue;
        if (S.evn > (uint32_t)EVC && lane == 0) atomicOr(&A.warn[r], (uint32_t)FSV_W_INS_EVENTS);
        int c0, c1;
        lane_columns(lane, blen, c0, c1);
        for (int c = c0; c < c1; c++) S.own[c] = 1;
        const bool differs = S.decide_columns(lane, c0, c1, cws, blen, len_now, false, A.ins_dag, [&](int c, int, bool kept) { S.own[c] = kept; });
        uint8_t (*s_out)[14] = S.out();
        int mine = 0;
        for (int c = c0; c < c1; c++) mine += s_out[c][0];
        if (__ballot(differs) == 0ull) continue;
        int off = wave_incl_sum(mine, lane) - mine;
        for (int c = c0; c < c1; c++) { S.off[c] = (uint16_t)off; off += s_out[c][0]; }
        const int sb = FSV_BND_SIDE, eb = blen - 1 - FSV_BND_SIDE;
        int fs = 0x7fffffff, fe = 0x7fffffff;
        for (int c = c0; c < c1; c++) { if (S.own[c] && c >= sb && c < fs) fs = c; if (S.own[c] && c >= eb && c < fe) fe = c; }
        for (int d = 32; d >= 1; d >>= 1) { fs = min(fs, __shfl_xor(fs, d)); fe = min(fe, __shfl_xor(fe, d)); }
        __syncthreads();
        if (eb <= sb || fs == 0x7fffffff || fe == 0x7fffffff) continue;
        const int o0 = (int)S.off[fs] + s_out[fs][0] - 1, o1 = (int)S.off[fe] + s_out[fe][0] - 1;
        const int R0 = cws + fs, R1 = cws + fe, sc = LB - cws;
        const int o_split = sc <= fs ? o0 : (sc > fe ? o1 + 1 : (int)S.off[sc]);
        const int lb_prev = (int)B.lb[gw - 1];
        BndPatch bp;
        bp.valid = 1; bp.pad = 0;
        bp.ts = (uint16_t)max(0, R0 - lb_prev); bp.told = (uint16_t)max(0, min(R1, LB - 1) - R0 + 1); bp.tnew = (uint16_t)(o_split - o0);
        bp.hs = (uint16_t)(max(R0, LB) - LB); bp.hold = (uint16_t)max(0, R1 - max(R0, LB) + 1); bp.hnew = (uint16_t)(o1 + 1 - o_split);
        if (R0 < lb_prev || o1 + 1 - o0 > FSV_CW_STRIDE) {
            if (lane == 0) atomicOr(&A.warn[r], (uint32_t)FSV_W_WINDOW_KEPT);
            continue;
        }
        uint8_t *dst = patch_bytes + (size_t)gw * FSV_CW_STRIDE;
        for (int c = c0; c < c1; c++)
            for (int b = 0; b < s_out[c][0]; b++) { const int pos = (int)S.off[c] + b; if (pos >= o0 && pos <= o1) dst[pos - o0] = s_out[c][1 + b]; }
        if (lane == 0) patch[gw] = bp;
    }
}

__global__ __launch_bounds__(64) void k_bnd_apply(const uint32_t *__restrict__ gwin_read, const uint32_t *__restrict__ gwin_off, const BndPatch *__restrict__ patch,
                                                  const uint8_t *__restrict__ patch_bytes, const uint32_t *__restrict__ bnd_flag, uint32_t n_gwin,
                                                  uint8_t *__restrict__ cwin, uint16_t *__restrict__ cwin_len, uint32_t *__restrict__ changed, uint32_t *__restrict__ warn)
{
    __shared__ uint8_t s_old[FSV_CW_STRIDE];
    const uint32_t gw = blockIdx.x;
    if (gw >= n_gwin) return;
    const uint32_t r = gwin_read[gw];
    const bool has_h = gw > gwin_off[r] && (bnd_flag[gw] & 1u) && patch[gw].valid;
    const bool has_t = gw + 1 < gwin_off[r + 1] && (bnd_flag[gw + 1] & 1u) && patch[gw + 1].valid;
    if (!has_h && !has_t) return;
    const int lane = threadIdx.x;
    const int len = cwin_len[gw];
    uint8_t *w = cwin + (size_t)gw * FSV_CW_STRIDE;
    for (int i = lane; i < len; i += 64) s_old[i] = w[i];
    __syncthreads();
    int hs = 0, hold = 0, hnew = 0, ts = len, told = 0, tnew = 0;
    const uint8_t *hb = nullptr, *tb = nullptr;
    if (has_h) { const BndPatch p = patch[gw]; hs = p.hs; hold = p.hold; hnew = p.hnew; hb = patch_bytes + (size_t)gw * FSV_CW_STRIDE + p.tnew; }
    if (has_t) { const BndPatch p = patch[gw + 1]; ts = p.ts; told = p.told; tnew = p.tnew; tb = patch_bytes + (size_t)(gw + 1) * FSV_CW_STRIDE; }
    if (told == 0 && tnew == 0) ts = len;
    const int new_len = len - hold + hnew - told + tnew;
    if (hs + hold > ts || ts + told > len || new_len > FSV_CW_STRIDE || new_len < 0) {
        if (lane == 0) atomicOr(&warn[r], (uint32_t)FSV_W_WINDOW_KEPT);
        return;
    }
    const int a1 = hs, a2 = a1 + hnew, a3 = a2 + (ts - hs - hold), a4 = a3 + tnew;
    for (int i = lane; i < new_len; i += 64) {
        uint8_t v;
        if (i < a1) v = s_old[i];
        else if (i < a2) v = hb[i - a1];
        else if (i < a3) v = s_old[hs + hold + (i - a2)];
        else if (i < a4) v = tb[i - a3];
        else v = s_old[ts + told + (i - a4)];
        w[i] = v;
    }
    if (lane == 0) { cwin_len[gw] = (uint16_t)new_len; changed[r] = 1u; }
}

}
```

Before: 2378 regions/s.

## Size junction and bcig passes by device task counts with grid-stride list kernels

Replaces the full-capacity grids of the junction and bcig passes with grid-stride kernels sized to a fixed number of blocks per CU that read the true task count from the device. Task generation now walks only the dirty overlaps instead of every task, with the index arrays pre-filled by a memset. Boundary apply now visits only the listed junction windows and their neighbours instead of launching one block per window. It also unrolls the dirty-path scan by four loads. This cuts the launch of many empty blocks, at the cost of extra memsets and possible imbalance when lists are long.

```diff
diff --git a/focalsv_amd/csrc/asm.hip b/focalsv_amd/csrc/asm.hip
--- a/focalsv_amd/csrc/asm.hip
+++ b/focalsv_amd/csrc/asm.hip
@@ -457,6 +457,7 @@
     int pass, round;
     bool wide_bands; int k_cap;
     bool all_accepted;
+    bool short_list = false;
 };
 
 template <bool STAMP, class Grid>
@@ -514,8 +515,12 @@
     if (fix) TRY(ensure(ctx, W.fix_list, task_cap));
     const PathLists lists{{W.dp_list16.p, W.dp_list.p, W.dp_list_e3.p, W.dp_list2.p, W.dp_list3.p, W.dp_wide.p, W.dp_xwide.p, fix ? W.fix_list.p : nullptr},
                           {ct + CT_DP_SB16, ct + CT_DP, ct + CT_DP_FR3, ct + CT_DP_SB, ct + CT_DP_GEN, ct + CT_DP_WIDE, ct + CT_DP_XW, fix ? ct + CT_FIX : nullptr}};
-    FSV_LAUNCH(ctx, ctx->stream, k_path_fast, dim3((fsv_grid_for(task_cap, 256) + 7u) & ~7u), dim3(256), 0, store, W.ovl.p, tasks, res, task_cap, paths, lists,
-               J.all_accepted, J.n_tasks_dev);
+    if (J.short_list && J.n_tasks_dev)
+        FSV_LAUNCH(ctx, ctx->stream, k_path_fast<true>, dim3(fsv_list_grid(ctx, task_cap, 256)), dim3(256), 0, store, W.ovl.p, tasks, res, task_cap, paths, lists,
+                   J.all_accepted, J.n_tasks_dev);
+    else
+        FSV_LAUNCH(ctx, ctx->stream, k_path_fast<false>, dim3((fsv_grid_for(task_cap, 256) + 7u) & ~7u), dim3(256), 0, store, W.ovl.p, tasks, res, task_cap, paths, lists,
+                   J.all_accepted, J.n_tasks_dev);
     W.kt.end(ctx);
     W.kt.begin(ctx, J.pass, KN_PATH_DP, 0);
     TRY(getenv("FSV_K6_STAMPS") ? path_walks<true>(ctx, W, J, persistent) : path_walks<false>(ctx, W, J, persistent));
@@ -536,6 +541,11 @@
     return FSV_OK;
 }
 
+static uint32_t walk_grid(const fsv_ctx *ctx, uint32_t n_pairs)
+{
+    return (std::max(1u, std::min<uint32_t>(fsv_grid_for(n_pairs, 4 * FSV_OW_SLOTS), (uint32_t)std::max(1, ctx->n_cu) * 64u)) + 7u) & ~7u;
+}
+
 static int second_pass(fsv_ctx *ctx, AsmWs &W, const Round &R)
 {
     const fsv_asm_params &P = R.P; const Batch &B = R.B; const Geometry &G = R.G;
@@ -563,30 +573,31 @@
     TRY(ensure_each(ctx, (size_t)n_gwin + 2, W.bnd_flag, W.bnd_list, W.bnd_patch));
     TRY(ensure(ctx, W.bnd_bytes, (size_t)(n_gwin + 2) * FSV_CW_STRIDE));
     TRY(zero(ctx, W.bnd_flag, (size_t)n_gwin + 2));
+    FSV_HIP(ctx, hipMemsetAsync(W.idx2.p, 0xff, (size_t)task_cap * sizeof(int32_t), ctx->stream));
     BndArgs A;
-    A.tasks = W.tasks.p; A.paths = W.paths.p; A.n_tasks = R.ct + CT_TASKS;
-    A.ovl_c = W.ovl_c.p; A.pair_base = W.pair_base.p; A.set_start = W.set_start.p; A.n_sets = B.n_sets; A.pair_read = W.pair_read.p;
+    A.tasks = W.tasks.p; A.paths = W.paths.p; A.n_tasks = R.ct + CT_TASKS; A.task_cap = task_cap;
+    A.ovl_c = W.ovl_c.p; A.n_pairs = B.n_pairs; A.pair_base = W.pair_base.p; A.set_start = W.set_start.p; A.n_sets = B.n_sets; A.pair_read = W.pair_read.p;
     A.gwin_off = W.gwin_off.p; A.lb = W.lb.p; A.cwin_len = W.cwin_len.p;
     A.cov3 = W.cov3.p; A.read_dirty = W.read_dirty.p;
     A.brel_off = W.brel_off.p; A.b_base = a_words; A.thr_tab = W.thr_tab.p;
     A.tasks2 = W.tasks2.p; A.idx2 = W.idx2.p; A.n_tasks2 = ct2 + CT_TASKS;
     A.bnd_flag = W.bnd_flag.p; A.bnd_list = W.bnd_list.p; A.n_bnd = ct2 + CT_B_LIST; A.store2 = store2;
-    FSV_LAUNCH(ctx, ctx->stream, k_bnd_tasks, dim3((fsv_grid_for(task_cap, 256) + 7u) & ~7u), dim3(256), 0, A);
+    FSV_LAUNCH(ctx, ctx->stream, k_bnd_tasks, dim3(walk_grid(ctx, B.n_pairs)), dim3(256), 0, A);
     W.kt.end(ctx);
     W.kt.begin(ctx, PASS_JUNCTIONS, KN_BPM, 0);
-    TRY(fsv_bpm_windows_dev_n(ctx, store2, W.tasks2.p, task_cap, ct2 + CT_TASKS, W.res2.p, P.k_cap));
-    FSV_LAUNCH(ctx, ctx->stream, k_bnd_retry, dim3(fsv_grid_for(task_cap, 256)), dim3(256), 0, W.tasks2.p, W.res2.p, ct2 + CT_TASKS, W.tasks3.p, W.src3.p,
-               ct2 + CT_B_RETRY, P.k_cap);
-    TRY(fsv_bpm_windows_dev_n(ctx, store2, W.tasks3.p, task_cap, ct2 + CT_B_RETRY, W.res3.p, P.k_cap));
-    FSV_LAUNCH(ctx, ctx->stream, k_bnd_scatter, dim3(fsv_grid_for(task_cap, 256)), dim3(256), 0, W.res2.p, W.res3.p, W.src3.p, ct2 + CT_B_RETRY);
+    const dim3 grid_s(fsv_list_grid(ctx, task_cap, 256));
+    TRY(fsv_bpm_windows_list_dev(ctx, store2, W.tasks2.p, task_cap, ct2 + CT_TASKS, W.res2.p, P.k_cap));
+    FSV_LAUNCH(ctx, ctx->stream, k_bnd_retry, grid_s, dim3(256), 0, W.tasks2.p, W.res2.p, ct2 + CT_TASKS, W.tasks3.p, W.src3.p, ct2 + CT_B_RETRY, P.k_cap, task_cap);
+    TRY(fsv_bpm_windows_list_dev(ctx, store2, W.tasks3.p, task_cap, ct2 + CT_B_RETRY, W.res3.p, P.k_cap));
+    FSV_LAUNCH(ctx, ctx->stream, k_bnd_scatter, grid_s, dim3(256), 0, W.res2.p, W.res3.p, W.src3.p, ct2 + CT_B_RETRY, task_cap);
     W.kt.end(ctx);
-    TRY(path_stage(ctx, W, PathJob{store2, W.tasks2.p, W.res2.p, W.paths2.p, task_cap, ct2 + CT_TASKS, ct2, PASS_JUNCTIONS, R.round, R.wide_bands, P.k_cap, false}));
+    TRY(path_stage(ctx, W, PathJob{store2, W.tasks2.p, W.res2.p, W.paths2.p, task_cap, ct2 + CT_TASKS, ct2, PASS_JUNCTIONS, R.round, R.wide_bands, P.k_cap, false, true}));
     const uint32_t grid_l = std::min<uint32_t>(std::max(1u, n_gwin), (uint32_t)ctx->n_cu * 16);
     W.kt.begin(ctx, PASS_JUNCTIONS, KN_BND_CONS, 0);
     if (R.wide_bands) FSV_LAUNCH(ctx, ctx->stream, k_bnd_consensus<FSV_EV_CAP_WIDE>, dim3(grid_l), dim3(64), 0, R.C, A, W.paths2.p, store2, W.bnd_patch.p, W.bnd_bytes.p);
     else FSV_LAUNCH(ctx, ctx->stream, k_bnd_consensus<FSV_EV_CAP>, dim3(grid_l), dim3(64), 0, R.C, A, W.paths2.p, store2, W.bnd_patch.p, W.bnd_bytes.p);
-    FSV_LAUNCH(ctx, ctx->stream, k_bnd_apply, dim3(std::max(1u, n_gwin)), dim3(64), 0, W.gwin_read.p, W.gwin_off.p, W.bnd_patch.p, W.bnd_bytes.p, W.bnd_flag.p, n_gwin,
-               W.cwin.p, W.cwin_len.p, W.changed.p, W.warn.p);
+    FSV_LAUNCH(ctx, ctx->stream, k_bnd_apply, dim3(grid_l), dim3(64), 0, W.gwin_read.p, W.gwin_off.p, W.bnd_patch.p, W.bnd_bytes.p, W.bnd_flag.p, W.bnd_list.p,
+               ct2 + CT_B_LIST, n_gwin, W.cwin.p, W.cwin_len.p, W.changed.p, W.warn.p);
     W.kt.end(ctx);
     return FSV_OK;
 }
@@ -888,21 +899,23 @@
     TRY(ensure(ctx, W.bc_win, (size_t)(n_gwin + 2) * 3));
     FSV_LAUNCH(ctx, ctx->stream, k_bcwin_init, dim3(fsv_grid_for(n_gwin + 2, 256)), dim3(256), 0, W.bc_win.p, n_gwin + 2);
     BcigArgs BA;
-    BA.tasks = W.tasks.p; BA.paths = W.paths.p; BA.n_tasks = R.ct + CT_TASKS;
+    BA.tasks = W.tasks.p; BA.paths = W.paths.p; BA.n_tasks = R.ct + CT_TASKS; BA.task_cap = task_cap;
+    BA.ovl_c = W.ovl_c.p; BA.n_pairs = R.B.n_pairs;
     BA.pair_read = W.pair_read.p; BA.read_dirty = W.read_dirty.p; BA.gwin_off = W.gwin_off.p;
     BA.thr_tab = W.thr_tab.p; BA.k_cap = P.k_cap;
     BA.tasks2 = W.tasks2.p; BA.bc_idx = W.bc_idx.p; BA.n_tasks2 = ct3 + CT_TASKS;
     BA.n_same = ct3 + CT_B_RETRY; BA.n_used = ct3 + CT_B_LIST;
     BA.res2 = W.res2.p; BA.paths2 = W.paths2.p; BA.bc_rec = W.bc_rec.p; BA.bc_win = W.bc_win.p;
     W.kt.begin(ctx, KN_PARTITION, 0);
-    FSV_LAUNCH(ctx, ctx->stream, k_bcig_tasks, dim3((fsv_grid_for(task_cap, 256) + 7u) & ~7u), dim3(256), 0, BA);
+    FSV_HIP(ctx, hipMemsetAsync(W.bc_idx.p, 0xff, (size_t)task_cap * sizeof(int32_t), ctx->stream));
+    FSV_LAUNCH(ctx, ctx->stream, k_bcig_tasks, dim3(walk_grid(ctx, R.B.n_pairs)), dim3(256), 0, BA);
     W.kt.end(ctx);
     W.kt.begin(ctx, PASS_BCIG, KN_BPM, 0);
-    TRY(fsv_bpm_windows_dev_n(ctx, R.store, W.tasks2.p, task_cap, ct3 + CT_TASKS, W.res2.p, P.k_cap));
+    TRY(fsv_bpm_windows_list_dev(ctx, R.store, W.tasks2.p, task_cap, ct3 + CT_TASKS, W.res2.p, P.k_cap));
     W.kt.end(ctx);
-    TRY(path_stage(ctx, W, PathJob{R.store, W.tasks2.p, W.res2.p, W.paths2.p, task_cap, ct3 + CT_TASKS, ct3, PASS_BCIG, R.round, R.wide_bands, P.k_cap, false}));
+    TRY(path_stage(ctx, W, PathJob{R.store, W.tasks2.p, W.res2.p, W.paths2.p, task_cap, ct3 + CT_TASKS, ct3, PASS_BCIG, R.round, R.wide_bands, P.k_cap, false, true}));
     W.kt.begin(ctx, KN_PARTITION, 0);
-    FSV_LAUNCH(ctx, ctx->stream, k_bcig_accept, dim3(fsv_grid_for(task_cap, 256)), dim3(256), 0, BA);
+    FSV_LAUNCH(ctx, ctx->stream, k_bcig_accept, dim3(fsv_list_grid(ctx, task_cap, 256)), dim3(256), 0, BA);
     W.kt.end(ctx);
     SA.bc_idx = W.bc_idx.p; SA.bc_rec = W.bc_rec.p; SA.bc_paths = W.paths2.p;
     SL.bc_win = W.bc_win.p;
@@ -1232,7 +1245,7 @@
             const uint32_t *c2 = h_ct.data() + (size_t)(PASS_JUNCTIONS * (P.n_rounds + 1) + sl) * CT_SLOT;
             const uint64_t n2 = c2[CT_TASKS], n3 = c2[CT_B_RETRY], n_dp2 = n_dp_of(c2);
             n_windows2 += n2 + n3;
-            set(PASS_JUNCTIONS, KN_BND, sl, nt * (sizeof(fsv_wtask) + 128ull) + n2 * sizeof(fsv_wtask));
+            set(PASS_JUNCTIONS, KN_BND, sl, (uint64_t)B.n_pairs * sizeof(uint4) + n2 * (2 * sizeof(fsv_wtask) + 128ull));
             set(PASS_JUNCTIONS, KN_BPM, sl, (n2 + n3) * 212ull);
             set(PASS_JUNCTIONS, KN_PATH_FAST, sl, n2 * (16ull + 196ull) + (n2 - n_dp2) * 128ull);
             set(PASS_JUNCTIONS, KN_PATH_DP, sl, n_dp2 * (196ull + 128ull));
diff --git a/focalsv_amd/csrc/asm_kernels.h b/focalsv_amd/csrc/asm_kernels.h
--- a/focalsv_amd/csrc/asm_kernels.h
+++ b/focalsv_amd/csrc/asm_kernels.h
@@ -881,15 +881,9 @@
     return true;
 }
 
-__global__ __launch_bounds__(256) void k_path_fast(const uint32_t *__restrict__ store, const fsv_ovl *__restrict__ ovl,
-                                                   const fsv_wtask *__restrict__ tasks, const fsv_wres *__restrict__ res, uint32_t n_tasks,
-                                                   fsv_wpath *__restrict__ paths, PathLists L, bool write_clean_ops, const uint32_t *__restrict__ n_dev)
-{
-    if (n_dev) n_tasks = min(*n_dev, n_tasks);
-    uint32_t blk;
-    if (!xcd_block((n_tasks + 255u) >> 8, blk)) return;
-    const uint32_t tid = blk * blockDim.x + threadIdx.x;
-    if (tid >= n_tasks) return;
+__device__ __forceinline__ void path_fast_task(const uint32_t *__restrict__ store, const fsv_ovl *__restrict__ ovl, const fsv_wtask *__restrict__ tasks,
+                                               const fsv_wres *__restrict__ res, fsv_wpath *__restrict__ paths, const PathLists &L, bool write_clean_ops, uint32_t tid)
+{
     const fsv_wtask t = tasks[tid];
     const fsv_wres r = res[tid];
     fsv_wpath *P = paths + tid;
@@ -916,6 +910,24 @@
             if (cls >= 0) { P->state = 2; list[at] = tid; }
         }
     }
+}
+
+template <bool SHORT_LIST>
+__global__ __launch_bounds__(256) void k_path_fast(const uint32_t *__restrict__ store, const fsv_ovl *__restrict__ ovl,
+                                                   const fsv_wtask *__restrict__ tasks, const fsv_wres *__restrict__ res, uint32_t n_tasks,
+                                                   fsv_wpath *__restrict__ paths, PathLists L, bool write_clean_ops, const uint32_t *__restrict__ n_dev)
+{
+    if (n_dev) n_tasks = min(*n_dev, n_tasks);
+    if (SHORT_LIST) {
+        for (uint32_t base = blockIdx.x * blockDim.x; base < n_tasks; base += gridDim.x * blockDim.x)
+            if (base + threadIdx.x < n_tasks) path_fast_task(store, ovl, tasks, res, paths, L, write_clean_ops, base + threadIdx.x);
+        return;
+    }
+    uint32_t blk;
+    if (!xcd_block((n_tasks + 255u) >> 8, blk)) return;
+    const uint32_t tid = blk * blockDim.x + threadIdx.x;
+    if (tid >= n_tasks) return;
+    path_fast_task(store, ovl, tasks, res, paths, L, write_clean_ops, tid);
 }
 
 struct PathWalk {
diff --git a/focalsv_amd/csrc/fsv_internal.h b/focalsv_amd/csrc/fsv_internal.h
--- a/focalsv_amd/csrc/fsv_internal.h
+++ b/focalsv_amd/csrc/fsv_internal.h
@@ -189,3 +189,11 @@
 
 int fsv_bpm_windows_dev_n(fsv_ctx *ctx, const uint32_t *store_dev, const fsv_wtask *tasks_dev, uint32_t n_tasks, const uint32_t *n_dev,
                           fsv_wres *res_dev, int k_cap);
+#define FSV_LIST_BLOCKS_PER_CU 8
+int fsv_bpm_windows_list_dev(fsv_ctx *ctx, const uint32_t *store_dev, const fsv_wtask *tasks_dev, uint32_t cap, const uint32_t *n_dev,
+                             fsv_wres *res_dev, int k_cap);
+static inline unsigned fsv_list_grid(const fsv_ctx *ctx, uint64_t cap, unsigned block)
+{
+    const unsigned full = fsv_grid_for(cap, block), fixed = (unsigned)(ctx->n_cu > 0 ? ctx->n_cu : 1) * FSV_LIST_BLOCKS_PER_CU;
+    return full < fixed ? (full ? full : 1u) : fixed;
+}
diff --git a/focalsv_amd/csrc/k5_bpm.hip b/focalsv_amd/csrc/k5_bpm.hip
--- a/focalsv_amd/csrc/k5_bpm.hip
+++ b/focalsv_amd/csrc/k5_bpm.hip
@@ -3,14 +3,8 @@
 
 namespace {
 
-__global__ __launch_bounds__(256) void k5_bpm_kernel(const uint32_t *__restrict__ store, const fsv_wtask *__restrict__ tasks,
-                                                     uint32_t n_tasks, fsv_wres *__restrict__ res, const uint32_t *__restrict__ n_dev)
+__device__ __forceinline__ void k5_bpm_task(const uint32_t *__restrict__ store, const fsv_wtask *__restrict__ tasks, fsv_wres *__restrict__ res, uint32_t tid)
 {
-    if (n_dev) n_tasks = min(*n_dev, n_tasks);
-    uint32_t blk;
-    if (!xcd_block((n_tasks + 255u) >> 8, blk)) return;
-    const uint32_t tid = blk * blockDim.x + threadIdx.x;
-    if (tid >= n_tasks) return;
     const fsv_wtask t = tasks[tid];
     fsv_wres r;
     bool exact = bpm_window_geometry(t, r);
@@ -44,6 +38,22 @@
     res[tid] = r;
 }
 
+template <bool SHORT_LIST>
+__global__ __launch_bounds__(256) void k5_bpm_kernel(const uint32_t *__restrict__ store, const fsv_wtask *__restrict__ tasks,
+                                                     uint32_t n_tasks, fsv_wres *__restrict__ res, const uint32_t *__restrict__ n_dev)
+{
+    if (n_dev) n_tasks = min(*n_dev, n_tasks);
+    if (SHORT_LIST) {
+        for (uint32_t tid = blockIdx.x * blockDim.x + threadIdx.x; tid < n_tasks; tid += gridDim.x * blockDim.x) k5_bpm_task(store, tasks, res, tid);
+        return;
+    }
+    uint32_t blk;
+    if (!xcd_block((n_tasks + 255u) >> 8, blk)) return;
+    const uint32_t tid = blk * blockDim.x + threadIdx.x;
+    if (tid >= n_tasks) return;
+    k5_bpm_task(store, tasks, res, tid);
+}
+
 __global__ __launch_bounds__(256) void k5_bpm_wide_kernel(const uint32_t *__restrict__ store, const fsv_wtask *__restrict__ tasks,
                                                           uint32_t n_tasks, fsv_wres *__restrict__ res, const uint32_t *__restrict__ n_dev, int k_cap)
 {
@@ -75,7 +85,17 @@
     if (k_cap > FSV_K_MAX)
         FSV_LAUNCH(ctx, ctx->stream, k5_bpm_wide_kernel, dim3(fsv_grid_for(n_tasks, 256)), dim3(256), 0, store_dev, tasks_dev, n_tasks, res_dev, n_dev, k_cap);
     else
-    FSV_LAUNCH(ctx, ctx->stream, k5_bpm_kernel, dim3((fsv_grid_for(n_tasks, 256) + 7u) & ~7u), dim3(256), 0, store_dev, tasks_dev, n_tasks, res_dev, n_dev);
+    FSV_LAUNCH(ctx, ctx->stream, k5_bpm_kernel<false>, dim3((fsv_grid_for(n_tasks, 256) + 7u) & ~7u), dim3(256), 0, store_dev, tasks_dev, n_tasks, res_dev, n_dev);
+    return FSV_OK;
+}
+
+int fsv_bpm_windows_list_dev(fsv_ctx *ctx, const uint32_t *store_dev, const fsv_wtask *tasks_dev, uint32_t cap, const uint32_t *n_dev,
+                             fsv_wres *res_dev, int k_cap)
+{
+    if (!ctx || !store_dev || !n_dev || (!tasks_dev && cap) || (!res_dev && cap)) return FSV_EINVAL;
+    if (cap == 0 || k_cap > FSV_K_MAX) return fsv_bpm_windows_dev_n(ctx, store_dev, tasks_dev, cap, n_dev, res_dev, k_cap);
+    FSV_HIP(ctx, hipSetDevice(ctx->device));
+    FSV_LAUNCH(ctx, ctx->stream, k5_bpm_kernel<true>, dim3(fsv_list_grid(ctx, cap, 256)), dim3(256), 0, store_dev, tasks_dev, cap, res_dev, n_dev);
     return FSV_OK;
 }
 
diff --git a/focalsv_amd/csrc/k_consensus.h b/focalsv_amd/csrc/k_consensus.h
--- a/focalsv_amd/csrc/k_consensus.h
+++ b/focalsv_amd/csrc/k_consensus.h
@@ -46,15 +46,22 @@
         if (!(oc.z >> 31)) continue;
         const int n_win = (int)(oc.z & 0x7fffffffu);
         int prev_end = 0; bool prev_ok = false;
-        for (int j = 0; j < n_win && !dirty; j++) {
-            const uint4 h0 = *reinterpret_cast<const uint4 *>(paths + (oc.y + (uint32_t)j));
-            const bool ok = (h0.w & 0xffu) == 1u;
-            if (ok) {
-                if ((int16_t)(h0.z >> 16) != 0) dirty = true;
-                if (prev_ok && (int)h0.x - prev_end - 1 != 0) dirty = true;
-                prev_end = (int)h0.y;
-            }
-            prev_ok = ok;
+        for (int j0 = 0; j0 < n_win && !dirty; j0 += 4) {
+            uint4 h[4];
+#pragma unroll
+            for (int k = 0; k < 4; k++)
+                h[k] = j0 + k < n_win ? *reinterpret_cast<const uint4 *>(paths + (oc.y + (uint32_t)(j0 + k))) : make_uint4(0u, 0u, 0u, 0u);
+#pragma unroll
+            for (int k = 0; k < 4; k++) {
+                const uint4 h0 = h[k];
+                const bool ok = (h0.w & 0xffu) == 1u;
+                if (ok) {
+                    if ((int16_t)(h0.z >> 16) != 0) dirty = true;
+                    if (prev_ok && (int)h0.x - prev_end - 1 != 0) dirty = true;
+                    prev_end = (int)h0.y;
+                }
+                prev_ok = ok;
+            }
         }
     }
     const bool any = __ballot(dirty) != 0ull;
@@ -675,6 +682,8 @@
 #define FSV_BC_SCAN 10
 struct BcigArgs {
     const fsv_wtask *tasks; const fsv_wpath *paths; const uint32_t *n_tasks;
+    uint32_t task_cap;
+    const uint4 *ovl_c; uint32_t n_pairs;
     const uint32_t *pair_read, *read_dirty, *gwin_off; const uint8_t *thr_tab; int k_cap;
     fsv_wtask *tasks2; int32_t *bc_idx; uint32_t *n_tasks2;
     const fsv_wres *res2; const fsv_wpath *paths2; uint4 *bc_rec; int32_t *bc_win;
@@ -720,23 +729,59 @@
     if (gw < n_gwin) { bc_win[3 * (size_t)gw] = 0; bc_win[3 * (size_t)gw + 1] = 0x7fffffff; bc_win[3 * (size_t)gw + 2] = -1; }
 }
 
-__global__ __launch_bounds__(256) void k_bcig_tasks(BcigArgs A)
-{
-    const uint32_t n_tasks = min(*A.n_tasks, gridDim.x * blockDim.x);
-    uint32_t blk;
-    if (!xcd_block((n_tasks + 255u) >> 8, blk)) return;
-    const uint32_t ti = blk * blockDim.x + threadIdx.x;
-    if (ti >= n_tasks) return;
-    A.bc_idx[ti] = -1;
-    if (ti + 1 >= n_tasks) return;
-    const fsv_wtask t0 = A.tasks[ti];
-    if (!A.read_dirty[A.pair_read[t0.ovl]]) return;
+#define FSV_OW_SLOTS 32
+struct OvlFacts { uint32_t p, read, first, a, b; };
+struct OvlWalkLds { uint32_t incl[4][FSV_OW_SLOTS], first[4][FSV_OW_SLOTS], read[4][FSV_OW_SLOTS], a[4][FSV_OW_SLOTS], b[4][FSV_OW_SLOTS]; };
+template <class Win>
+__device__ __forceinline__ void walk_dirty_overlaps(const uint4 *__restrict__ ovl_c, const uint32_t *__restrict__ pair_read, const uint32_t *__restrict__ read_dirty,
+                                                    const uint32_t *__restrict__ per_read_a, const uint32_t *__restrict__ per_read_b, uint32_t n_pairs, Win win)
+{
+    static_assert((FSV_OW_SLOTS & (FSV_OW_SLOTS - 1)) == 0 && FSV_OW_SLOTS <= 64, "the owner search halves a power of two; a slot a lane");
+    __shared__ OvlWalkLds S;
+    const uint32_t lane = threadIdx.x & 63u, wv = (threadIdx.x >> 6) & 3u, per_block = 4u * FSV_OW_SLOTS;
+    const uint32_t n_items = (uint32_t)(((uint64_t)n_pairs + per_block - 1) / per_block), per = (n_items + 7u) >> 3;
+    for (uint32_t it = blockIdx.x; (it >> 3) < per; it += gridDim.x) {
+        const uint32_t item = (it & 7u) * per + (it >> 3);
+        if (item >= n_items) break;
+        const uint64_t p0 = (uint64_t)item * per_block + (uint64_t)wv * FSV_OW_SLOTS, p = p0 + lane;
+        uint32_t first = 0, nw = 0, r = 0, fa = 0, fb = 0;
+        if (lane < FSV_OW_SLOTS && p < n_pairs) {
+            const uint4 oc = ovl_c[p];
+            if (oc.z >> 31) {
+                r = pair_read[p];
+                const uint32_t dirty = read_dirty[r];
+                if (per_read_a) fa = per_read_a[r];
+                if (per_read_b) fb = per_read_b[r];
+                if (dirty) { first = oc.y; nw = oc.z & 0x7fffffffu; }
+            }
+        }
+        uint32_t incl = nw;
+        for (uint32_t off = 1; off < FSV_OW_SLOTS; off <<= 1) { const uint32_t o = __shfl_up(incl, off, 64); if (lane >= off) incl += o; }
+        const uint32_t total = __shfl(incl, FSV_OW_SLOTS - 1, 64);
+        __syncthreads();
+        if (lane < FSV_OW_SLOTS) { S.incl[wv][lane] = incl; S.first[wv][lane] = first; S.read[wv][lane] = r; S.a[wv][lane] = fa; S.b[wv][lane] = fb; }
+        __syncthreads();
+        for (uint32_t i = lane; i < total; i += 64u) {
+            uint32_t o = 0;
+#pragma unroll
+            for (uint32_t st = FSV_OW_SLOTS / 2; st; st >>= 1) if (S.incl[wv][o + st - 1] <= i) o += st;
+            const uint32_t end = S.incl[wv][o], before = o ? S.incl[wv][o - 1] : 0u;
+            OvlFacts F;
+            F.p = (uint32_t)p0 + o; F.read = S.read[wv][o]; F.first = S.first[wv][o]; F.a = S.a[wv][o]; F.b = S.b[wv][o];
+            win(F, i - before, end - before);
+        }
+    }
+}
+
+__device__ __forceinline__ void bcig_window(const BcigArgs &A, const OvlFacts &F, uint32_t j, uint32_t n_win, uint32_t n_tasks)
+{
+    const uint32_t ti = F.first + j;
+    if (j + 1 >= n_win || ti + 1 >= n_tasks) return;
+    const fsv_wtask t0 = A.tasks[ti], t1 = A.tasks[ti + 1];
     const uint4 h0 = *reinterpret_cast<const uint4 *>(A.paths + ti), h1 = *reinterpret_cast<const uint4 *>(A.paths + ti + 1);
     if ((h0.w & 0xffu) != 1u || (h1.w & 0xffu) != 1u) return;
     const int y_distance = (int)h1.x - (int)h0.y - 1;
     if (y_distance == 0 && !((h0.w >> 16) & 2u) && !((h1.w >> 16) & 1u)) return;
-    const fsv_wtask t1 = A.tasks[ti + 1];
-    if (t1.ovl != t0.ovl) return;
     int y_start = (int)h0.y, x_start = t0.x_start + (int)t0.x_len - 1;
     const int leftLen = min(min(x_start - t0.x_start, y_start), FSV_BC_SIDE);
     const int rightLen = min(min(t1.x_start + (int)t1.x_len - x_start, t0.y_len - y_start), FSV_BC_SIDE);
@@ -753,10 +798,14 @@
     A.bc_idx[ti] = (int32_t)slot;
 }
 
-__global__ __launch_bounds__(256) void k_bcig_accept(BcigArgs A)
-{
-    const uint32_t slot = blockIdx.x * blockDim.x + threadIdx.x;
-    if (slot >= *A.n_tasks2) return;
+__global__ __launch_bounds__(256) void k_bcig_tasks(BcigArgs A)
+{
+    const uint32_t n_tasks = min(*A.n_tasks, A.task_cap);
+    walk_dirty_overlaps(A.ovl_c, A.pair_read, A.read_dirty, nullptr, nullptr, A.n_pairs, [&](const OvlFacts &F, uint32_t j, uint32_t n_win) { bcig_window(A, F, j, n_win, n_tasks); });
+}
+
+__device__ __forceinline__ void bcig_accept_one(const BcigArgs &A, uint32_t slot, uint32_t n_tasks)
+{
     A.bc_rec[slot] = make_uint4(0, 0, 0, 0);
     const fsv_wtask w = A.tasks2[slot];
     const fsv_wres r = A.res2[slot];
@@ -775,7 +824,7 @@
     const uint32_t first_ti = ti - t0.win;
     if (t0.win == 0 && w.x_start == t0.x_start) L = 0;
     {
-        const bool last_junction = ti + 2 >= *A.n_tasks || A.tasks[ti + 2].ovl != t0.ovl;
+        const bool last_junction = ti + 2 >= n_tasks || A.tasks[ti + 2].ovl != t0.ovl;
         if (last_junction && w.x_start + xLen - 1 == t1.x_start + (int)t1.x_len - 1) R = 0;
     }
     (void)first_ti;
@@ -833,6 +882,12 @@
         if (mm1) A.bc_win[3 * (size_t)(g0 + 1)] = 1;
         atomicMin(&A.bc_win[3 * (size_t)(g0 + 1) + 1], w.x_start + lo1 - gs0 - FSV_WINDOW); atomicMax(&A.bc_win[3 * (size_t)(g0 + 1) + 2], w.x_start + hi1d - gs0 - FSV_WINDOW);
     }
+}
+
+__global__ __launch_bounds__(256) void k_bcig_accept(BcigArgs A)
+{
+    const uint32_t n2 = min(*A.n_tasks2, A.task_cap), n_tasks = min(*A.n_tasks, A.task_cap);
+    for (uint32_t slot = blockIdx.x * blockDim.x + threadIdx.x; slot < n2; slot += gridDim.x * blockDim.x) bcig_accept_one(A, slot, n_tasks);
 }
 
 #define FSV_SITE_WIN_CAP 255
@@ -1172,7 +1227,9 @@
 #define FSV_BND_SIDE 25
 struct BndArgs {
     const fsv_wtask *tasks; const fsv_wpath *paths; const uint32_t *n_tasks;
-    const uint4 *ovl_c; const uint32_t *pair_base, *set_start; uint32_t n_sets; const uint32_t *pair_read;
+    uint32_t task_cap;
+    const uint4 *ovl_c; uint32_t n_pairs;
+    const uint32_t *pair_base, *set_start; uint32_t n_sets; const uint32_t *pair_read;
     const uint32_t *gwin_off, *lb; const uint16_t *cwin_len; const uint8_t *cov3; const uint32_t *read_dirty;
     const uint32_t *brel_off; uint32_t b_base;
     const uint8_t *thr_tab;
@@ -1181,23 +1238,16 @@
     const uint32_t *store2;
 };
 
-__global__ __launch_bounds__(256) void k_bnd_tasks(BndArgs A)
-{
-    const uint32_t n_tasks = min(*A.n_tasks, gridDim.x * blockDim.x);
-    uint32_t blk;
-    if (!xcd_block((n_tasks + 255u) >> 8, blk)) return;
-    const uint32_t ti = blk * blockDim.x + threadIdx.x;
+__device__ __forceinline__ void bnd_window(const BndArgs &A, const OvlFacts &F, uint32_t j, uint32_t n_tasks)
+{
+    const uint32_t ti = F.first + j;
     if (ti >= n_tasks) return;
-    A.idx2[ti] = -1;
     const fsv_wtask t = A.tasks[ti];
+    const uint4 h0 = *reinterpret_cast<const uint4 *>(A.paths + ti);
     if (t.x_start % FSV_WINDOW != 0 || t.x_start == 0) return;
-    const uint32_t p = t.ovl;
-    const uint32_t r = A.pair_read[p];
-    const uint4 oc = A.ovl_c[p];
-    const uint4 h0 = *reinterpret_cast<const uint4 *>(A.paths + ti);
-    const uint32_t dirty = A.read_dirty[r], gwo = A.gwin_off[r];
-    if (!(dirty && (oc.z >> 31) && (h0.w & 0xffu) == 1u)) return;
-    const uint32_t gw = gwo + (uint32_t)(t.x_start / FSV_WINDOW);
+    const uint32_t p = F.p;
+    if ((h0.w & 0xffu) != 1u) return;
+    const uint32_t gw = F.a + (uint32_t)(t.x_start / FSV_WINDOW);
     const uint32_t cov = A.cov3[gw], cwl = A.cwin_len[gw];
     const int LB = (int)A.lb[gw];
     if (!cov || LB == 0) return;
@@ -1205,7 +1255,7 @@
     const int cws = max(0, LB - FSV_BND_HALF), cwe = min(len_now - 1, LB + FSV_BND_HALF - 1), blen = cwe - cws + 1;
     const int y_start = (int)h0.x - FSV_BND_HALF;
     if (y_start < 0 || blen < 1) return;
-    const uint32_t xw2 = A.b_base + A.brel_off[r];
+    const uint32_t xw2 = A.b_base + F.b;
     if (y_start + blen <= t.y_len) {
         uint32_t acc = 0;
 #pragma unroll
@@ -1236,23 +1286,32 @@
     if (!(atomicOr(&A.bnd_flag[gw], 1u) & 1u)) A.bnd_list[atomicAdd(A.n_bnd, 1u)] = gw;
 }
 
+__global__ __launch_bounds__(256, 8) void k_bnd_tasks(BndArgs A)
+{
+    const uint32_t n_tasks = min(*A.n_tasks, A.task_cap);
+    walk_dirty_overlaps(A.ovl_c, A.pair_read, A.read_dirty, A.gwin_off, A.brel_off, A.n_pairs, [&](const OvlFacts &F, uint32_t j, uint32_t) { bnd_window(A, F, j, n_tasks); });
+}
+
 __global__ __launch_bounds__(256) void k_bnd_retry(fsv_wtask *__restrict__ tasks2, const fsv_wres *__restrict__ res2, const uint32_t *__restrict__ n_tasks2,
-                                                   fsv_wtask *__restrict__ tasks3, uint32_t *__restrict__ src3, uint32_t *__restrict__ n3, int k_cap)
-{
-    const uint32_t i = blockIdx.x * blockDim.x + threadIdx.x;
-    if (i >= *n_tasks2 || res2[i].err >= 0) return;
-    fsv_wtask t = tasks2[i];
-    t.k = (uint8_t)double_thr(t.k, t.x_len, k_cap);
-    tasks2[i].k = t.k;
-    const uint32_t j = atomicAdd(n3, 1u);
-    tasks3[j] = t; src3[j] = i;
+                                                   fsv_wtask *__restrict__ tasks3, uint32_t *__restrict__ src3, uint32_t *__restrict__ n3, int k_cap,
+                                                   uint32_t task_cap)
+{
+    const uint32_t n2 = min(*n_tasks2, task_cap);
+    for (uint32_t i = blockIdx.x * blockDim.x + threadIdx.x; i < n2; i += gridDim.x * blockDim.x) {
+        if (res2[i].err >= 0) continue;
+        fsv_wtask t = tasks2[i];
+        t.k = (uint8_t)double_thr(t.k, t.x_len, k_cap);
+        tasks2[i].k = t.k;
+        const uint32_t j = atomicAdd(n3, 1u);
+        tasks3[j] = t; src3[j] = i;
+    }
 }
 
 __global__ __launch_bounds__(256) void k_bnd_scatter(fsv_wres *__restrict__ res2, const fsv_wres *__restrict__ res3, const uint32_t *__restrict__ src3,
-                                                     const uint32_t *__restrict__ n3)
-{
-    const uint32_t j = blockIdx.x * blockDim.x + threadIdx.x;
-    if (j < *n3) res2[src3[j]] = res3[j];
+                                                     const uint32_t *__restrict__ n3, uint32_t task_cap)
+{
+    const uint32_t n = min(*n3, task_cap);
+    for (uint32_t j = blockIdx.x * blockDim.x + threadIdx.x; j < n; j += gridDim.x * blockDim.x) res2[src3[j]] = res3[j];
 }
 
 struct BndPatch { uint16_t ts, told, tnew, hs, hold, hnew, valid, pad; };
@@ -1347,13 +1406,10 @@
     }
 }
 
-__global__ __launch_bounds__(64) void k_bnd_apply(const uint32_t *__restrict__ gwin_read, const uint32_t *__restrict__ gwin_off, const BndPatch *__restrict__ patch,
-                                                  const uint8_t *__restrict__ patch_bytes, const uint32_t *__restrict__ bnd_flag, uint32_t n_gwin,
-                                                  uint8_t *__restrict__ cwin, uint16_t *__restrict__ cwin_len, uint32_t *__restrict__ changed, uint32_t *__restrict__ warn)
-{
-    __shared__ uint8_t s_old[FSV_CW_STRIDE];
-    const uint32_t gw = blockIdx.x;
-    if (gw >= n_gwin) return;
+__device__ __forceinline__ void bnd_apply_window(uint32_t gw, uint8_t *s_old, const uint32_t *__restrict__ gwin_read, const uint32_t *__restrict__ gwin_off,
+                                                 const BndPatch *__restrict__ patch, const uint8_t *__restrict__ patch_bytes, const uint32_t *__restrict__ bnd_flag,
+                                                 uint8_t *__restrict__ cwin, uint16_t *__restrict__ cwin_len, uint32_t *__restrict__ changed, uint32_t *__restrict__ warn)
+{
     const uint32_t r = gwin_read[gw];
     const bool has_h = gw > gwin_off[r] && (bnd_flag[gw] & 1u) && patch[gw].valid;
     const bool has_t = gw + 1 < gwin_off[r + 1] && (bnd_flag[gw + 1] & 1u) && patch[gw + 1].valid;
@@ -1386,4 +1442,22 @@
     if (lane == 0) { cwin_len[gw] = (uint16_t)new_len; changed[r] = 1u; }
 }
 
-}
+__global__ __launch_bounds__(64) void k_bnd_apply(const uint32_t *__restrict__ gwin_read, const uint32_t *__restrict__ gwin_off, const BndPatch *__restrict__ patch,
+                                                  const uint8_t *__restrict__ patch_bytes, const uint32_t *__restrict__ bnd_flag, const uint32_t *__restrict__ bnd_list,
+                                                  const uint32_t *__restrict__ n_bnd, uint32_t n_gwin,
+                                                  uint8_t *__restrict__ cwin, uint16_t *__restrict__ cwin_len, uint32_t *__restrict__ changed, uint32_t *__restrict__ warn)
+{
+    __shared__ uint8_t s_old[FSV_CW_STRIDE];
+    const uint32_t n_list = min(*n_bnd, n_gwin);
+    for (uint32_t li = blockIdx.x; li < n_list; li += gridDim.x) {
+        const uint32_t gw = bnd_list[li];
+        if (gw >= n_gwin) continue;
+        __syncthreads();
+        bnd_apply_window(gw, s_old, gwin_read, gwin_off, patch, patch_bytes, bnd_flag, cwin, cwin_len, changed, warn);
+        if (gw == 0u || (bnd_flag[gw - 1] & 1u)) continue;
+        __syncthreads();
+        bnd_apply_window(gw - 1, s_old, gwin_read, gwin_off, patch, patch_bytes, bnd_flag, cwin, cwin_len, changed, warn);
+    }
+}
+
+}
```

Measured after the change: 2183 regions/s. 0.918x the previous value.
